# MARSLab-UMN/vi_depth_completion

Measured on AMD Instinct MI355X. Metric: frames/sec, higher is better.
Workload: dtype f32

## Files before the change

include/vidc.h:

```cpp
#ifndef VIDC_H
#define VIDC_H

#include <stddef.h>
#include <stdint.h>

#ifdef __cplusplus
extern "C" {
#endif

#if defined(__GNUC__) || defined(__clang__)
#pragma GCC visibility push(default)
#endif

typedef void* vidc_stream_t;

enum vidc_status {
    VIDC_OK = 0,
    VIDC_ERR_NULL = -1,
    VIDC_ERR_SHAPE = -2,
    VIDC_ERR_HIP = -3,
    VIDC_ERR_STATE = -4
};

int vidc_version(void);
const char* vidc_last_error(void);
int vidc_device_info(int* n_cu, int* lds_bytes_per_cu, char* arch_name, int arch_name_len);
#define VIDC_CLOCK_STAMP_WGS 8
int vidc_clock_stamp(long long* out, vidc_stream_t stream);


#define VIDC_WARP_PARAMS 32

int vidc_warp2dof_params(const float* gravity, const float* aligned, int B, float fx, float fy, float cx, float cy,
                         const float* K_inv, int W, int H, float* params, vidc_stream_t stream);

int vidc_warp2dof_fwd(const float* x, const float* params, float* y, int B, int C, int H, int W, float cx, float cy,
                      int align_corners, vidc_stream_t stream);

int vidc_warp2dof_inv_rot_norm(const float* x, const float* params, float* z, int B, int H, int W, float cx, float cy,
                               int align_corners, int normalize, vidc_stream_t stream);

int vidc_warp2dof_fwd_backward(const float* dy, const float* params, float* dx, int B, int C, int H, int W, float cx, float cy,
                               int align_corners, vidc_stream_t stream);
int vidc_warp2dof_inv_rot_norm_backward(const float* x, const float* dz, const float* params, float* dx, int B, int H, int W,
                                        float cx, float cy, int align_corners, int normalize, vidc_stream_t stream);


int vidc_pack_conv_weight(const float* w_oihw, float* w_packed, int Cout, int Cin, int KH, int KW, vidc_stream_t stream);

enum vidc_conv_flags {
    VIDC_RELU1 = 1,
    VIDC_AFFINE2 = 2,
    VIDC_RELU2 = 4,
    VIDC_RESIDUAL = 8,
    VIDC_RELU3 = 16,
    VIDC_ACCUM = 32,
    VIDC_SPLIT_OUT = 64,
    VIDC_NO_F32_OUT = 128,
    VIDC_X_PLANAR_GROUPS = 512,
    VIDC_MXFP8_OUT = 1024,
    VIDC_BF16_OUT = 2048,
    VIDC_STATS_OUT = 256
};

typedef struct vidc_conv_desc {
    const float* x;
    const float* w;
    float* y;
    const float* scale1;
    const float* shift1;
    const float* scale2;
    const float* shift2;
    const float* residual;
    float* workspace;
    int32_t B, H, W, Cin, ldx;
    int32_t Ho, Wo, Cout, ldy, ldr;
    int32_t KH, KW, stride, pad;
    int32_t flags;
    int32_t groups;
    int64_t x_gs, w_gs, y_gs, r_gs, p_gs;
    int32_t tile;
    int32_t splitk;
    int32_t precision;
    int32_t dilation;
    void* y_split;
} vidc_conv_desc;

enum vidc_conv_tile { VIDC_TILE_AUTO = 0, VIDC_TILE_128x128 = 1, VIDC_TILE_128x64 = 2, VIDC_TILE_64x128 = 3,
                      VIDC_TILE_64x64 = 4, VIDC_TILE_64x64_K2 = 5, VIDC_TILE_32x64_K2 = 6, VIDC_TILE_32x32_K4 = 7,
                      VIDC_TILE_32x128 = 8, VIDC_TILE_32x32_K8 = 9,
                      VIDC_TILE_32x64_K2_D5 = 10, VIDC_TILE_32x32_K4_D4 = 11, VIDC_TILE_32x128_D6 = 12, VIDC_TILE_64x64_K2_D4 = 13,
                      VIDC_TILE_32x64_K2_L = 14, VIDC_TILE_32x64_K2_D5_L = 15, VIDC_TILE_32x32_K4_D4_L = 16, VIDC_TILE_64x64_L = 17,
                      VIDC_TILE_64x64_K2_D4_L = 18, VIDC_TILE_64x128_L = 19, VIDC_TILE_128x64_L = 20,
                      VIDC_TILE_64x32_K2 = 21, VIDC_TILE_64x32_K2_D5 = 22, VIDC_TILE_64x32_K2_D5_L = 23,
                      VIDC_TILE_128x128_D3 = 24, VIDC_TILE_128x128_D3_L = 25,
                      VIDC_TILE_256x128 = 26, VIDC_TILE_128x256 = 27,
                      VIDC_TILE_32x64_K2_D2 = 28, VIDC_TILE_64x64_D2 = 29, VIDC_TILE_32x32_K4_D2 = 30, VIDC_TILE_64x128_D2 = 31,
                      VIDC_TILE_64x32_K2_D2 = 32,
                      VIDC_TILE_128x128_D4_P = 33, VIDC_TILE_128x128_D3_P = 34, VIDC_TILE_64x64_D4_P = 35, VIDC_TILE_128x64_D4_P = 36,
                      VIDC_TILE_64x64_K2_D4_P = 37, VIDC_TILE_64x32_K2_D5_P = 38, VIDC_TILE_32x64_K2_D5_P = 39,
                      VIDC_TILE_G96x32_STREAM = 40,
                      VIDC_TILE_G96x64_STREAM3 = 41,
                      VIDC_TILE_WINO4_FUSED = 42,
                      VIDC_TILE_COUNT = 43 };
enum vidc_conv_tile_kind { VIDC_TILE_KIND_AUTO = 0,
                           VIDC_TILE_KIND_MFMA = 1,
                           VIDC_TILE_KIND_STREAM = 2,
                           VIDC_TILE_KIND_WINOGRAD = 3 };
typedef struct vidc_tile_info {
    const char* name;
    int32_t bm, bn, wmw, wnw, wkw, ns, spec;
    int32_t kind;
    int32_t precisions, planner;
} vidc_tile_info;
int vidc_conv_tile_info(int tile, vidc_tile_info* out);

enum vidc_conv_precision { VIDC_PREC_FP32 = 0, VIDC_PREC_BF16X3 = 1, VIDC_PREC_BF16 = 2, VIDC_PREC_MXFP8 = 3 };
int vidc_quant_mxfp8(const float* x, void* y, long long rows, int C, int ldx, int groups, vidc_stream_t stream);
int vidc_pack_conv_weight_mxfp8(const float* w_oihw, void* w_packed, int Cout, int Cin, int KH, int KW, vidc_stream_t stream);
int vidc_cast_bf16(const float* x, void* y, long long rows, int C, int ldx, vidc_stream_t stream);
int vidc_split_bf16x3(const float* x, void* y, long long rows, int C, int ldx, vidc_stream_t stream);
int vidc_pack_conv_weight_bf16x3(const float* w_oihw, void* w_packed, int Cout, int Cin, int KH, int KW, vidc_stream_t stream);
int vidc_pack_conv_weight_bf16(const float* w_oihw, void* w_packed, int Cout, int Cin, int KH, int KW, vidc_stream_t stream);

int vidc_conv2d_bn_act(const vidc_conv_desc* d, vidc_stream_t stream);
#define VIDC_SPLITK_COUNTERS 16384
size_t vidc_conv2d_workspace_bytes(const vidc_conv_desc* d);
int vidc_conv2d_plan(vidc_conv_desc* d);

int vidc_winograd_tiles(int H, int W, int m, int* th, int* tw);
int vidc_winograd_weight_transform(const float* w_oihw, float* u, int Cout, int Cin, int m, vidc_stream_t stream);
int vidc_winograd_weight_pack_fused(const float* u, float* u_packed, int Cout, int Cin, vidc_stream_t stream);
int vidc_winograd_input_transform(const float* x, void* v, int B, int H, int W, int C, int ldx, int Cin, int m, int split, int ldv,
                                  vidc_stream_t stream);
int vidc_winograd_output_transform(const float* mm, float* y, void* y_split, const float* scale1, const float* shift1,
                                   const float* scale2, const float* shift2, int B, int Ho, int Wo, int C, int Cout, int ldy, int m,
                                   int flags, int ldm, vidc_stream_t stream);

int vidc_stem_conv3x3s2(const float* x, const float* w_oihw, float* y, int B, int Cin, int H, int W, int Cout, int ldy,
                        int relu, void* y_split, int split_ch0, vidc_stream_t stream);

int vidc_stem_conv3x3s2_warped(const float* x, const float* warp_params, const float* w_oihw, float* y, int B, int H, int W, int Cout, int ldy,
                               int relu, void* y_split, int split_ch0, float cx, float cy, int align_corners, vidc_stream_t stream);

int vidc_maxpool3x3s2(const float* x, float* y, int B, int H, int W, int C, int ldx, int ldy, void* y_split, vidc_stream_t stream);

enum vidc_up_flags { VIDC_UP_RELU = 1, VIDC_UP_ACCUM = 2, VIDC_UP_NO_F32_OUT = 4,
                     VIDC_UP_SUM_GROUPS_SHIFT = 8  };
int vidc_upsample_bilinear_ac(const float* x, float* y, int B, int h, int w, int C, int ldx, int H, int W, int ldy,
                              int flags, void* y_split, vidc_stream_t stream);

int vidc_avgpool2d(const float* x, float* y, int B, int H, int W, int C, int ldx, int kh, int kw, int sh, int sw, int ph, int pw, int ldy,
                   vidc_stream_t stream);

int vidc_avgpool2d_backward(const float* dy, float* dx, int B, int H, int W, int C, int ldx, int kh, int kw, int sh, int sw, int ph, int pw, int ldy,
                            vidc_stream_t stream);

int vidc_normalize_nchw(const float* x, float* y, int B, int C, int HW, vidc_stream_t stream);

int vidc_head_conv1x1_upsample(const float* x, const float* w, const float* bias, float* lowres, float* y, int B, int h,
                               int w_in, int Cin, int ldx, int Cout, int pad, int H, int W, int relu, vidc_stream_t stream);


#define VIDC_MAX_HYP 300
#define VIDC_PLANE_RECORD 16

size_t vidc_plane_scratch_bytes(int n_slots, int B, int HW);

int vidc_plane_ransac_normal(const float* normals, const uint8_t* ids, const int32_t* slots, int n_slots,
                             const int32_t* hyp_pix, int HW, uint8_t* inlier_mask, int32_t* counts, void* scratch,
                             vidc_stream_t stream);

int vidc_plane_offset(const float* homo, const float* depth, const int32_t* slots, int n_slots, int B,
                      const uint8_t* inlier_mask, const int32_t* counts, int HW, void* scratch, float* records,
                      vidc_stream_t stream);

int vidc_plane_offset_dense(const float* homo, const float* depth, const int32_t* slots, int n_slots, int B,
                            const uint8_t* inlier_mask, const int32_t* counts, int HW, void* scratch, float* records,
                            const int32_t* dense_hyp, const int32_t* dense_n, float* dense_dots, vidc_stream_t stream);

int vidc_plane_project_depth(const float* homo, const int32_t* slots, int n_slots, const uint8_t* inlier_mask, int HW,
                             void* scratch, float* records, float* plane_depth, vidc_stream_t stream);

int vidc_plane_info_count(int B, int HW);
int vidc_plane_finalize(const float* depth, float* plane_depth, int B, int HW, const float* records, int n_slots,
                        int32_t* info, vidc_stream_t stream);

int vidc_plane_block(const float* normals, const uint8_t* ids, const int32_t* slots, int n_slots, const int32_t* hyp_pix, int B, int HW,
                     const float* homo, const float* depth, uint8_t* inlier_mask, int32_t* counts, void* scratch, float* records,
                     const int32_t* dense_hyp, const int32_t* dense_n, float* dense_dots, float* plane_depth, int32_t* info,
                     vidc_stream_t stream);

int vidc_enrich_scatter(const float* plane_depth, const int32_t* sub, const int32_t* sub_offsets, const int32_t* chunk_base,
                        int B, int HW, float* enriched, vidc_stream_t stream);

int vidc_enrich_scatter_from(const float* plane_depth, const float* sparse_depth, const int32_t* sub, const int32_t* sub_offsets,
                             const int32_t* chunk_base, int B, int HW, float* enriched, vidc_stream_t stream);


int vidc_resize_coeffs(int in_size, int out_size, int32_t* bounds, int32_t* coeffs, int coeffs_capacity, int* ksize_out);

int vidc_resize_bilinear_u8_to_chw(const uint8_t* src_hwc, float* dst_chw, int B, int H, int W, int C, int Ho, int Wo,
                                   const int32_t* bounds_x, const int32_t* coeffs_x, int ksize_x, const int32_t* bounds_y,
                                   const int32_t* coeffs_y, int ksize_y, vidc_stream_t stream);

int vidc_rasterize_sparse_depth(const double* tracks, const int32_t* offsets, int B, double fx, double fy, double cx, double cy,
                                float* depth, int H, int W, vidc_stream_t stream);
int vidc_nearest_table(int in_size, int out_size, int32_t* table);
int vidc_resize_nearest_u16_depth(const uint16_t* src, float* dst, int B, int H, int W, int Ho, int Wo, const int32_t* xtab,
                                  const int32_t* ytab, float divisor, vidc_stream_t stream);


size_t vidc_depth_metrics_scratch_bytes(long long n);
int vidc_depth_metrics(const float* pred, const float* gt, long long n, double* stats, int accumulate, void* scratch, vidc_stream_t stream);

int vidc_depth_to_mm_u32(const float* depth, uint32_t* mm, long long n, vidc_stream_t stream);

int vidc_normal_metrics(const float* pred, const float* gt, const float* mask, int B, int HW, float* err, double* stats,
                        int accumulate, void* scratch, vidc_stream_t stream);

int vidc_hist_u16(const float* vals, long long n, int hi_filter, uint32_t* hist, vidc_stream_t stream);


size_t vidc_nms_scratch_bytes(int n);
int vidc_nms(const float* boxes_xyxy, const int32_t* order, int n, float threshold, int inclusive, int32_t* keep, int32_t* n_keep,
             void* scratch, vidc_stream_t stream);

size_t vidc_nms_segmented_scratch_bytes(int n_segments, int max_n);
int vidc_nms_segmented(const float* boxes_xyxy, const int32_t* seg_offsets, const int32_t* seg_counts, int n_segments, int max_n,
                       float threshold, int inclusive, int max_keep, int32_t* keep, int32_t* n_keep, void* scratch, vidc_stream_t stream);

int vidc_roi_align_forward(const float* x_nhwc, const float* rois, float* y, int K, int C, int H, int W, int ldx, int pooled_h,
                           int pooled_w, float spatial_scale, int sampling_ratio, vidc_stream_t stream);


int vidc_det_stem_im2col(const float* image01_nchw, float* cols, int B, int H, int W, int Hp, int Wp, float mean_b, float mean_g,
                         float mean_r, vidc_stream_t stream);
int vidc_upsample_nearest2x(const float* x, float* y, int B, int h, int w, int C, int ldx, int ldy, vidc_stream_t stream);

int vidc_mask_scale(const float* x, const float* image_nchw, float* y, int B, int h, int w, int C, int ldx, int ldy, int H, int W,
                    vidc_stream_t stream);
int vidc_rpn_topk_decode(const float* rpn_map, int B, int h, int w, int ld, int A, int stride, const float* cell_anchors_host,
                         int pre_nms_top_n, int img_h, int img_w, float* boxes, float* scores, long long out_stride, vidc_stream_t stream);
int vidc_rpn_topk_decode_levels(const float* const* maps_host, const int32_t* hw_host, const int32_t* strides_host,
                                const float* cell_anchors_host, const int32_t* level_offsets_host, int n_levels, int B, int ld, int A,
                                int pre_nms_top_n, int img_h, int img_w, float* boxes, float* scores, long long out_stride,
                                vidc_stream_t stream);
int vidc_rpn_select(const float* boxes, const float* scores, const int32_t* keep, const int32_t* n_keep, int B, int n_levels,
                    const int32_t* level_offsets_host, int per_level, int total, float* proposals, float* proposal_scores,
                    int32_t* n_proposals, vidc_stream_t stream);
int vidc_roi_align_fpn(const float* const* feats_host, const int32_t* hw_host, int n_levels, int C, const float* boxes, int B, int R,
                       int pooled, int sampling_ratio, float* y, vidc_stream_t stream);
int vidc_det_candidates(const float* head_out, int ld, const float* proposals, const int32_t* n_proposals, int B, int R, int img_h, int img_w,
                        float score_thresh, float* cand_boxes, float* cand_scores, int32_t* cand_src, int32_t* n_cand, vidc_stream_t stream);
int vidc_det_select(const float* cand_boxes, const float* cand_scores, const int32_t* cand_src, const int32_t* n_cand, const int32_t* keep,
                    const int32_t* n_keep, int B, int R, float* det_boxes, float* det_scores, int32_t* n_det, vidc_stream_t stream);
int vidc_mask_paste(const float* mask_logits, int ld, int cls, int M, const float* det_boxes, const int32_t* n_det, int B, int R, int H, int W,
                    float thresh, uint8_t* pasted, vidc_stream_t stream);
size_t vidc_instance_map_scratch_bytes(int B, int R, int H, int W);
int vidc_instance_map(const uint8_t* pasted, const float* det_scores, const int32_t* n_det, int B, int R, int H, int W, float confidence,
                      float min_fraction, uint8_t* inst, void* scratch, vidc_stream_t stream);


size_t vidc_train_scratch_bytes(long long M, int C);

int vidc_bn_train_forward(const float* x, float* y, long long M, int C, int ldx, int ldy, const float* gamma, const float* beta,
                          float* running_mean, float* running_var, float eps, float momentum, int relu, float* save_mean, float* save_rstd,
                          void* y_bf16, void* scratch, vidc_stream_t stream);
int vidc_bn_train_forward_add(const float* x, float* y, long long M, int C, int ldx, int ldy, const float* gamma, const float* beta,
                              float* running_mean, float* running_var, float eps, float momentum, int relu, float* save_mean, float* save_rstd,
                              void* y_bf16, const float* residual, int ldr, void* scratch, vidc_stream_t stream);
int vidc_bn_train_forward_stats(const float* x, float* y, long long M, int C, int ldx, int ldy, const float* gamma, const float* beta,
                                float* running_mean, float* running_var, float eps, float momentum, int relu, float* save_mean, float* save_rstd,
                                void* y_bf16, const float* residual, int ldr, const void* conv_stats, void* scratch, vidc_stream_t stream);
int vidc_bn_train_backward(const float* dy, const float* x, const float* y_relu, float* dx, long long M, int C, int lddy, int ldx, int ldy,
                           int lddx, const float* gamma, const float* save_mean, const float* save_rstd, float* dgamma, float* dbeta,
                           void* dx_bf16, void* scratch, vidc_stream_t stream);
int vidc_bn_train_backward_t(const float* dy, const float* x, const float* y_relu, float* dx, long long M, int C, int lddy, int ldx, int ldy,
                             int lddx, const float* gamma, const float* save_mean, const float* save_rstd, float* dgamma, float* dbeta,
                             void* dx_bf16, void* dx_bf16_t, int Mp, void* scratch, vidc_stream_t stream);
int vidc_colsum(const float* dy, long long M, int C, int ld, float* out, void* scratch, vidc_stream_t stream);
int vidc_add_rows(const float* a, const float* b, float* y, long long M, int C, int lda, int ldb, int ldy, int relu, vidc_stream_t stream);
int vidc_add_rows_bf16(const float* a, const float* b, float* y, long long M, int C, int lda, int ldb, int ldy, int relu, void* y_bf16,
                       vidc_stream_t stream);
int vidc_relu_backward(const float* dy, const float* y, float* dx, long long M, int C, int lddy, int ldy, int lddx, int accumulate,
                       vidc_stream_t stream);
int vidc_maxpool3x3s2_backward(const float* x, const float* dy, float* dx, int B, int H, int W, int C, int ldx, int lddy, int lddx,
                               vidc_stream_t stream);
int vidc_upsample_bilinear_ac_backward(const float* dy, float* dx, int B, int h, int w, int C, int lddy, int lddx, int H, int W,
                                       vidc_stream_t stream);
size_t vidc_head_backward_multi_scratch_bytes(int B, int h, int w, int C, int Cout, int pad);
int vidc_head_backward_multi(const float* g_low, const float* x, const float* wgt, float* dx, float* dw, float* dbias, int B, int h, int w,
                             int C, int ldx, int lddx, int Cout, int pad, void* scratch, vidc_stream_t stream);
size_t vidc_head_backward_scratch_bytes(int B, int h, int w, int C);
int vidc_head_backward(const float* g_low, const float* x, const float* wgt, float* dx, float* dw, float* dbias, int B, int h, int w, int C,
                       int ldx, int lddx, void* scratch, vidc_stream_t stream);
int vidc_masked_l1_loss(const float* pred, const float* gt, long long n, int hw, double* loss, float* dpred, float* terms, void* scratch,
                        vidc_stream_t stream);
int vidc_adam_step(float* p, const float* g, float* m, float* v, long long n, float lr, float beta1, float beta2, float eps, int step,
                   vidc_stream_t stream);
int vidc_train_bn_fold(int enable);
int vidc_grad_narrow_bf16(const float* x, void* y_bf16, long long n, vidc_stream_t stream);
int vidc_grad_widen_bf16(const void* x_bf16, float* y, long long n, vidc_stream_t stream);
int vidc_pack_conv_weight_dgrad(const float* w_oihw, float* w_packed, int Cout, int Cin, int KH, int KW, vidc_stream_t stream);
int vidc_host_mt19937_permutation_prefix(uint32_t* key624, int32_t* pos, long long n, int k, int32_t* idx_out, int32_t* scratch);
typedef struct vidc_pack_item {
    const float* w;
    float* packed;
    int32_t Cout, Cin, KH, KW;
    int32_t kind, reserved;
    int64_t block_begin;
} vidc_pack_item;
long long vidc_pack_item_blocks(int Cout, int Cin, int KH, int KW, int kind);
int vidc_pack_conv_weights_batched(const vidc_pack_item* items_device, int n_items, long long total_blocks, vidc_stream_t stream);
int vidc_zero_stuff(const float* dy, float* z, int B, int Ho, int Wo, int C, int lddy, int stride, int H, int W, vidc_stream_t stream);
size_t vidc_conv_wgrad_scratch_bytes(int B, int Ho, int Wo, int Cout, int Cin, int KH, int KW);
int vidc_conv_wgrad(const float* dy, const float* x, float* dw_oihw, int B, int H, int W, int Cin, int ldx, int Ho, int Wo, int Cout, int lddy,
                    int KH, int KW, int stride, int pad, void* scratch, vidc_stream_t stream);
size_t vidc_conv_wgrad_dilated_scratch_bytes(int B, int Ho, int Wo, int Cout, int Cin, int KH, int KW);
int vidc_conv_wgrad_dilated(const float* dy, const float* x, float* dw_oihw, int B, int H, int W, int Cin, int ldx, int Ho, int Wo, int Cout, int lddy,
                            int KH, int KW, int stride, int pad, int dilation, void* scratch, vidc_stream_t stream);
int vidc_im2col_transposed(const float* x, float* xt, int B, int H, int W, int C, int ldx, int Ho, int Wo, int KH, int KW, int stride, int pad,
                           int Mp, int split, vidc_stream_t stream);
int vidc_im2col_transposed_dilated(const float* x, float* xt, int B, int H, int W, int C, int ldx, int Ho, int Wo, int KH, int KW, int stride, int pad,
                                   int dilation, int Mp, int split, vidc_stream_t stream);
int vidc_transpose_bf16(const void* x_bf16, void* xt_bf16, long long M, int C, int Mp, vidc_stream_t stream);
int vidc_im2col_transposed_bf16(const void* x_bf16, void* xt_bf16, int B, int H, int W, int C, int Ho, int Wo, int KH, int KW, int stride, int pad,
                                int Mp, vidc_stream_t stream);
int vidc_wgrad_permute(const float* tmp, float* dw_oihw, int Cout, int Cin, int taps, vidc_stream_t stream);
int vidc_affine_act_backward(const float* dy, const float* y, const float* c_raw, const float* scale, const float* shift, float* dc,
                             float* dscale, float* dshift, long long M, int C, int lddy, int ldy, int ldc, int lddc, int relu, void* scratch,
                             vidc_stream_t stream);
int vidc_stem_conv3x3s2_backward_data(const float* dy, const float* y_relu, const float* w_oihw, float* dx_nchw, int B, int Cin, int H, int W,
                                      int Cout, int lddy, int ldy, vidc_stream_t stream);
size_t vidc_stem_wgrad_scratch_bytes(int B, int Cin, int H, int W, int Cout);
int vidc_stem_wgrad(const float* dy, const float* x_nchw, float* dw_oihw, int B, int Cin, int H, int W, int Cout, int lddy, void* scratch,
                    vidc_stream_t stream);


size_t vidc_normal_l1_loss_scratch_bytes(int B, int H, int W);
int vidc_normal_l1_loss(const float* pred, const float* normal_gt, const float* mask, int B, int H, int W, int normalize_prediction,
                        double* loss, double* count, double* angle, float* dpred, void* scratch, vidc_stream_t stream);

enum vidc_op_kind { VIDC_OP_CONV = 1, VIDC_OP_STEM = 2, VIDC_OP_MAXPOOL = 3, VIDC_OP_UPSAMPLE = 4, VIDC_OP_HEAD = 5,
                    VIDC_OP_WARP_PARAMS = 6, VIDC_OP_WARP_FWD = 7, VIDC_OP_WARP_INV = 8, VIDC_OP_COPY = 9, VIDC_OP_SPLIT = 10,
                    VIDC_OP_AVGPOOL = 11, VIDC_OP_NORMALIZE = 12, VIDC_OP_DET_IM2COL = 13, VIDC_OP_NEAREST2X = 14,
                     VIDC_OP_MASK = 16 ,
                    VIDC_OP_WINO_IN = 17  ,
                    VIDC_OP_WINO_OUT = 18 ,
                    VIDC_OP_QUANT = 19    ,
                    VIDC_OP_CAST = 20      };

typedef struct vidc_generic_args {
    const void* p[8];
    int32_t i[16];
    float f[8];
} vidc_generic_args;

typedef struct vidc_op {
    int32_t kind;
    int32_t stream_id;
    int32_t wait_mask;
    int32_t reserved;
    union {
        vidc_conv_desc conv;
        vidc_generic_args g;
    } u;
} vidc_op;

#define VIDC_MAX_STREAMS 4
#define VIDC_MAX_SEGMENTS 4

typedef struct vidc_program vidc_program;
int vidc_program_create(const vidc_op* ops, int n_ops, vidc_program** out);
int vidc_program_run(vidc_program* p, vidc_stream_t stream);
int vidc_program_capture(vidc_program* p, vidc_stream_t stream);
int vidc_program_launch(vidc_program* p, vidc_stream_t stream);
int vidc_program_run_range(vidc_program* p, vidc_stream_t stream, int begin, int end);
int vidc_program_capture_range(vidc_program* p, vidc_stream_t stream, int begin, int end, int segment);
int vidc_program_launch_segment(vidc_program* p, vidc_stream_t stream, int segment);
int vidc_program_time(vidc_program* p, vidc_stream_t stream, int iters, int use_graph, float* ms_out, float* per_op_ms);
int vidc_program_destroy(vidc_program* p);

#if defined(__GNUC__) || defined(__clang__)
#pragma GCC visibility pop
#endif

#ifdef __cplusplus
}
#endif
#endif
```

vi_depth_completion_amd/_lib.py:

```python
import ctypes as C
import os
import subprocess

_HERE = os.path.dirname(os.path.abspath(__file__))
LIB_PATH = os.path.join(_HERE, os.environ.get("VIDC_LIB_NAME", "libvidc.so"))
CSRC = os.path.join(_HERE, "csrc")

WARP_PARAMS = 32
MAX_HYP = 300
PLANE_RECORD = 16
MAX_STREAMS = 4
MAX_SEGMENTS = 4
CLOCK_STAMP_WGS = 8

RELU1, AFFINE2, RELU2, RESIDUAL, RELU3, ACCUM, SPLIT_OUT, NO_F32_OUT, STATS_OUT, X_PLANAR_GROUPS, MXFP8_OUT, BF16_OUT = 1, 2, 4, 8, 16, 32, 64, 128, 256, 512, 1024, 2048
UP_RELU, UP_ACCUM, UP_NO_F32_OUT = 1, 2, 4
OP_CONV, OP_STEM, OP_MAXPOOL, OP_UPSAMPLE, OP_HEAD, OP_WARP_PARAMS, OP_WARP_FWD, OP_WARP_INV, OP_COPY, OP_SPLIT, OP_AVGPOOL, OP_NORMALIZE, OP_DET_IM2COL, OP_NEAREST2X, _OP_RETIRED_15, OP_MASK, OP_WINO_IN, OP_WINO_OUT, OP_QUANT, OP_CAST = range(1, 21)
TILE_AUTO = 0
PREC_FP32, PREC_BF16X3, PREC_BF16, PREC_MXFP8 = 0, 1, 2, 3
TILE_KIND_AUTO, TILE_KIND_MFMA, TILE_KIND_STREAM, TILE_KIND_WINOGRAD = range(4)
SPLITK_COUNTERS = 16384

_f32p = C.POINTER(C.c_float)


class PackItem(C.Structure):
    _fields_ = [("w", C.c_void_p), ("packed", C.c_void_p), ("Cout", C.c_int32), ("Cin", C.c_int32), ("KH", C.c_int32), ("KW", C.c_int32),
                ("kind", C.c_int32), ("reserved", C.c_int32), ("block_begin", C.c_int64)]


class TileInfo(C.Structure):
    _fields_ = [("_name", C.c_char_p)] + [(f, C.c_int32) for f in ("bm", "bn", "wmw", "wnw", "wkw", "ns", "spec", "kind", "precisions", "planner")]
    name = property(lambda self: self._name.decode())


class ConvDesc(C.Structure):
    _fields_ = [
        ("x", C.c_void_p), ("w", C.c_void_p), ("y", C.c_void_p),
        ("scale1", C.c_void_p), ("shift1", C.c_void_p), ("scale2", C.c_void_p), ("shift2", C.c_void_p),
        ("residual", C.c_void_p), ("workspace", C.c_void_p),
        ("B", C.c_int32), ("H", C.c_int32), ("W", C.c_int32), ("Cin", C.c_int32), ("ldx", C.c_int32),
        ("Ho", C.c_int32), ("Wo", C.c_int32), ("Cout", C.c_int32), ("ldy", C.c_int32), ("ldr", C.c_int32),
        ("KH", C.c_int32), ("KW", C.c_int32), ("stride", C.c_int32), ("pad", C.c_int32),
        ("flags", C.c_int32), ("groups", C.c_int32),
        ("x_gs", C.c_int64), ("w_gs", C.c_int64), ("y_gs", C.c_int64), ("r_gs", C.c_int64), ("p_gs", C.c_int64),
        ("tile", C.c_int32), ("splitk", C.c_int32), ("precision", C.c_int32), ("dilation", C.c_int32),
        ("y_split", C.c_void_p),
    ]


def conv_desc(B, H, W, Cin, Cout, KH=1, KW=1, stride=1, pad=0, dilation=1, groups=1, Ho=None, Wo=None, ldx=None, ldy=None,
              precision=PREC_FP32, x=None, w=None, y=None, scale1=None, shift1=None, shared_affine=False, scale2=None, shift2=None,
              relu1=False, relu2=False, residual=None, ldr=None, relu3=False, accumulate=False, split_out=None, mx_out=None,
              stats_out=None, no_f32_out=False, wino_fused=False, bf16_out=None):
    assert sum(p is not None for p in (split_out, mx_out, stats_out, bf16_out)) <= 1
    dil = max(dilation, 1)
    Ho = (H + 2 * pad - dil * (KH - 1) - 1) // stride + 1 if Ho is None else Ho
    Wo = (W + 2 * pad - dil * (KW - 1) - 1) // stride + 1 if Wo is None else Wo
    ldx = (Cin if precision == PREC_MXFP8 else groups * Cin) if ldx is None else ldx
    ldy = groups * Cout if ldy is None else ldy
    flags = ((RELU1 if relu1 else 0) | (AFFINE2 | (RELU2 if relu2 else 0) if scale2 is not None else 0) |
             (RESIDUAL | (RELU3 if relu3 else 0) if residual is not None else 0) | (ACCUM if accumulate else 0) |
             (SPLIT_OUT if split_out is not None else 0) | (MXFP8_OUT if mx_out is not None else 0) | (STATS_OUT if stats_out is not None else 0) |
             (BF16_OUT if bf16_out is not None else 0) |
             (NO_F32_OUT if no_f32_out and (split_out is not None or mx_out is not None or bf16_out is not None) else 0))
    x_gs, w_gs = Cin, Cout * KH * KW * Cin
    if precision == PREC_BF16:
        Cin, ldx = Cin // 2, ldx // 2
        x_gs, w_gs = Cin, Cout * KH * KW * Cin
    elif precision == PREC_MXFP8:
        assert ldx == Cin, "an MXFP8 activation is one dense plane of Cin channels per group"
        x_gs, w_gs = B * H * W * Cin // 128 * 33, Cout * KH * KW * Cin // 128 * 33
        Cin, ldx = Cin // 4, Cin // 4
    if wino_fused:
        w_gs = 36 * Cout * Cin
    return ConvDesc(x=x, w=w, y=y, scale1=scale1, shift1=shift1, scale2=scale2, shift2=shift2, residual=residual,
                    B=B, H=H, W=W, Cin=Cin, ldx=ldx, Ho=Ho, Wo=Wo, Cout=Cout, ldy=ldy, ldr=(0 if residual is None else ldr or ldy),
                    KH=KH, KW=KW, stride=stride, pad=pad, flags=flags, groups=groups,
                    x_gs=x_gs, w_gs=w_gs, y_gs=Cout, r_gs=(0 if residual is None else Cout),
                    p_gs=(0 if shared_affine and groups > 1 else Cout),
                    tile=(__getattr__("TILE_WINO4_FUSED") if wino_fused else TILE_AUTO), splitk=1, precision=precision, dilation=dil,
                    y_split=next((p for p in (split_out, mx_out, stats_out, bf16_out) if p is not None), None))


def gemm_desc(rows, K, N, groups=1, ldx=None, ldy=None, precision=PREC_FP32, planar=False, x=None, w=None, y=None, scale1=None,
              shift1=None, shared_affine=True):
    d = conv_desc(1, 1, rows, K, N, groups=groups, ldx=ldx, ldy=ldy, precision=precision, x=x, w=w, y=y, scale1=scale1, shift1=shift1,
                  shared_affine=shared_affine)
    if planar:
        d.flags |= X_PLANAR_GROUPS
        d.x_gs, d.y_gs = rows * d.ldx, rows * d.ldy
    return d


def plan(d, tiling=None):
    if tiling is not None:
        d.tile, d.splitk = tiling
    else:
        check(lib().vidc_conv2d_plan(C.byref(d)), "conv plan")
    return d


class GenericArgs(C.Structure):
    _fields_ = [("p", C.c_void_p * 8), ("i", C.c_int32 * 16), ("f", C.c_float * 8)]


class _OpUnion(C.Union):
    _fields_ = [("conv", ConvDesc), ("g", GenericArgs)]


class Op(C.Structure):
    _fields_ = [("kind", C.c_int32), ("stream_id", C.c_int32), ("wait_mask", C.c_int32), ("reserved", C.c_int32),
                ("u", _OpUnion)]


_vp, _i, _f = C.c_void_p, C.c_int, C.c_float
SIGNATURES = {
    "vidc_version": (C.c_int, []),
    "vidc_last_error": (C.c_char_p, []),
    "vidc_device_info": (C.c_int, [C.POINTER(C.c_int), C.POINTER(C.c_int), C.c_char_p, _i]),
    "vidc_warp2dof_params": (C.c_int, [_vp, _vp, _i, _f, _f, _f, _f, _vp, _i, _i, _vp, _vp]),
    "vidc_warp2dof_fwd": (C.c_int, [_vp, _vp, _vp, _i, _i, _i, _i, _f, _f, _i, _vp]),
    "vidc_warp2dof_inv_rot_norm": (C.c_int, [_vp, _vp, _vp, _i, _i, _i, _f, _f, _i, _i, _vp]),
    "vidc_warp2dof_fwd_backward": (C.c_int, [_vp, _vp, _vp, _i, _i, _i, _i, _f, _f, _i, _vp]),
    "vidc_warp2dof_inv_rot_norm_backward": (C.c_int, [_vp, _vp, _vp, _vp, _i, _i, _i, _f, _f, _i, _i, _vp]),
    "vidc_affine_act_backward": (C.c_int, [_vp, _vp, _vp, _vp, _vp, _vp, _vp, _vp, C.c_longlong, _i, _i, _i, _i, _i, _i, _vp, _vp]),
    "vidc_stem_conv3x3s2_backward_data": (C.c_int, [_vp, _vp, _vp, _vp, _i, _i, _i, _i, _i, _i, _i, _vp]),
    "vidc_pack_conv_weight": (C.c_int, [_vp, _vp, _i, _i, _i, _i, _vp]),
    "vidc_split_bf16x3": (C.c_int, [_vp, _vp, C.c_longlong, _i, _i, _vp]),
    "vidc_pack_conv_weight_bf16x3": (C.c_int, [_vp, _vp, _i, _i, _i, _i, _vp]),
    "vidc_pack_conv_weight_bf16": (C.c_int, [_vp, _vp, _i, _i, _i, _i, _vp]),
    "vidc_quant_mxfp8": (C.c_int, [_vp, _vp, C.c_longlong, _i, _i, _i, _vp]),
    "vidc_pack_conv_weight_mxfp8": (C.c_int, [_vp, _vp, _i, _i, _i, _i, _vp]),
    "vidc_conv2d_bn_act": (C.c_int, [C.POINTER(ConvDesc), _vp]),
    "vidc_conv2d_workspace_bytes": (C.c_size_t, [C.POINTER(ConvDesc)]),
    "vidc_conv2d_plan": (C.c_int, [C.POINTER(ConvDesc)]),
    "vidc_conv_tile_info": (C.c_int, [_i, C.POINTER(TileInfo)]),
    "vidc_train_scratch_bytes": (C.c_size_t, [C.c_longlong, _i]),
    "vidc_bn_train_forward": (C.c_int, [_vp, _vp, C.c_longlong, _i, _i, _i, _vp, _vp, _vp, _vp, _f, _f, _i, _vp, _vp, _vp, _vp, _vp]),
    "vidc_bn_train_forward_add": (C.c_int, [_vp, _vp, C.c_longlong, _i, _i, _i, _vp, _vp, _vp, _vp, _f, _f, _i, _vp, _vp, _vp, _vp, _i, _vp, _vp]),
    "vidc_bn_train_forward_stats": (C.c_int, [_vp, _vp, C.c_longlong, _i, _i, _i, _vp, _vp, _vp, _vp, _f, _f, _i, _vp, _vp, _vp, _vp, _i, _vp, _vp, _vp]),
    "vidc_bn_train_backward": (C.c_int, [_vp, _vp, _vp, _vp, C.c_longlong, _i, _i, _i, _i, _i, _vp, _vp, _vp, _vp, _vp, _vp, _vp, _vp]),
    "vidc_bn_train_backward_t": (C.c_int, [_vp, _vp, _vp, _vp, C.c_longlong, _i, _i, _i, _i, _i, _vp, _vp, _vp, _vp, _vp, _vp, _vp, _i, _vp, _vp]),
    "vidc_colsum": (C.c_int, [_vp, C.c_longlong, _i, _i, _vp, _vp, _vp]),
    "vidc_add_rows": (C.c_int, [_vp, _vp, _vp, C.c_longlong, _i, _i, _i, _i, _i, _vp]),
    "vidc_add_rows_bf16": (C.c_int, [_vp, _vp, _vp, C.c_longlong, _i, _i, _i, _i, _i, _vp, _vp]),
    "vidc_relu_backward": (C.c_int, [_vp, _vp, _vp, C.c_longlong, _i, _i, _i, _i, _i, _vp]),
    "vidc_maxpool3x3s2_backward": (C.c_int, [_vp, _vp, _vp, _i, _i, _i, _i, _i, _i, _i, _vp]),
    "vidc_upsample_bilinear_ac_backward": (C.c_int, [_vp, _vp, _i, _i, _i, _i, _i, _i, _i, _i, _vp]),
    "vidc_head_backward_scratch_bytes": (C.c_size_t, [_i, _i, _i, _i]),
    "vidc_head_backward": (C.c_int, [_vp, _vp, _vp, _vp, _vp, _vp, _i, _i, _i, _i, _i, _i, _vp, _vp]),
    "vidc_masked_l1_loss": (C.c_int, [_vp, _vp, C.c_longlong, _i, _vp, _vp, _vp, _vp, _vp]),
    "vidc_normal_l1_loss_scratch_bytes": (C.c_size_t, [_i, _i, _i]),
    "vidc_normal_l1_loss": (C.c_int, [_vp, _vp, _vp, _i, _i, _i, _i, _vp, _vp, _vp, _vp, _vp, _vp]),
    "vidc_head_backward_multi_scratch_bytes": (C.c_size_t, [_i, _i, _i, _i, _i, _i]),
    "vidc_head_backward_multi": (C.c_int, [_vp, _vp, _vp, _vp, _vp, _vp, _i, _i, _i, _i, _i, _i, _i, _i, _vp, _vp]),
    "vidc_clock_stamp": (C.c_int, [_vp, _vp]),
    "vidc_adam_step": (C.c_int, [_vp, _vp, _vp, _vp, C.c_longlong, _f, _f, _f, _f, _i, _vp]),
    "vidc_train_bn_fold": (C.c_int, [_i]),
    "vidc_grad_narrow_bf16": (C.c_int, [_vp, _vp, C.c_longlong, _vp]),
    "vidc_grad_widen_bf16": (C.c_int, [_vp, _vp, C.c_longlong, _vp]),
    "vidc_pack_conv_weight_dgrad": (C.c_int, [_vp, _vp, _i, _i, _i, _i, _vp]),
    "vidc_cast_bf16": (C.c_int, [_vp, _vp, C.c_longlong, _i, _i, _vp]),
    "vidc_host_mt19937_permutation_prefix": (C.c_int, [_vp, _vp, C.c_longlong, _i, _vp, _vp]),
    "vidc_pack_item_blocks": (C.c_longlong, [_i, _i, _i, _i, _i]),
    "vidc_pack_conv_weights_batched": (C.c_int, [_vp, _i, C.c_longlong, _vp]),
    "vidc_zero_stuff": (C.c_int, [_vp, _vp, _i, _i, _i, _i, _i, _i, _i, _i, _vp]),
    "vidc_conv_wgrad_scratch_bytes": (C.c_size_t, [_i, _i, _i, _i, _i, _i, _i]),
    "vidc_conv_wgrad": (C.c_int, [_vp, _vp, _vp, _i, _i, _i, _i, _i, _i, _i, _i, _i, _i, _i, _i, _i, _vp, _vp]),
    "vidc_im2col_transposed": (C.c_int, [_vp, _vp, _i, _i, _i, _i, _i, _i, _i, _i, _i, _i, _i, _i, _i, _vp]),
    "vidc_conv_wgrad_dilated_scratch_bytes": (C.c_size_t, [_i, _i, _i, _i, _i, _i, _i]),
    "vidc_conv_wgrad_dilated": (C.c_int, [_vp, _vp, _vp, _i, _i, _i, _i, _i, _i, _i, _i, _i, _i, _i, _i, _i, _i, _vp, _vp]),
    "vidc_im2col_transposed_dilated": (C.c_int, [_vp, _vp, _i, _i, _i, _i, _i, _i, _i, _i, _i, _i, _i, _i, _i, _i, _vp]),
    "vidc_wgrad_permute": (C.c_int, [_vp, _vp, _i, _i, _i, _vp]),
    "vidc_transpose_bf16": (C.c_int, [_vp, _vp, C.c_longlong, _i, _i, _vp]),
    "vidc_im2col_transposed_bf16": (C.c_int, [_vp, _vp, _i, _i, _i, _i, _i, _i, _i, _i, _i, _i, _i, _vp]),
    "vidc_stem_wgrad_scratch_bytes": (C.c_size_t, [_i, _i, _i, _i, _i]),
    "vidc_stem_wgrad": (C.c_int, [_vp, _vp, _vp, _i, _i, _i, _i, _i, _i, _vp, _vp]),
    "vidc_winograd_tiles": (C.c_int, [_i, _i, _i, C.POINTER(C.c_int), C.POINTER(C.c_int)]),
    "vidc_winograd_weight_transform": (C.c_int, [_vp, _vp, _i, _i, _i, _vp]),
    "vidc_winograd_weight_pack_fused": (C.c_int, [_vp, _vp, _i, _i, _vp]),
    "vidc_winograd_input_transform": (C.c_int, [_vp, _vp, _i, _i, _i, _i, _i, _i, _i, _i, _i, _vp]),
    "vidc_winograd_output_transform": (C.c_int, [_vp, _vp, _vp, _vp, _vp, _vp, _vp, _i, _i, _i, _i, _i, _i, _i, _i, _i, _vp]),
    "vidc_stem_conv3x3s2": (C.c_int, [_vp, _vp, _vp, _i, _i, _i, _i, _i, _i, _i, _vp, _i, _vp]),
    "vidc_stem_conv3x3s2_warped": (C.c_int, [_vp, _vp, _vp, _vp, _i, _i, _i, _i, _i, _i, _vp, _i, _f, _f, _i, _vp]),
    "vidc_maxpool3x3s2": (C.c_int, [_vp, _vp, _i, _i, _i, _i, _i, _i, _vp, _vp]),
    "vidc_upsample_bilinear_ac": (C.c_int, [_vp, _vp, _i, _i, _i, _i, _i, _i, _i, _i, _i, _vp, _vp]),
    "vidc_avgpool2d": (C.c_int, [_vp, _vp, _i, _i, _i, _i, _i, _i, _i, _i, _i, _i, _i, _i, _vp]),
    "vidc_avgpool2d_backward": (C.c_int, [_vp, _vp, _i, _i, _i, _i, _i, _i, _i, _i, _i, _i, _i, _i, _vp]),
    "vidc_normalize_nchw": (C.c_int, [_vp, _vp, _i, _i, _i, _vp]),
    "vidc_head_conv1x1_upsample": (C.c_int, [_vp, _vp, _vp, _vp, _vp, _i, _i, _i, _i, _i, _i, _i, _i, _i, _i, _vp]),
    "vidc_plane_scratch_bytes": (C.c_size_t, [_i, _i, _i]),
    "vidc_plane_ransac_normal": (C.c_int, [_vp, _vp, _vp, _i, _vp, _i, _vp, _vp, _vp, _vp]),
    "vidc_plane_offset": (C.c_int, [_vp, _vp, _vp, _i, _i, _vp, _vp, _i, _vp, _vp, _vp]),
    "vidc_plane_offset_dense": (C.c_int, [_vp, _vp, _vp, _i, _i, _vp, _vp, _i, _vp, _vp, _vp, _vp, _vp, _vp]),
    "vidc_plane_project_depth": (C.c_int, [_vp, _vp, _i, _vp, _i, _vp, _vp, _vp, _vp]),
    "vidc_plane_info_count": (C.c_int, [_i, _i]),
    "vidc_plane_finalize": (C.c_int, [_vp, _vp, _i, _i, _vp, _i, _vp, _vp]),
    "vidc_plane_block": (C.c_int, [_vp, _vp, _vp, _i, _vp, _i, _i, _vp, _vp, _vp, _vp, _vp, _vp, _vp, _vp, _vp, _vp, _vp, _vp]),
    "vidc_enrich_scatter": (C.c_int, [_vp, _vp, _vp, _vp, _i, _i, _vp, _vp]),
    "vidc_enrich_scatter_from": (C.c_int, [_vp, _vp, _vp, _vp, _vp, _i, _i, _vp, _vp]),
    "vidc_resize_coeffs": (C.c_int, [_i, _i, _vp, _vp, _i, C.POINTER(C.c_int)]),
    "vidc_resize_bilinear_u8_to_chw": (C.c_int, [_vp, _vp, _i, _i, _i, _i, _i, _i, _vp, _vp, _i, _vp, _vp, _i, _vp]),
    "vidc_rasterize_sparse_depth": (C.c_int, [_vp, _vp, _i, C.c_double, C.c_double, C.c_double, C.c_double, _vp, _i, _i, _vp]),
    "vidc_nearest_table": (C.c_int, [_i, _i, _vp]),
    "vidc_resize_nearest_u16_depth": (C.c_int, [_vp, _vp, _i, _i, _i, _i, _i, _vp, _vp, C.c_float, _vp]),
    "vidc_depth_metrics_scratch_bytes": (C.c_size_t, [C.c_longlong]),
    "vidc_depth_metrics": (C.c_int, [_vp, _vp, C.c_longlong, _vp, _i, _vp, _vp]),
    "vidc_depth_to_mm_u32": (C.c_int, [_vp, _vp, C.c_longlong, _vp]),
    "vidc_normal_metrics": (C.c_int, [_vp, _vp, _vp, _i, _i, _vp, _vp, _i, _vp, _vp]),
    "vidc_hist_u16": (C.c_int, [_vp, C.c_longlong, _i, _vp, _vp]),
    "vidc_nms_scratch_bytes": (C.c_size_t, [_i]),
    "vidc_nms": (C.c_int, [_vp, _vp, _i, _f, _i, _vp, _vp, _vp, _vp]),
    "vidc_nms_segmented_scratch_bytes": (C.c_size_t, [_i, _i]),
    "vidc_nms_segmented": (C.c_int, [_vp, _vp, _vp, _i, _i, _f, _i, _i, _vp, _vp, _vp, _vp]),
    "vidc_roi_align_forward": (C.c_int, [_vp, _vp, _vp, _i, _i, _i, _i, _i, _i, _i, _f, _i, _vp]),
    "vidc_det_stem_im2col": (C.c_int, [_vp, _vp, _i, _i, _i, _i, _i, _f, _f, _f, _vp]),
    "vidc_upsample_nearest2x": (C.c_int, [_vp, _vp, _i, _i, _i, _i, _i, _i, _vp]),
    "vidc_mask_scale": (C.c_int, [_vp, _vp, _vp, _i, _i, _i, _i, _i, _i, _i, _i, _vp]),
    "vidc_rpn_topk_decode": (C.c_int, [_vp, _i, _i, _i, _i, _i, _i, _vp, _i, _i, _i, _vp, _vp, C.c_longlong, _vp]),
    "vidc_rpn_topk_decode_levels": (C.c_int, [_vp, _vp, _vp, _vp, _vp, _i, _i, _i, _i, _i, _i, _i, _vp, _vp, C.c_longlong, _vp]),
    "vidc_rpn_select": (C.c_int, [_vp, _vp, _vp, _vp, _i, _i, _vp, _i, _i, _vp, _vp, _vp, _vp]),
    "vidc_roi_align_fpn": (C.c_int, [_vp, _vp, _i, _i, _vp, _i, _i, _i, _i, _vp, _vp]),
    "vidc_det_candidates": (C.c_int, [_vp, _i, _vp, _vp, _i, _i, _i, _i, _f, _vp, _vp, _vp, _vp, _vp]),
    "vidc_det_select": (C.c_int, [_vp, _vp, _vp, _vp, _vp, _vp, _i, _i, _vp, _vp, _vp, _vp]),
    "vidc_mask_paste": (C.c_int, [_vp, _i, _i, _i, _vp, _vp, _i, _i, _i, _i, _f, _vp, _vp]),
    "vidc_instance_map_scratch_bytes": (C.c_size_t, [_i, _i, _i, _i]),
    "vidc_instance_map": (C.c_int, [_vp, _vp, _vp, _i, _i, _i, _i, _f, _f, _vp, _vp, _vp]),
    "vidc_program_create": (C.c_int, [C.POINTER(Op), _i, C.POINTER(_vp)]),
    "vidc_program_run": (C.c_int, [_vp, _vp]),
    "vidc_program_capture": (C.c_int, [_vp, _vp]),
    "vidc_program_launch": (C.c_int, [_vp, _vp]),
    "vidc_program_run_range": (C.c_int, [_vp, _vp, _i, _i]),
    "vidc_program_capture_range": (C.c_int, [_vp, _vp, _i, _i, _i]),
    "vidc_program_launch_segment": (C.c_int, [_vp, _vp, _i]),
    "vidc_program_time": (C.c_int, [_vp, _vp, _i, _i, _f32p, _f32p]),
    "vidc_program_destroy": (C.c_int, [_vp]),
}

_lib = None


def build(force=False, verbose=False):
    srcs = [os.path.join(CSRC, f) for f in os.listdir(CSRC) if f.endswith((".hip", ".h", ".def", ".map")) or f == "Makefile"]
    srcs.append(os.path.join(os.path.dirname(_HERE), "include", "vidc.h"))
    if not force and os.path.exists(LIB_PATH) and os.path.getmtime(LIB_PATH) >= max(os.path.getmtime(s) for s in srcs):
        return LIB_PATH
    cmd = ["make", "-C", CSRC, "-j%d" % min(8, os.cpu_count() or 1)]
    r = subprocess.run(cmd, stdout=subprocess.PIPE, stderr=subprocess.STDOUT, text=True)
    if verbose or r.returncode != 0:
        print(r.stdout)
    if r.returncode != 0:
        raise RuntimeError("building libvidc.so failed (hipcc, gfx950)")
    return LIB_PATH


def lib():
    global _lib
    if _lib is None:
        if not os.path.exists(LIB_PATH):
            raise RuntimeError("libvidc.so is not built (%s); run `python -c 'import __graft_entry__ as g; g.build()'`. "
                               "There is no CPU/eager fallback for the HIP path." % LIB_PATH)
        L = C.CDLL(LIB_PATH)
        for name, (res, args) in SIGNATURES.items():
            fn = getattr(L, name)
            fn.restype, fn.argtypes = res, args
        if L.vidc_version() != 1:
            raise RuntimeError("libvidc.so ABI version mismatch")
        _lib = L
    return _lib


_TILE_TABLES = ("TILE_INFO", "TILE_COUNT", "TILE_NAMES", "MXFP8_TILES", "BF16_TILES", "TILE_WINO4_FUSED")


def __getattr__(name):
    if name not in _TILE_TABLES:
        raise AttributeError("module %r has no attribute %r" % (__name__, name))
    info, ti = {}, TileInfo()
    while lib().vidc_conv_tile_info(len(info), C.byref(ti)) == 0:
        info[len(info)], ti = ti, TileInfo()
    globals().update(TILE_INFO=info, TILE_COUNT=len(info), TILE_NAMES={t: ti.name for t, ti in info.items()},
                     MXFP8_TILES=tuple(t for t, ti in info.items() if ti.precisions >> PREC_MXFP8 & 1),
                     BF16_TILES=tuple(t for t, ti in info.items() if ti.precisions >> PREC_BF16 & 1),
                     TILE_WINO4_FUSED=next(t for t, ti in info.items() if ti.kind == TILE_KIND_WINOGRAD))
    return globals()[name]


def check(rc, what=""):
    if rc != 0:
        raise RuntimeError("libvidc %s failed (status %d): %s" % (what, rc, lib().vidc_last_error().decode()))


def ptr(t):
    return None if t is None else t.data_ptr()


_raw_stream = None


def current_stream():
    global _raw_stream
    import torch
    if _raw_stream is None:
        get_raw, get_dev = getattr(torch._C, "_cuda_getCurrentRawStream", None), getattr(torch._C, "_cuda_getDevice", None)
        if get_raw is not None and get_dev is not None:
            _raw_stream = lambda: get_raw(get_dev())
        else:
            _raw_stream = lambda: torch.cuda.current_stream().cuda_stream
    return _raw_stream()
```

vi_depth_completion_amd/csrc/common.h:

```cpp
#pragma once
#include <hip/hip_runtime.h>
#include <cstdio>
#include <cstdarg>
#include "../../include/vidc.h"

namespace vidc {

void set_error(const char* fmt, ...);

inline hipStream_t as_stream(vidc_stream_t s) { return reinterpret_cast<hipStream_t>(s); }

#define VIDC_REQUIRE(cond, code, ...)                  \
    do {                                               \
        if (!(cond)) {                                 \
            ::vidc::set_error(__VA_ARGS__);            \
            return (code);                             \
        }                                              \
    } while (0)

#define VIDC_CHECK_LAUNCH(name)                                                          \
    do {                                                                                 \
        hipError_t e__ = hipGetLastError();                                              \
        if (e__ != hipSuccess) {                                                         \
            ::vidc::set_error("%s: launch failed: %s", name, hipGetErrorString(e__));    \
            return VIDC_ERR_HIP;                                                         \
        }                                                                                \
    } while (0)

#define VIDC_HIP(call)                                                                        \
    do {                                                                                      \
        hipError_t e__ = (call);                                                              \
        if (e__ != hipSuccess) {                                                              \
            ::vidc::set_error("%s failed: %s", #call, hipGetErrorString(e__));                \
            return VIDC_ERR_HIP;                                                              \
        }                                                                                     \
    } while (0)

__host__ __device__ inline int cdiv(int a, int b) { return (a + b - 1) / b; }

constexpr int TT = 256;
inline unsigned blocks(long long n) { return (unsigned)((n + TT - 1) / TT); }
template <int K>
__device__ inline void block_tree(double (*red)[TT]) {
    __syncthreads();
    for (int off = TT / 2; off > 0; off >>= 1) {
        if ((int)threadIdx.x < off) {
#pragma unroll
            for (int k = 0; k < K; ++k) red[k][threadIdx.x] += red[k][threadIdx.x + off];
        }
        __syncthreads();
    }
}

int launch_wgemm_stream(const vidc_conv_desc& d, hipStream_t st);
int launch_wino4_fused(const vidc_conv_desc& d, hipStream_t st);

__device__ inline unsigned short bf16_rne(float x) {
    unsigned u = __float_as_uint(x);
    u += 0x7FFFu + ((u >> 16) & 1u);
    return (unsigned short)(u >> 16);
}
__device__ inline void split_bf16(float x, unsigned short& hi, unsigned short& lo) {
    hi = bf16_rne(x);
    lo = bf16_rne(x - __uint_as_float((unsigned)hi << 16));
}
__device__ inline void store_split(unsigned short* img, size_t row, int ld, int c, float v) {
    unsigned short hi, lo;
    split_bf16(v, hi, lo);
    unsigned short* u = img + (row * ld + (c & ~31)) * 2 + (c & 31);
    u[0] = hi;
    u[32] = lo;
}
__device__ inline void store_split4(unsigned short* img, size_t row, int ld, int c, float4 v) {
    unsigned short h0, h1, h2, h3, l0, l1, l2, l3;
    split_bf16(v.x, h0, l0); split_bf16(v.y, h1, l1); split_bf16(v.z, h2, l2); split_bf16(v.w, h3, l3);
    unsigned short* u = img + (row * ld + (c & ~31)) * 2 + (c & 31);
    *reinterpret_cast<uint2*>(u) = make_uint2(h0 | ((unsigned)h1 << 16), h2 | ((unsigned)h3 << 16));
    *reinterpret_cast<uint2*>(u + 32) = make_uint2(l0 | ((unsigned)l1 << 16), l2 | ((unsigned)l3 << 16));
}

struct Taps {
    int o00, o01, o10, o11;
    float w00, w01, w10, w11;
};

__device__ inline Taps make_taps(float u, float v, float cx, float cy, int W, int H, int align_corners) {
    float gx = (1.0f / ((float)W / 2)) * (u - cx);
    float gy = (1.0f / ((float)H / 2)) * (v - cy);
    float ix, iy;
    if (align_corners) {
        ix = ((gx + 1.f) / 2.f) * (float)(W - 1);
        iy = ((gy + 1.f) / 2.f) * (float)(H - 1);
    } else {
        ix = ((gx + 1.f) * (float)W - 1.f) / 2.f;
        iy = ((gy + 1.f) * (float)H - 1.f) / 2.f;
    }
    if (!(ix > -2.0f && ix < (float)W + 1.0f)) ix = -2.0f;
    if (!(iy > -2.0f && iy < (float)H + 1.0f)) iy = -2.0f;
    float fx0 = floorf(ix), fy0 = floorf(iy);
    int x0 = (int)fx0, y0 = (int)fy0, x1 = x0 + 1, y1 = y0 + 1;
    float wx1 = ix - fx0, wx0 = (fx0 + 1.f) - ix;
    float wy1 = iy - fy0, wy0 = (fy0 + 1.f) - iy;
    bool vx0 = x0 >= 0 && x0 < W, vx1 = x1 >= 0 && x1 < W, vy0 = y0 >= 0 && y0 < H, vy1 = y1 >= 0 && y1 < H;
    int cx0 = min(max(x0, 0), W - 1), cx1 = min(max(x1, 0), W - 1), cy0 = min(max(y0, 0), H - 1), cy1 = min(max(y1, 0), H - 1);
    Taps t;
    t.o00 = cy0 * W + cx0; t.o01 = cy0 * W + cx1; t.o10 = cy1 * W + cx0; t.o11 = cy1 * W + cx1;
    t.w00 = (vx0 && vy0) ? wx0 * wy0 : 0.f;
    t.w01 = (vx1 && vy0) ? wx1 * wy0 : 0.f;
    t.w10 = (vx0 && vy1) ? wx0 * wy1 : 0.f;
    t.w11 = (vx1 && vy1) ? wx1 * wy1 : 0.f;
    return t;
}

__device__ inline float sample(const float* __restrict__ plane, const Taps& t) {
    return fmaf(plane[t.o11], t.w11, fmaf(plane[t.o10], t.w10, fmaf(plane[t.o01], t.w01, plane[t.o00] * t.w00)));
}
__device__ inline float sample_nt(const float* __restrict__ plane, const Taps& t) {
    const float a00 = __builtin_nontemporal_load(plane + t.o00), a01 = __builtin_nontemporal_load(plane + t.o01);
    const float a10 = __builtin_nontemporal_load(plane + t.o10), a11 = __builtin_nontemporal_load(plane + t.o11);
    return fmaf(a11, t.w11, fmaf(a10, t.w10, fmaf(a01, t.w01, a00 * t.w00)));
}

__device__ inline Taps warp_fwd_taps(const float* __restrict__ p, int X, int Y, float cx, float cy, int W, int H, int align_corners) {
    const float px_min = p[27], py_min = p[28], kw = p[29], kh = p[30];
    float Xs, Ys, P0, P1, P2;
    {
#pragma clang fp contract(off)
        Xs = (1.0f / kw) * (float)X + px_min;
        Ys = (1.0f / kh) * (float)Y + py_min;
        P0 = (p[18] * Xs + p[19] * Ys) + p[20];
        P1 = (p[21] * Xs + p[22] * Ys) + p[23];
        P2 = (p[24] * Xs + p[25] * Ys) + p[26];
    }
    return make_taps(P0 / P2, P1 / P2, cx, cy, W, H, align_corners);
}

}
```

vi_depth_completion_amd/csrc/pointwise.hip:

```cpp
#include "common.h"
#include <cstdlib>

namespace {

template <int CIN, bool WARP, bool CONTROL = false>
__global__ void __launch_bounds__(256)
stem_conv_kernel(const float* __restrict__ x, const float* __restrict__ w, float* __restrict__ y, int H, int W, int Ho, int Wo,
                 int Cout, int ldy, int relu, unsigned short* __restrict__ ysp, int ch0, const float* __restrict__ warp_params, float wcx, float wcy,
                 int align_corners) {
    constexpr int PIX = 64;
    constexpr int PW = 2 * PIX + 1;
    __shared__ float patch[CIN][3][PW + 3];
    const int b = blockIdx.z, oy = blockIdx.y, ox0 = blockIdx.x * PIX;
    const int tid = threadIdx.x;
    const size_t plane = (size_t)H * W;
    const float* xb = x + (size_t)b * CIN * plane;
    const int ix_base = ox0 * 2 - 1, iy_base = oy * 2 - 1;
    if constexpr (WARP) {
        __shared__ float wp[VIDC_WARP_PARAMS];
        if (tid < VIDC_WARP_PARAMS) wp[tid] = __builtin_nontemporal_load(warp_params + (size_t)b * VIDC_WARP_PARAMS + tid);
        __syncthreads();
        for (int e = tid; e < 3 * PW; e += 256) {
            const int r = e / PW, i = e - r * PW;
            const int iy = iy_base + r, ix = ix_base + i;
            const bool in = (unsigned)iy < (unsigned)H && (unsigned)ix < (unsigned)W;
            vidc::Taps t;
            if (in) t = vidc::warp_fwd_taps(wp, ix, iy, wcx, wcy, W, H, align_corners);
            if constexpr (CONTROL) {
                typedef float f32x2_ __attribute__((ext_vector_type(2)));
                f32x2_ wa = {t.w01, t.w10}, ones = {1.0f, 1.0f}, wd;
                asm volatile("v_pk_mul_f32 %0, %1, %2 op_sel:[0,1] op_sel_hi:[1,0]" : "=&v"(wd) : "v"(wa), "v"(ones));
                t.w01 = wd.x;
                t.w10 = wd.y;
            }
#pragma unroll
            for (int c = 0; c < CIN; ++c) {
                float v = 0.f;
                if (in) {
                    const float* pl = xb + c * plane;
                    const float a00 = __hip_atomic_load(pl + t.o00, __ATOMIC_RELAXED, __HIP_MEMORY_SCOPE_SYSTEM), a01 = __hip_atomic_load(pl + t.o01, __ATOMIC_RELAXED, __HIP_MEMORY_SCOPE_SYSTEM);
                    const float a10 = __hip_atomic_load(pl + t.o10, __ATOMIC_RELAXED, __HIP_MEMORY_SCOPE_SYSTEM), a11 = __hip_atomic_load(pl + t.o11, __ATOMIC_RELAXED, __HIP_MEMORY_SCOPE_SYSTEM);
                    v = fmaf(a11, t.w11, fmaf(a10, t.w10, fmaf(a01, t.w01, a00 * t.w00)));
                }
                patch[c][r][i] = v;
            }
        }
    } else {
        for (int e = tid; e < CIN * 3 * PW; e += 256) {
            int c = e / (3 * PW), r = (e / PW) % 3, i = e % PW;
            int iy = iy_base + r, ix = ix_base + i;
            float v = 0.f;
            if ((unsigned)iy < (unsigned)H && (unsigned)ix < (unsigned)W) v = __builtin_nontemporal_load(xb + c * plane + (size_t)iy * W + ix);
            patch[c][r][i] = v;
        }
    }
    __syncthreads();
    const int co = tid & 63, pgrp = tid >> 6;
    for (int cbase = 0; cbase < Cout; cbase += 64) {
        const int c_out = cbase + co;
        float wr[CIN * 9];
        if (c_out < Cout) {
#pragma unroll
            for (int k = 0; k < CIN * 9; ++k) wr[k] = w[(size_t)c_out * CIN * 9 + k];
        }
        for (int p = pgrp; p < PIX; p += 4) {
            const int ox = ox0 + p;
            if (ox >= Wo || c_out >= Cout) continue;
            float acc = 0.f;
#pragma unroll
            for (int c = 0; c < CIN; ++c)
#pragma unroll
                for (int r = 0; r < 3; ++r)
#pragma unroll
                    for (int s = 0; s < 3; ++s) acc += patch[c][r][2 * p + s] * wr[(c * 3 + r) * 3 + s];
            if (relu) acc = fmaxf(acc, 0.f);
            const size_t row = (size_t)(b * Ho + oy) * Wo + ox;
            if (y) y[row * ldy + c_out] = acc;
            if (ysp) vidc::store_split(ysp, row, ldy, ch0 + c_out, acc);
        }
    }
}

__device__ __forceinline__ void xcd_band_block(unsigned& bx, unsigned& by) {
    const unsigned gx = gridDim.x, L = blockIdx.y * gx + blockIdx.x, per = (gx >> 3) * gridDim.y;
    const unsigned idx = (L & 7u) * per + (L >> 3);
    by = idx / gx;
    bx = idx - by * gx;
}
constexpr unsigned kRowGroup = 4;
__device__ __forceinline__ void xcd_rowgroup_block(unsigned& bx, unsigned& by) {
    const unsigned gx = gridDim.x, L = blockIdx.y * gx + blockIdx.x;
    const unsigned k = L & 7u, j = L >> 3, per_group = kRowGroup * gx;
    const unsigned t = j / per_group, r = j - t * per_group;
    const unsigned rr = r / gx;
    by = (t * 8u + k) * kRowGroup + rr;
    bx = r - rr * gx;
}

__global__ void __launch_bounds__(256)
maxpool_kernel(const float* __restrict__ x, float* __restrict__ y, int B, int H, int W, int C, int ldx, int Ho, int Wo, int ldy,
               unsigned short* __restrict__ ysp) {
    const unsigned q = (unsigned)C / 4u;
    unsigned bx, by;
    xcd_band_block(bx, by);
    const unsigned i = bx * blockDim.x + threadIdx.x;
    if (i >= (unsigned)Wo * q) return;
    const int ox = (int)(i / q);
    const int c = (int)(i - (unsigned)ox * q) * 4;
    const int b = (int)(by / (unsigned)Ho), oy = (int)(by - (unsigned)b * (unsigned)Ho);
    float4 m = make_float4(-INFINITY, -INFINITY, -INFINITY, -INFINITY);
#pragma unroll
    for (int r = 0; r < 3; ++r) {
        int iy = oy * 2 - 1 + r;
        if ((unsigned)iy >= (unsigned)H) continue;
#pragma unroll
        for (int s = 0; s < 3; ++s) {
            int ix = ox * 2 - 1 + s;
            if ((unsigned)ix >= (unsigned)W) continue;
            float4 v = *reinterpret_cast<const float4*>(&x[((size_t)(b * H + iy) * W + ix) * ldx + c]);
            m.x = fmaxf(m.x, v.x); m.y = fmaxf(m.y, v.y); m.z = fmaxf(m.z, v.z); m.w = fmaxf(m.w, v.w);
        }
    }
    const size_t row = (size_t)(b * Ho + oy) * Wo + ox;
    if (y) *reinterpret_cast<float4*>(&y[row * ldy + c]) = m;
    if (ysp) vidc::store_split4(ysp, row, ldy, c, m);
}

__device__ inline void src_index(int dst, int in, int out, int& i0, int& i1, float& l1) {
    float scale = out > 1 ? (float)(in - 1) / (float)(out - 1) : 0.f;
    float s = scale * (float)dst;
    i0 = (int)s;
    if (i0 > in - 1) i0 = in - 1;
    i1 = i0 + ((i0 < in - 1) ? 1 : 0);
    l1 = s - (float)i0;
}

__global__ void __launch_bounds__(256)
upsample_kernel(const float* __restrict__ x, float* __restrict__ y, int B, int h, int w, int C, int ldx, int H, int W, int ldy,
                int flags, unsigned short* __restrict__ ysp) {
    const unsigned q = (unsigned)C / 4u;
    unsigned bx, by;
    xcd_rowgroup_block(bx, by);
    const unsigned i = bx * blockDim.x + threadIdx.x;
    if (i >= (unsigned)W * q) return;
    const int ox = (int)(i / q);
    const int c = (int)(i - (unsigned)ox * q) * 4;
    if (by >= (unsigned)(B * H)) return;
    const int b = (int)(by / (unsigned)H), oy = (int)(by - (unsigned)b * (unsigned)H);
    int y0, y1, x0, x1; float ly, lx;
    src_index(oy, h, H, y0, y1, ly);
    src_index(ox, w, W, x0, x1, lx);
    const float hy = 1.f - ly, hx = 1.f - lx;
    const size_t row = (size_t)(b * H + oy) * W + ox;
    float4* dst = reinterpret_cast<float4*>(&y[row * ldy + c]);
    const int G = (flags >> 8) & 0xFF;
    float4 o = make_float4(0.f, 0.f, 0.f, 0.f);
    if (flags & VIDC_UP_ACCUM) o = *dst;
    for (int g = 0; g < (G > 1 ? G : 1); ++g) {
        const float* xb = x + (size_t)b * h * w * ldx + g * C + c;
        const float4 v00 = *reinterpret_cast<const float4*>(xb + ((size_t)y0 * w + x0) * ldx);
        const float4 v01 = *reinterpret_cast<const float4*>(xb + ((size_t)y0 * w + x1) * ldx);
        const float4 v10 = *reinterpret_cast<const float4*>(xb + ((size_t)y1 * w + x0) * ldx);
        const float4 v11 = *reinterpret_cast<const float4*>(xb + ((size_t)y1 * w + x1) * ldx);
        float4 u;
        u.x = hy * (hx * v00.x + lx * v01.x) + ly * (hx * v10.x + lx * v11.x);
        u.y = hy * (hx * v00.y + lx * v01.y) + ly * (hx * v10.y + lx * v11.y);
        u.z = hy * (hx * v00.z + lx * v01.z) + ly * (hx * v10.z + lx * v11.z);
        u.w = hy * (hx * v00.w + lx * v01.w) + ly * (hx * v10.w + lx * v11.w);
        if (flags & VIDC_UP_RELU) { u.x = fmaxf(u.x, 0.f); u.y = fmaxf(u.y, 0.f); u.z = fmaxf(u.z, 0.f); u.w = fmaxf(u.w, 0.f); }
        o.x = u.x + o.x; o.y = u.y + o.y; o.z = u.z + o.z; o.w = u.w + o.w;
    }
    if (!(flags & VIDC_UP_NO_F32_OUT)) *dst = o;
    if (ysp) vidc::store_split4(ysp, row, ldy, c, o);
}

__global__ void __launch_bounds__(256)
head_conv_kernel(const float* __restrict__ x, const float* __restrict__ w, const float* __restrict__ bias, float* __restrict__ low,
                 int B, int h, int wd, int Cin, int ldx, int Cout, int pad) {
    const int hp = h + 2 * pad, wp = wd + 2 * pad;
    const int wave = (blockIdx.x * blockDim.x + threadIdx.x) >> 6, lane = threadIdx.x & 63;
    const int total = B * hp * wp;
    if (wave >= total) return;
    const int px = wave % wp, py = (wave / wp) % hp, b = wave / (wp * hp);
    const int iy = py - pad, ix = px - pad;
    float acc[4] = {0.f, 0.f, 0.f, 0.f};
    if ((unsigned)iy < (unsigned)h && (unsigned)ix < (unsigned)wd) {
        const float* xp = x + ((size_t)(b * h + iy) * wd + ix) * ldx;
        for (int c = lane; c < Cin; c += 64) {
            float v = xp[c];
            for (int o = 0; o < Cout; ++o) acc[o] += v * w[o * Cin + c];
        }
    }
    for (int o = 0; o < Cout; ++o) {
        float v = acc[o];
#pragma unroll
        for (int off = 32; off > 0; off >>= 1) v += __shfl_xor(v, off, 64);
        if (lane == 0) low[((size_t)(b * Cout + o) * hp + py) * wp + px] = v + bias[o];
    }
}

__global__ void __launch_bounds__(256)
head_upsample_kernel(const float* __restrict__ low, float* __restrict__ y, int BC, int h, int w, int H, int W, int relu) {
    const long long idx = (long long)blockIdx.x * blockDim.x + threadIdx.x;
    if (idx >= (long long)BC * H * W) return;
    const int ox = (int)(idx % W);
    const int oy = (int)((idx / W) % H);
    const int bc = (int)(idx / ((long long)W * H));
    int y0, y1, x0, x1; float ly, lx;
    src_index(oy, h, H, y0, y1, ly);
    src_index(ox, w, W, x0, x1, lx);
    const float* p = low + (size_t)bc * h * w;
    const float hy = 1.f - ly, hx = 1.f - lx;
    float v = hy * (hx * p[y0 * w + x0] + lx * p[y0 * w + x1]) + ly * (hx * p[y1 * w + x0] + lx * p[y1 * w + x1]);
    if (relu) v = fmaxf(v, 0.f);
    y[idx] = v;
}

__global__ void __launch_bounds__(256)
avgpool_kernel(const float* __restrict__ x, float* __restrict__ y, int B, int H, int W, int C, int ldx, int kh, int kw, int sh, int sw, int ph,
               int pw, int Ho, int Wo, int ldy) {
    const int q = C / 4;
    const long long idx = (long long)blockIdx.x * blockDim.x + threadIdx.x;
    if (idx >= (long long)B * Ho * Wo * q) return;
    const int c = (int)(idx % q) * 4;
    long long t = idx / q;
    const int ox = (int)(t % Wo); t /= Wo;
    const int oy = (int)(t % Ho);
// ... 176 lines not shown
```

vi_depth_completion_amd/csrc/program.hip:

```cpp
#include "common.h"
#include <vector>

struct vidc_program {
    std::vector<vidc_op> ops;
    hipStream_t side[VIDC_MAX_STREAMS] = {nullptr, nullptr, nullptr, nullptr};
    hipEvent_t ev[VIDC_MAX_STREAMS] = {nullptr, nullptr, nullptr, nullptr};
    hipEvent_t fork_ev = nullptr;
    int n_streams = 1;
    hipGraph_t graph[VIDC_MAX_SEGMENTS] = {};
    hipGraphExec_t exec[VIDC_MAX_SEGMENTS] = {};
    std::vector<hipEvent_t> op_ev;
};

namespace {

int launch_op(const vidc_op& op, hipStream_t st) {
    vidc_stream_t s = reinterpret_cast<vidc_stream_t>(st);
    const vidc_generic_args& g = op.u.g;
    switch (op.kind) {
        case VIDC_OP_CONV:
            return vidc_conv2d_bn_act(&op.u.conv, s);
        case VIDC_OP_STEM:
            if (g.p[4])
                return vidc_stem_conv3x3s2_warped((const float*)g.p[0], (const float*)g.p[4], (const float*)g.p[1], (float*)g.p[2], g.i[0], g.i[2], g.i[3], g.i[4],
                                                  g.i[5], g.i[6], const_cast<void*>(g.p[3]), g.i[7], g.f[0], g.f[1], g.i[8], s);
            return vidc_stem_conv3x3s2((const float*)g.p[0], (const float*)g.p[1], (float*)g.p[2], g.i[0], g.i[1], g.i[2], g.i[3],
                                       g.i[4], g.i[5], g.i[6], const_cast<void*>(g.p[3]), g.i[7], s);
        case VIDC_OP_MAXPOOL:
            return vidc_maxpool3x3s2((const float*)g.p[0], (float*)g.p[1], g.i[0], g.i[1], g.i[2], g.i[3], g.i[4], g.i[5],
                                     const_cast<void*>(g.p[2]), s);
        case VIDC_OP_UPSAMPLE:
            return vidc_upsample_bilinear_ac((const float*)g.p[0], (float*)g.p[1], g.i[0], g.i[1], g.i[2], g.i[3], g.i[4], g.i[5],
                                             g.i[6], g.i[7], g.i[8], const_cast<void*>(g.p[2]), s);
        case VIDC_OP_HEAD:
            return vidc_head_conv1x1_upsample((const float*)g.p[0], (const float*)g.p[1], (const float*)g.p[2], (float*)g.p[3],
                                              (float*)g.p[4], g.i[0], g.i[1], g.i[2], g.i[3], g.i[4], g.i[5], g.i[6], g.i[7],
                                              g.i[8], g.i[9], s);
        case VIDC_OP_WARP_PARAMS:
            return vidc_warp2dof_params((const float*)g.p[0], (const float*)g.p[1], g.i[0], g.f[0], g.f[1], g.f[2], g.f[3],
                                        (const float*)g.p[2], g.i[1], g.i[2], (float*)g.p[3], s);
        case VIDC_OP_WARP_FWD:
            return vidc_warp2dof_fwd((const float*)g.p[0], (const float*)g.p[1], (float*)g.p[2], g.i[0], g.i[1], g.i[2], g.i[3],
                                     g.f[0], g.f[1], g.i[4], s);
        case VIDC_OP_WARP_INV:
            return vidc_warp2dof_inv_rot_norm((const float*)g.p[0], (const float*)g.p[1], (float*)g.p[2], g.i[0], g.i[1], g.i[2],
                                              g.f[0], g.f[1], g.i[3], g.i[4], s);
        case VIDC_OP_SPLIT: {
            long long rows = (long long)(uint32_t)g.i[0] | ((long long)(uint32_t)g.i[1] << 32);
            return vidc_split_bf16x3((const float*)g.p[0], const_cast<void*>(g.p[1]), rows, g.i[2], g.i[3], s);
        }
        case VIDC_OP_AVGPOOL:
            return vidc_avgpool2d((const float*)g.p[0], (float*)g.p[1], g.i[0], g.i[1], g.i[2], g.i[3], g.i[4], g.i[5], g.i[6], g.i[7], g.i[8],
                                  g.i[9], g.i[10], g.i[11], s);
        case VIDC_OP_NORMALIZE:
            return vidc_normalize_nchw((const float*)g.p[0], (float*)g.p[1], g.i[0], g.i[1], g.i[2], s);
        case VIDC_OP_DET_IM2COL:
            return vidc_det_stem_im2col((const float*)g.p[0], (float*)g.p[1], g.i[0], g.i[1], g.i[2], g.i[3], g.i[4], g.f[0], g.f[1], g.f[2], s);
        case VIDC_OP_NEAREST2X:
            return vidc_upsample_nearest2x((const float*)g.p[0], (float*)g.p[1], g.i[0], g.i[1], g.i[2], g.i[3], g.i[4], g.i[5], s);
        case VIDC_OP_MASK:
            return vidc_mask_scale((const float*)g.p[0], (const float*)g.p[1], (float*)g.p[2], g.i[0], g.i[1], g.i[2], g.i[3], g.i[4], g.i[5], g.i[6], g.i[7], s);
        case VIDC_OP_WINO_IN:
            return vidc_winograd_input_transform((const float*)g.p[0], const_cast<void*>(g.p[1]), g.i[0], g.i[1], g.i[2], g.i[3], g.i[4], g.i[5], g.i[6],
                                                 g.i[7], g.i[8], s);
        case VIDC_OP_WINO_OUT:
            return vidc_winograd_output_transform((const float*)g.p[0], (float*)g.p[1], const_cast<void*>(g.p[2]), (const float*)g.p[3],
                                                  (const float*)g.p[4], (const float*)g.p[5], (const float*)g.p[6], g.i[0], g.i[1], g.i[2], g.i[3],
                                                  g.i[4], g.i[5], g.i[6], g.i[7], g.i[8], s);
        case VIDC_OP_QUANT: {
            long long rows = (long long)(uint32_t)g.i[0] | ((long long)(uint32_t)g.i[1] << 32);
            return vidc_quant_mxfp8((const float*)g.p[0], const_cast<void*>(g.p[1]), rows, g.i[2], g.i[3], g.i[4], s);
        }
        case VIDC_OP_CAST: {
            long long rows = (long long)(uint32_t)g.i[0] | ((long long)(uint32_t)g.i[1] << 32);
            return vidc_cast_bf16((const float*)g.p[0], const_cast<void*>(g.p[1]), rows, g.i[2], g.i[3], s);
        }
        case VIDC_OP_COPY: {
            size_t bytes = (size_t)(uint32_t)g.i[0] | ((size_t)(uint32_t)g.i[1] << 32);
            VIDC_HIP(hipMemcpyAsync(const_cast<void*>(g.p[1]), g.p[0], bytes, hipMemcpyDeviceToDevice, st));
            return VIDC_OK;
        }
        default:
            vidc::set_error("program: unknown op kind %d", op.kind);
            return VIDC_ERR_SHAPE;
    }
}

int issue(vidc_program* p, hipStream_t main, bool timing, size_t begin = 0, size_t end = (size_t)-1) {
    if (end > p->ops.size()) end = p->ops.size();
    hipStream_t st[VIDC_MAX_STREAMS];
    st[0] = main;
    for (int k = 1; k < VIDC_MAX_STREAMS; ++k) st[k] = p->side[k];
    bool forked[VIDC_MAX_STREAMS] = {true, false, false, false};
    bool dirty[VIDC_MAX_STREAMS] = {false, false, false, false};
    for (size_t i = begin; i < end; ++i) {
        const vidc_op& op = p->ops[i];
        const int sid = op.stream_id;
        if (!forked[sid]) {
            VIDC_HIP(hipEventRecord(p->fork_ev, main));
            VIDC_HIP(hipStreamWaitEvent(st[sid], p->fork_ev, 0));
            forked[sid] = true;
        }
        for (int k = 0; k < p->n_streams; ++k)
            if (k != sid && (op.wait_mask >> k & 1)) {
                VIDC_HIP(hipEventRecord(p->ev[k], st[k]));
                VIDC_HIP(hipStreamWaitEvent(st[sid], p->ev[k], 0));
                if (sid == 0) dirty[k] = false;
            }
        if (timing) VIDC_HIP(hipEventRecord(p->op_ev[i], st[sid]));
        int rc = launch_op(op, st[sid]);
        if (rc != VIDC_OK) return rc;
        dirty[sid] = true;
    }
    if (timing) VIDC_HIP(hipEventRecord(p->op_ev[end], main));
    for (int k = 1; k < p->n_streams; ++k)
        if (forked[k] && dirty[k]) {
            VIDC_HIP(hipEventRecord(p->ev[k], st[k]));
            VIDC_HIP(hipStreamWaitEvent(main, p->ev[k], 0));
        }
    return VIDC_OK;
}

}

extern "C" int vidc_program_create(const vidc_op* ops, int n_ops, vidc_program** out) {
    VIDC_REQUIRE(ops && out, VIDC_ERR_NULL, "vidc_program_create: null pointer");
    VIDC_REQUIRE(n_ops > 0, VIDC_ERR_SHAPE, "vidc_program_create: empty program");
    vidc_program* p = new vidc_program();
    p->ops.assign(ops, ops + n_ops);
    for (const vidc_op& op : p->ops) {
        if (op.stream_id < 0 || op.stream_id >= VIDC_MAX_STREAMS) {
            delete p;
            vidc::set_error("vidc_program_create: stream_id %d out of range", op.stream_id);
            return VIDC_ERR_SHAPE;
        }
        if (op.stream_id + 1 > p->n_streams) p->n_streams = op.stream_id + 1;
    }
    hipError_t e = hipSuccess;
    for (int k = 1; k < p->n_streams && e == hipSuccess; ++k) e = hipStreamCreateWithFlags(&p->side[k], hipStreamNonBlocking);
    for (int k = 0; k < p->n_streams && e == hipSuccess; ++k) e = hipEventCreateWithFlags(&p->ev[k], hipEventDisableTiming);
    if (e == hipSuccess) e = hipEventCreateWithFlags(&p->fork_ev, hipEventDisableTiming);
    if (e != hipSuccess) {
        vidc::set_error("vidc_program_create: stream/event creation failed: %s", hipGetErrorString(e));
        vidc_program_destroy(p);
        return VIDC_ERR_HIP;
    }
    *out = p;
    return VIDC_OK;
}

extern "C" int vidc_program_run(vidc_program* p, vidc_stream_t stream) {
    VIDC_REQUIRE(p, VIDC_ERR_STATE, "vidc_program_run: null program");
    return issue(p, vidc::as_stream(stream), false);
}

namespace {
int capture_range(vidc_program* p, hipStream_t st, size_t begin, size_t end, int seg) {
    if (p->exec[seg]) { hipGraphExecDestroy(p->exec[seg]); p->exec[seg] = nullptr; }
    if (p->graph[seg]) { hipGraphDestroy(p->graph[seg]); p->graph[seg] = nullptr; }
    VIDC_HIP(hipStreamBeginCapture(st, hipStreamCaptureModeThreadLocal));
    int rc = issue(p, st, false, begin, end);
    hipGraph_t g = nullptr;
    hipError_t e = hipStreamEndCapture(st, &g);
    if (rc != VIDC_OK) { if (g) hipGraphDestroy(g); return rc; }
    if (e != hipSuccess) { vidc::set_error("hipStreamEndCapture failed: %s", hipGetErrorString(e)); return VIDC_ERR_HIP; }
    p->graph[seg] = g;
    VIDC_HIP(hipGraphInstantiate(&p->exec[seg], p->graph[seg], nullptr, nullptr, 0));
    return VIDC_OK;
}
}

extern "C" int vidc_program_capture(vidc_program* p, vidc_stream_t stream) {
    VIDC_REQUIRE(p, VIDC_ERR_STATE, "vidc_program_capture: null program");
    hipStream_t st = vidc::as_stream(stream);
    VIDC_REQUIRE(st != nullptr, VIDC_ERR_STATE, "vidc_program_capture: needs a non-default stream");
    return capture_range(p, st, 0, p->ops.size(), 0);
}

extern "C" int vidc_program_launch(vidc_program* p, vidc_stream_t stream) {
    VIDC_REQUIRE(p && p->exec[0], VIDC_ERR_STATE, "vidc_program_launch: program not captured");
    for (int k = 0; k < VIDC_MAX_SEGMENTS && p->exec[k]; ++k)
        VIDC_HIP(hipGraphLaunch(p->exec[k], vidc::as_stream(stream)));
    return VIDC_OK;
}

extern "C" int vidc_program_run_range(vidc_program* p, vidc_stream_t stream, int begin, int end) {
    VIDC_REQUIRE(p, VIDC_ERR_STATE, "vidc_program_run_range: null program");
    VIDC_REQUIRE(begin >= 0 && begin < end && (size_t)end <= p->ops.size(), VIDC_ERR_SHAPE, "vidc_program_run_range: bad range [%d, %d)", begin, end);
    return issue(p, vidc::as_stream(stream), false, (size_t)begin, (size_t)end);
}

extern "C" int vidc_program_capture_range(vidc_program* p, vidc_stream_t stream, int begin, int end, int segment) {
    VIDC_REQUIRE(p, VIDC_ERR_STATE, "vidc_program_capture_range: null program");
    VIDC_REQUIRE(begin >= 0 && begin < end && (size_t)end <= p->ops.size(), VIDC_ERR_SHAPE, "vidc_program_capture_range: bad range [%d, %d)", begin, end);
    VIDC_REQUIRE(segment >= 0 && segment < VIDC_MAX_SEGMENTS, VIDC_ERR_SHAPE, "vidc_program_capture_range: segment %d out of range", segment);
    hipStream_t st = vidc::as_stream(stream);
    VIDC_REQUIRE(st != nullptr, VIDC_ERR_STATE, "vidc_program_capture_range: needs a non-default stream");
    return capture_range(p, st, (size_t)begin, (size_t)end, segment);
}

extern "C" int vidc_program_launch_segment(vidc_program* p, vidc_stream_t stream, int segment) {
    VIDC_REQUIRE(p && segment >= 0 && segment < VIDC_MAX_SEGMENTS && p->exec[segment], VIDC_ERR_STATE,
                 "vidc_program_launch_segment: segment not captured");
    VIDC_HIP(hipGraphLaunch(p->exec[segment], vidc::as_stream(stream)));
    return VIDC_OK;
}

extern "C" int vidc_program_time(vidc_program* p, vidc_stream_t stream, int iters, int use_graph, float* ms_out, float* per_op_ms) {
    VIDC_REQUIRE(p && ms_out, VIDC_ERR_NULL, "vidc_program_time: null pointer");
    VIDC_REQUIRE(iters > 0, VIDC_ERR_SHAPE, "vidc_program_time: iters must be > 0");
    hipStream_t st = vidc::as_stream(stream);
    hipEvent_t t0, t1;
    VIDC_HIP(hipEventCreate(&t0));
    VIDC_HIP(hipEventCreate(&t1));
    int rc = VIDC_OK;
    if (per_op_ms && !use_graph) {
        const size_t n = p->ops.size();
        if (p->op_ev.size() != n + 1) {
            p->op_ev.resize(n + 1);
            for (auto& e : p->op_ev) VIDC_HIP(hipEventCreate(&e));
        }
// ... 45 lines not shown
```

vi_depth_completion_amd/csrc/winograd.hip:

```cpp
#include "common.h"

#pragma clang fp contract(off)

namespace {

template <int N> struct vecn {
    float v[N];
};
template <int N> __device__ __forceinline__ vecn<N> operator+(const vecn<N>& a, const vecn<N>& b) {
    vecn<N> r;
#pragma unroll
    for (int i = 0; i < N; ++i) r.v[i] = a.v[i] + b.v[i];
    return r;
}
template <int N> __device__ __forceinline__ vecn<N> operator-(const vecn<N>& a, const vecn<N>& b) {
    vecn<N> r;
#pragma unroll
    for (int i = 0; i < N; ++i) r.v[i] = a.v[i] - b.v[i];
    return r;
}
template <int N> __device__ __forceinline__ vecn<N> operator*(float s, const vecn<N>& a) {
    vecn<N> r;
#pragma unroll
    for (int i = 0; i < N; ++i) r.v[i] = s * a.v[i];
    return r;
}
template <int N> __device__ __forceinline__ vecn<N> vzero() {
    vecn<N> r;
#pragma unroll
    for (int i = 0; i < N; ++i) r.v[i] = 0.f;
    return r;
}
template <int N> __device__ __forceinline__ vecn<N> vload(const float* p) {
    vecn<N> r;
    if constexpr (N == 4) {
        const float4 t = *reinterpret_cast<const float4*>(p);
        r.v[0] = t.x; r.v[1] = t.y; r.v[2] = t.z; r.v[3] = t.w;
    } else {
#pragma unroll
        for (int i = 0; i < N; ++i) r.v[i] = p[i];
    }
    return r;
}
template <int N> __device__ __forceinline__ void vstore(float* p, const vecn<N>& a) {
    if constexpr (N == 4) *reinterpret_cast<float4*>(p) = make_float4(a.v[0], a.v[1], a.v[2], a.v[3]);
    else {
#pragma unroll
        for (int i = 0; i < N; ++i) p[i] = a.v[i];
    }
}
template <int N> __device__ __forceinline__ void vstore_split(unsigned short* img, size_t row, int ld, int c, const vecn<N>& a) {
    if constexpr (N == 4) vidc::store_split4(img, row, ld, c, make_float4(a.v[0], a.v[1], a.v[2], a.v[3]));
    else {
#pragma unroll
        for (int i = 0; i < N; ++i) vidc::store_split(img, row, ld, c + i, a.v[i]);
    }
}

template <int M_> struct Wino;
template <> struct Wino<2> {
    static constexpr int A = 4;
    template <typename V> __device__ static __forceinline__ void bt(const V (&d)[4], V (&t)[4]) {
        t[0] = d[0] - d[2];
        t[1] = d[1] + d[2];
        t[2] = d[2] - d[1];
        t[3] = d[1] - d[3];
    }
    template <typename V> __device__ static __forceinline__ void at(const V (&m)[4], V (&o)[2]) {
        o[0] = (m[0] + m[1]) + m[2];
        o[1] = (m[1] - m[2]) - m[3];
    }
};
template <> struct Wino<4> {
    static constexpr int A = 6;
    template <typename V> __device__ static __forceinline__ void bt(const V (&d)[6], V (&t)[6]) {
        const V p = d[4] - 4.f * d[2], q = d[3] - 4.f * d[1];
        const V r = d[4] - d[2], s = 2.f * (d[3] - d[1]);
        t[0] = (4.f * d[0] - 5.f * d[2]) + d[4];
        t[1] = p + q;
        t[2] = p - q;
        t[3] = r + s;
        t[4] = r - s;
        t[5] = (4.f * d[1] - 5.f * d[3]) + d[5];
    }
    template <typename V> __device__ static __forceinline__ void at(const V (&m)[6], V (&o)[4]) {
        const V s12 = m[1] + m[2], d12 = m[1] - m[2], s34 = m[3] + m[4], d34 = m[3] - m[4];
        o[0] = (m[0] + s12) + s34;
        o[1] = d12 + 2.f * d34;
        o[2] = s12 + 4.f * s34;
        o[3] = (d12 + 8.f * d34) + m[5];
    }
};

__device__ __forceinline__ void band_block(unsigned& bx, unsigned& by) {
    const unsigned gx = gridDim.x, L = blockIdx.y * gx + blockIdx.x, per = (gx >> 3) * gridDim.y;
    const unsigned idx = (L & 7u) * per + (L >> 3);
    by = idx / gx;
    bx = idx - by * gx;
}

template <int M_, int N>
__global__ void __launch_bounds__(256)
wino_in_kernel(const float* __restrict__ x, float* __restrict__ v, unsigned short* __restrict__ vsp, int H, int W, int C, int ldx, int Cin,
               int th, int tw, int ldv) {
    constexpr int A = Wino<M_>::A;
    typedef vecn<N> V;
    const unsigned q = (unsigned)C / (unsigned)N;
    unsigned bx, by;
    band_block(bx, by);
    const unsigned i = bx * blockDim.x + threadIdx.x;
    if (i >= (unsigned)tw * q) return;
    const int tx = (int)(i / q);
    const int c = (int)(i - (unsigned)tx * q) * N;
    const int b = (int)(by / (unsigned)th), ty = (int)(by - (unsigned)b * (unsigned)th);
    const int iy0 = ty * M_ - 1, ix0 = tx * M_ - 1;
    V d[A][A];
#pragma unroll
    for (int r = 0; r < A; ++r) {
        const int iy = iy0 + r;
        const bool rok = (unsigned)iy < (unsigned)H;
#pragma unroll
        for (int s = 0; s < A; ++s) {
            const int ix = ix0 + s;
            d[r][s] = (rok && (unsigned)ix < (unsigned)W) ? vload<N>(&x[((size_t)(b * H + iy) * W + ix) * ldx + c]) : vzero<N>();
        }
    }
    V t[A][A];
#pragma unroll
    for (int s = 0; s < A; ++s) {
        V col[A], out[A];
#pragma unroll
        for (int r = 0; r < A; ++r) col[r] = d[r][s];
        Wino<M_>::bt(col, out);
#pragma unroll
        for (int r = 0; r < A; ++r) t[r][s] = out[r];
    }
    const int gg = c / Cin, cc = c - gg * Cin;
    const size_t tile = ((size_t)by) * tw + tx;
    const int ch0 = gg * (A * A) * Cin + cc;
#pragma unroll
    for (int r = 0; r < A; ++r) {
        V out[A];
        Wino<M_>::bt(t[r], out);
#pragma unroll
        for (int s = 0; s < A; ++s) {
            const int ch = ch0 + (r * A + s) * Cin;
            if (vsp) vstore_split<N>(vsp, tile, ldv, ch, out[s]);
            else vstore<N>(&v[tile * ldv + ch], out[s]);
        }
    }
}

template <int M_, int N>
__global__ void __launch_bounds__(256)
wino_out_kernel(const float* __restrict__ mm, float* __restrict__ y, unsigned short* __restrict__ ysp, const float* __restrict__ scale1,
                const float* __restrict__ shift1, const float* __restrict__ scale2, const float* __restrict__ shift2, int Ho, int Wo, int C,
                int Cout, int ldy, int th, int tw, int flags, int ldm) {
    constexpr int A = Wino<M_>::A;
    typedef vecn<N> V;
    const unsigned q = (unsigned)C / (unsigned)N;
    unsigned bx, by;
    band_block(bx, by);
    const unsigned i = bx * blockDim.x + threadIdx.x;
    if (i >= (unsigned)tw * q) return;
    const int tx = (int)(i / q);
    const int c = (int)(i - (unsigned)tx * q) * N;
    const int b = (int)(by / (unsigned)th), ty = (int)(by - (unsigned)b * (unsigned)th);
    const int gg = c / Cout, cc = c - gg * Cout;
    const size_t tile = ((size_t)by) * tw + tx;
    const float* src = mm + tile * ldm + gg * (A * A) * Cout + cc;
    V m[A][A];
#pragma unroll
    for (int r = 0; r < A; ++r)
#pragma unroll
        for (int s = 0; s < A; ++s) m[r][s] = vload<N>(&src[(r * A + s) * Cout]);
    V t[M_][A];
#pragma unroll
    for (int s = 0; s < A; ++s) {
        V col[A], out[M_];
#pragma unroll
        for (int r = 0; r < A; ++r) col[r] = m[r][s];
        Wino<M_>::at(col, out);
#pragma unroll
        for (int r = 0; r < M_; ++r) t[r][s] = out[r];
    }
    const V s1 = vload<N>(&scale1[c]), b1 = vload<N>(&shift1[c]);
    const float lo1 = (flags & VIDC_RELU1) ? 0.f : -INFINITY, lo2 = (flags & VIDC_RELU2) ? 0.f : -INFINITY;
    const bool aff2 = flags & VIDC_AFFINE2;
    V s2 = vzero<N>(), b2 = vzero<N>();
    if (aff2) { s2 = vload<N>(&scale2[c]); b2 = vload<N>(&shift2[c]); }
    const bool st_f32 = !(flags & VIDC_NO_F32_OUT);
#pragma unroll
    for (int r = 0; r < M_; ++r) {
        V out[M_];
        Wino<M_>::at(t[r], out);
        const int oy = ty * M_ + r;
        if (oy >= Ho) continue;
#pragma unroll
        for (int s = 0; s < M_; ++s) {
            const int ox = tx * M_ + s;
            if (ox >= Wo) continue;
            V o = out[s];
#pragma unroll
            for (int k = 0; k < N; ++k) o.v[k] = fmaxf(o.v[k] * s1.v[k] + b1.v[k], lo1);
            if (aff2) {
#pragma unroll
                for (int k = 0; k < N; ++k) o.v[k] = fmaxf(o.v[k] * s2.v[k] + b2.v[k], lo2);
            }
            const size_t row = (size_t)(b * Ho + oy) * Wo + ox;
            if (st_f32) vstore<N>(&y[row * ldy + c], o);
            if (ysp) vstore_split<N>(ysp, row, ldy, c, o);
        }
    }
}

template <int M_>
__global__ void __launch_bounds__(256)
wino_weight_kernel(const float* __restrict__ w, float* __restrict__ u, int Cout, int Cin) {
    constexpr int A = M_ + 2;
    const long long idx = (long long)blockIdx.x * blockDim.x + threadIdx.x;
    if (idx >= (long long)Cout * Cin) return;
    double G[A][3];
    if constexpr (M_ == 2) {
        const double g_[4][3] = {{1, 0, 0}, {.5, .5, .5}, {.5, -.5, .5}, {0, 0, 1}};
        for (int i = 0; i < A; ++i) for (int j = 0; j < 3; ++j) G[i][j] = g_[i][j];
    } else {
        const double g_[6][3] = {{1. / 4, 0, 0}, {-1. / 6, -1. / 6, -1. / 6}, {-1. / 6, 1. / 6, -1. / 6}, {1. / 24, 1. / 12, 1. / 6}, {1. / 24, -1. / 12, 1. / 6}, {0, 0, 1}};
        for (int i = 0; i < A; ++i) for (int j = 0; j < 3; ++j) G[i][j] = g_[i][j];
    }
    double g[3][3];
    for (int k = 0; k < 9; ++k) g[k / 3][k % 3] = (double)w[idx * 9 + k];
    double t[A][3];
    for (int i = 0; i < A; ++i)
        for (int j = 0; j < 3; ++j) t[i][j] = G[i][0] * g[0][j] + G[i][1] * g[1][j] + G[i][2] * g[2][j];
    for (int i = 0; i < A; ++i)
        for (int j = 0; j < A; ++j) {
            const double v = t[i][0] * G[j][0] + t[i][1] * G[j][1] + t[i][2] * G[j][2];
            u[(size_t)(i * A + j) * Cout * Cin + idx] = (float)v;
        }
}

}

extern "C" int vidc_winograd_tiles(int H, int W, int m, int* th, int* tw) {
    VIDC_REQUIRE(th && tw, VIDC_ERR_NULL, "vidc_winograd_tiles: null pointer");
    VIDC_REQUIRE((m == 2 || m == 4) && H > 0 && W > 0, VIDC_ERR_SHAPE, "vidc_winograd_tiles: m must be 2 or 4");
    *th = (H + m - 1) / m;
    *tw = (W + m - 1) / m;
    return VIDC_OK;
}

extern "C" int vidc_winograd_weight_transform(const float* w_oihw, float* u, int Cout, int Cin, int m, vidc_stream_t stream) {
    VIDC_REQUIRE(w_oihw && u, VIDC_ERR_NULL, "vidc_winograd_weight_transform: null pointer");
    VIDC_REQUIRE((m == 2 || m == 4) && Cout > 0 && Cin > 0, VIDC_ERR_SHAPE, "vidc_winograd_weight_transform: m must be 2 or 4");
    const unsigned blocks = (unsigned)(((long long)Cout * Cin + 255) / 256);
    if (m == 2) hipLaunchKernelGGL(wino_weight_kernel<2>, dim3(blocks), dim3(256), 0, vidc::as_stream(stream), w_oihw, u, Cout, Cin);
    else hipLaunchKernelGGL(wino_weight_kernel<4>, dim3(blocks), dim3(256), 0, vidc::as_stream(stream), w_oihw, u, Cout, Cin);
    VIDC_CHECK_LAUNCH("wino_weight_kernel");
    return VIDC_OK;
}

extern "C" int vidc_winograd_input_transform(const float* x, void* v, int B, int H, int W, int C, int ldx, int Cin, int m, int split,
                                             int ldv, vidc_stream_t stream) {
    VIDC_REQUIRE(x && v, VIDC_ERR_NULL, "vidc_winograd_input_transform: null pointer");
    VIDC_REQUIRE(m == 2 || m == 4, VIDC_ERR_SHAPE, "vidc_winograd_input_transform: m must be 2 or 4");
    VIDC_REQUIRE(B > 0 && H > 0 && W > 0 && C > 0 && Cin > 0 && C % Cin == 0 && Cin % 4 == 0 && ldx % 4 == 0 && ldx >= C, VIDC_ERR_SHAPE,
                 "vidc_winograd_input_transform: bad shape (C = G * Cin, Cin and ldx multiples of 4)");
    VIDC_REQUIRE(!split || Cin % 32 == 0, VIDC_ERR_SHAPE, "vidc_winograd_input_transform: split output needs Cin % 32 == 0");
    const int th = (H + m - 1) / m, tw = (W + m - 1) / m;
    if (ldv == 0) ldv = (m + 2) * (m + 2) * C;
    VIDC_REQUIRE(ldv >= (m + 2) * (m + 2) * C && ldv % 4 == 0 && (!split || ldv % 32 == 0), VIDC_ERR_SHAPE, "vidc_winograd_input_transform: bad row stride ldv = %d", ldv);
    VIDC_REQUIRE((long long)B * th <= 65535, VIDC_ERR_SHAPE, "vidc_winograd_input_transform: B * tile rows = %lld exceed the grid", (long long)B * th);
    const bool wide = (long long)B * th * tw * (C / 4) >= 131072;
    const int per = wide ? 4 : 1;
    const dim3 grid((unsigned)(vidc::cdiv(tw * (C / per), 256) + 7) / 8 * 8, (unsigned)(B * th));
    float* vf = split ? nullptr : reinterpret_cast<float*>(v);
    unsigned short* vs = split ? reinterpret_cast<unsigned short*>(v) : nullptr;
    hipStream_t st = vidc::as_stream(stream);
    if (m == 2 && wide) hipLaunchKernelGGL((wino_in_kernel<2, 4>), grid, dim3(256), 0, st, x, vf, vs, H, W, C, ldx, Cin, th, tw, ldv);
    else if (m == 2) hipLaunchKernelGGL((wino_in_kernel<2, 1>), grid, dim3(256), 0, st, x, vf, vs, H, W, C, ldx, Cin, th, tw, ldv);
    else if (wide) hipLaunchKernelGGL((wino_in_kernel<4, 4>), grid, dim3(256), 0, st, x, vf, vs, H, W, C, ldx, Cin, th, tw, ldv);
    else hipLaunchKernelGGL((wino_in_kernel<4, 1>), grid, dim3(256), 0, st, x, vf, vs, H, W, C, ldx, Cin, th, tw, ldv);
    VIDC_CHECK_LAUNCH("wino_in_kernel");
    return VIDC_OK;
}

extern "C" int vidc_winograd_output_transform(const float* mm, float* y, void* y_split, const float* scale1, const float* shift1,
                                              const float* scale2, const float* shift2, int B, int Ho, int Wo, int C, int Cout, int ldy,
                                              int m, int flags, int ldm, vidc_stream_t stream) {
    VIDC_REQUIRE(mm && scale1 && shift1 && (y || y_split), VIDC_ERR_NULL, "vidc_winograd_output_transform: null pointer");
    VIDC_REQUIRE(m == 2 || m == 4, VIDC_ERR_SHAPE, "vidc_winograd_output_transform: m must be 2 or 4");
    VIDC_REQUIRE(B > 0 && Ho > 0 && Wo > 0 && C > 0 && Cout > 0 && C % Cout == 0 && Cout % 4 == 0 && ldy % 4 == 0 && ldy >= C, VIDC_ERR_SHAPE,
                 "vidc_winograd_output_transform: bad shape (C = G * Cout, Cout and ldy multiples of 4)");
    VIDC_REQUIRE(!(flags & ~(VIDC_RELU1 | VIDC_AFFINE2 | VIDC_RELU2 | VIDC_SPLIT_OUT | VIDC_NO_F32_OUT)), VIDC_ERR_SHAPE,
                 "vidc_winograd_output_transform: unsupported flags 0x%x", flags);
    VIDC_REQUIRE(!(flags & VIDC_AFFINE2) || (scale2 && shift2), VIDC_ERR_NULL, "vidc_winograd_output_transform: AFFINE2 without scale2 / shift2");
    VIDC_REQUIRE(!!(flags & VIDC_SPLIT_OUT) == (y_split != nullptr), VIDC_ERR_SHAPE, "vidc_winograd_output_transform: SPLIT_OUT and y_split must come together");
    VIDC_REQUIRE(!(flags & VIDC_NO_F32_OUT) || y_split, VIDC_ERR_SHAPE, "vidc_winograd_output_transform: NO_F32_OUT without y_split writes nothing");
    VIDC_REQUIRE((flags & VIDC_NO_F32_OUT) || y, VIDC_ERR_NULL, "vidc_winograd_output_transform: y is NULL");
    VIDC_REQUIRE(!y_split || ldy % 32 == 0, VIDC_ERR_SHAPE, "vidc_winograd_output_transform: split output needs ldy % 32 == 0");
    const int th = (Ho + m - 1) / m, tw = (Wo + m - 1) / m;
    if (ldm == 0) ldm = (m + 2) * (m + 2) * C;
    VIDC_REQUIRE(ldm >= (m + 2) * (m + 2) * C && ldm % 4 == 0, VIDC_ERR_SHAPE, "vidc_winograd_output_transform: bad row stride ldm = %d", ldm);
    VIDC_REQUIRE((long long)B * th <= 65535, VIDC_ERR_SHAPE, "vidc_winograd_output_transform: B * tile rows = %lld exceed the grid", (long long)B * th);
    const bool wide = (long long)B * th * tw * (C / 4) >= 131072;
    const int per = wide ? 4 : 1;
    const dim3 grid((unsigned)(vidc::cdiv(tw * (C / per), 256) + 7) / 8 * 8, (unsigned)(B * th));
    unsigned short* ys = reinterpret_cast<unsigned short*>(y_split);
    hipStream_t st = vidc::as_stream(stream);
    if (m == 2 && wide) hipLaunchKernelGGL((wino_out_kernel<2, 4>), grid, dim3(256), 0, st, mm, y, ys, scale1, shift1, scale2, shift2, Ho, Wo, C, Cout, ldy, th, tw, flags, ldm);
    else if (m == 2) hipLaunchKernelGGL((wino_out_kernel<2, 1>), grid, dim3(256), 0, st, mm, y, ys, scale1, shift1, scale2, shift2, Ho, Wo, C, Cout, ldy, th, tw, flags, ldm);
    else if (wide) hipLaunchKernelGGL((wino_out_kernel<4, 4>), grid, dim3(256), 0, st, mm, y, ys, scale1, shift1, scale2, shift2, Ho, Wo, C, Cout, ldy, th, tw, flags, ldm);
    else hipLaunchKernelGGL((wino_out_kernel<4, 1>), grid, dim3(256), 0, st, mm, y, ys, scale1, shift1, scale2, shift2, Ho, Wo, C, Cout, ldy, th, tw, flags, ldm);
    VIDC_CHECK_LAUNCH("wino_out_kernel");
    return VIDC_OK;
}
```

vi_depth_completion_amd/engine.py:

```python
import collections
import ctypes as C
import json
import os

import torch

from . import _lib as L


class K(tuple):

    def __new__(cls, items):
        return super().__new__(cls, (items,) if isinstance(items, str) else tuple(items))

    def __add__(self, s):
        return K(p + s for p in self)


def _keys(k):
    return k if isinstance(k, K) else K(k)


class T:
    __slots__ = ("buf", "B", "H", "W", "C", "G", "ld", "ch_off", "nchw", "esz")

    def __init__(self, buf, B, H, W, Cc, G=1, ld=None, ch_off=0, nchw=False, esz=4):
        self.buf, self.B, self.H, self.W, self.C, self.G = buf, B, H, W, Cc, G
        self.ld = ld if ld is not None else G * Cc
        self.ch_off, self.nchw = ch_off, nchw
        self.esz = esz

    @property
    def numel(self):
        return self.B * self.H * self.W * self.ld


class WeightStore:

    def __init__(self, module):
        self.module = module
        self._cache = {}
        self._sd = None
        self._virtual = {}
        self.bn_eps = 1e-5

    def add_virtual(self, name, fn):
        if name not in self._virtual:
            self._virtual[name] = fn
            self._sd = None

    def invalidate(self):
        self._cache.clear()
        self._sd = None

    def sd(self):
        if self._sd is None:
            self._sd = {k: v.detach() for k, v in self.module.state_dict().items()}
            for name, fn in self._virtual.items():
                self._sd[name] = fn(self._sd)
        return self._sd

    def raw(self, key):
        return self.sd()[key]

    def packed(self, keys, dry_run=False, precision=0):
        ck = ("w", precision) + tuple(keys)
        if ck not in self._cache:
            ws = [self.sd()[k + ".weight"].contiguous() for k in keys]
            co, ci, kh, kw = ws[0].shape
            fmt = FORMATS[precision]
            out = torch.empty((len(ws), co, fmt.welems(kh * kw * ci)), dtype=torch.float32, device=ws[0].device)
            for g, w in enumerate(ws):
                assert tuple(w.shape) == (co, ci, kh, kw)
                if not dry_run:
                    L.check(getattr(L.lib(), fmt.pack)(L.ptr(w), L.ptr(out[g]), co, ci, kh, kw, L.current_stream()), "pack")
            if dry_run:
                return out
            self._cache[ck] = out
        return self._cache[ck]

    def packed_winograd(self, keys, m, dry_run=False, precision=0):
        ck = ("wino", m, precision) + tuple(keys)
        if ck not in self._cache:
            ws = [self.sd()[k + ".weight"].contiguous() for k in keys]
            co, ci, kh, kw = ws[0].shape
            assert (kh, kw) == (3, 3)
            a2 = (m + 2) * (m + 2)
            out = torch.empty((len(ws) * a2, co, ci), dtype=torch.float32, device=ws[0].device)
            if dry_run:
                return out
            for g, w in enumerate(ws):
                assert tuple(w.shape) == (co, ci, 3, 3)
                L.check(L.lib().vidc_winograd_weight_transform(L.ptr(w), L.ptr(out[g * a2]), co, ci, m, L.current_stream()), "winograd weights")
            if precision == L.PREC_BF16X3:
                img = torch.empty_like(out)
                L.check(L.lib().vidc_pack_conv_weight_bf16x3(L.ptr(out), L.ptr(img), len(ws) * a2 * co, ci, 1, 1, L.current_stream()), "pack")
                out = img
            self._cache[ck] = out
        return self._cache[ck]

    def packed_winograd_fused(self, keys, dry_run=False):
        ck = ("winof",) + tuple(keys)
        if ck not in self._cache:
            u = self.packed_winograd(keys, 4, dry_run, 0)
            out = torch.empty_like(u)
            if dry_run:
                return out
            co, ci = u.shape[1], u.shape[2]
            for g in range(len(keys)):
                L.check(L.lib().vidc_winograd_weight_pack_fused(L.ptr(u[g * 36]), L.ptr(out[g * 36]), co, ci, L.current_stream()), "winograd weights (fused order)")
            self._cache[ck] = out
        return self._cache[ck]

    def identity_affine(self, co, device):
        ck = ("id", co, str(device))
        if ck not in self._cache:
            self._cache[ck] = (torch.ones(co, dtype=torch.float32, device=device), torch.zeros(co, dtype=torch.float32, device=device))
        return self._cache[ck]

    def affine(self, conv_keys, bn_keys):
        ck = ("a",) + tuple(conv_keys) + tuple(bn_keys or ())
        if ck not in self._cache:
            sd = self.sd()
            scales, shifts = [], []
            for g, ckey in enumerate(conv_keys):
                co = sd[ckey + ".weight"].shape[0] if ckey is not None else sd[bn_keys[g] + ".weight"].shape[0]
                dev = sd[(ckey or bn_keys[g]) + ".weight"].device
                bias = sd.get(ckey + ".bias") if ckey is not None else None
                bias = bias.double() if bias is not None else torch.zeros(co, dtype=torch.float64, device=dev)
                if bn_keys is not None:
                    bn = bn_keys[g]
                    s = sd[bn + ".weight"].double() / torch.sqrt(sd[bn + ".running_var"].double() + self.bn_eps)
                    t = sd[bn + ".bias"].double() - sd[bn + ".running_mean"].double() * s + bias * s
                else:
                    s, t = torch.ones(co, dtype=torch.float64, device=dev), bias
                scales.append(s.float())
                shifts.append(t.float())
            self._cache[ck] = (torch.stack(scales).contiguous(), torch.stack(shifts).contiguous())
        return self._cache[ck]


class JointWeightStore(WeightStore):

    def __init__(self, modules):
        super().__init__(None)
        self.modules = dict(modules)

    def sd(self):
        if self._sd is None:
            self._sd = {"%s/%s" % (name, k): v.detach() for name, m in self.modules.items() for k, v in m.state_dict().items()}
            for name, fn in self._virtual.items():
                self._sd[name] = fn(self._sd)
        return self._sd


_TUNING = None


def tuning_table():
    global _TUNING
    if _TUNING is None:
        path = os.path.join(os.path.dirname(os.path.abspath(__file__)), "conv_tuning.json")
        _TUNING = json.load(open(path)) if os.path.exists(path) else {}
        if os.environ.get("VIDC_TUNING_OVERRIDE"):
            _TUNING = dict(_TUNING)
            _TUNING.update(json.loads(os.environ["VIDC_TUNING_OVERRIDE"]))
    return _TUNING


def precision_mode():
    return os.environ.get("VIDC_PRECISION", "mixed")


def default_precision(flops):
    return L.PREC_BF16X3 if flops >= 1.5e9 else L.PREC_FP32


MXFP8_MIN_FLOPS = 1e8
MXFP8_EXCLUDED = ("layer1.", "_upsamping.", "feature_concat.")


def mxfp8_layer(key, co, ci, flops):
    return ci % 128 == 0 and co % 32 == 0 and flops >= MXFP8_MIN_FLOPS and not any(e in key for e in MXFP8_EXCLUDED)


BF16_EXCLUDED = ()


def bf16_layer(key, co, ci, flops):
    return ci % 64 == 0 and co % 32 == 0 and not any(e in key for e in BF16_EXCLUDED)


def winograd_mode():
    return os.environ.get("VIDC_WINOGRAD", "auto")


def winograd_choice(B, H, W, co, ci, kh, kw, stride, padding, dilation, G, mode=None, precision=None, reduced=False):
    if reduced or (kh, kw, stride, padding, dilation) != (3, 3, 1, 1, 1) or ci % 32 or co % 32:
        return 0
    mode = mode if mode is not None else winograd_mode()
    precision = precision if precision is not None else precision_mode()
    if precision in ("mxfp8", "bf16"):
        precision = "mixed"
    if mode in ("0", "2", "4"):
        m = int(mode)
    else:
        ent = None
        for gg in (G, 4, 3, 1, 2):
            ent = tuning_table().get("W:" + conv_signature(L.conv_desc(B, H, W, ci, co, 3, 3, 1, 1, groups=gg)))
            if ent is not None:
                break
        if ent is not None:
            m = int(ent[1 if precision == "mixed" else 0]) if isinstance(ent, (list, tuple)) else int(ent)
            if m == 5 and gg != G:
                m = 4
        elif ci < 128 or precision == "mixed":
            m = 0
        else:
            m = 4 if min(H, W) >= 24 else 2
    if m:
        mt = 4 if m == 5 else m
        a2 = (mt + 2) * (mt + 2)
        tiles = B * (-(-H // mt)) * (-(-W // mt))
        if tiles * a2 * G * max(ci, co) * 4 >= 2 ** 31 or B * (-(-H // mt)) > 65535:
            return 0
    return m


def conv_signature(d):
    return "M%d_N%d_K%d_k%ds%d_G%d" % (d.B * d.Ho * d.Wo, d.Cout, d.KH * d.KW * d.Cin, d.KH, d.stride, d.groups)


Format = collections.namedtuple("Format", "name pack welems kind op unit esz elems sliceable folded out_flag out_key out_gs out_esz",
                                defaults=(None,) * 11)
FORMATS = {
    L.PREC_FP32: Format("fp32", "vidc_pack_conv_weight", lambda k: k),
    L.PREC_BF16X3: Format("bf16x3", "vidc_pack_conv_weight_bf16x3", lambda k: k,
                          kind="split", op=L.OP_SPLIT, unit=32, esz=4, elems=lambda rows, c, g: rows * c * g, sliceable=True, folded=True,
                          out_flag=L.SPLIT_OUT, out_key="split_out", out_gs=lambda d: d.y_gs, out_esz=4),
    L.PREC_MXFP8: Format("mxfp8", "vidc_pack_conv_weight_mxfp8", lambda k: k // 128 * 33,
                         kind="quant", op=L.OP_QUANT, unit=128, esz=4, elems=lambda rows, c, g: -(-g * rows * c * 33 // 128), sliceable=False,
                         folded=False, out_flag=L.MXFP8_OUT, out_key="mx_out", out_gs=lambda d: d.B * d.Ho * d.Wo * d.Cout * 33 // 128, out_esz=4),
    L.PREC_BF16: Format("bf16", "vidc_pack_conv_weight_bf16", lambda k: k // 2,
                        kind="cast", op=L.OP_CAST, unit=64, esz=2, elems=lambda rows, c, g: rows * c * g // 2, sliceable=True, folded=True,
                        out_flag=L.BF16_OUT, out_key="bf16_out", out_gs=lambda d: d.y_gs, out_esz=2),
}
IMAGE_FORMATS = {f.kind: f for f in FORMATS.values() if f.kind}
OP_KINDS = dict({"conv": L.OP_CONV, "stem": L.OP_STEM, "maxpool": L.OP_MAXPOOL, "upsample": L.OP_UPSAMPLE, "head": L.OP_HEAD,
                 "warp_params": L.OP_WARP_PARAMS, "warp_fwd": L.OP_WARP_FWD, "warp_inv": L.OP_WARP_INV, "avgpool": L.OP_AVGPOOL,
                 "normalize": L.OP_NORMALIZE, "det_im2col": L.OP_DET_IM2COL, "mask": L.OP_MASK, "wino_in": L.OP_WINO_IN,
                 "wino_out": L.OP_WINO_OUT, "nearest2x": L.OP_NEAREST2X, "copy": L.OP_COPY}, **{f.kind: f.op for f in IMAGE_FORMATS.values()})
MODE_LAYERS = {"mxfp8": (mxfp8_layer, L.PREC_MXFP8), "bf16": (bf16_layer, L.PREC_BF16)}


def _args(g, p=(), i=(), f=()):
    for arr, vals in ((g.p, p), (g.i, i), (g.f, f)):
        for j, v in enumerate(vals):
            arr[j] = v


class Program:

    def __init__(self, weights, device, batch, reuse_buffers=True, mode=None, winograd=None):
        self.ws, self.device, self.B = weights, device, batch
        self.ops = []
        self.buf_elems = []
        self.pinned = set()
        self.inputs, self.outputs = {}, {}
        self.reuse = reuse_buffers and os.environ.get("VIDC_NO_BUFFER_REUSE", "0") != "1"
        self.stream_id = 0
        self.wait_mask = 0
        self.handle = None
        self.flops = 0
        self.direct_flops = 0
        self.ref_flops = 0
        self._keep = []
        self._images = {}
        self.cuts = []
        self._cut_markers = []
        self.n_fused_splits = self.n_fused_quants = self.n_fused_casts = self.n_fused_warps = 0
        self.mode = mode if mode is not None else precision_mode()
        if self.mode not in ("fp32", "mixed", "mxfp8", "bf16"):
            raise ValueError("unknown precision mode %r (VIDC_PRECISION: fp32, mixed, mxfp8 or bf16)" % (self.mode,))
        self.winograd = winograd

    def _new_buf(self, elems, pinned=False):
        self.buf_elems.append(int(elems))
        if pinned:
            self.pinned.add(len(self.buf_elems) - 1)
        return len(self.buf_elems) - 1

    def input_nchw(self, name, Cc, H, W):
        t = T(self._new_buf(self.B * Cc * H * W, True), self.B, H, W, Cc, nchw=True)
        self.inputs[name] = t
        return t

    def input_raw(self, name, elems):
        t = T(self._new_buf(elems, True), 1, 1, 1, elems)
        self.inputs[name] = t
        return t

    def mark_output(self, name, t):
        self.pinned.add(t.buf)
        self.outputs[name] = t

    def nhwc(self, H, W, Cc, G=1):
        return T(self._new_buf(self.B * H * W * G * Cc), self.B, H, W, Cc, G)

    def cut(self):
        assert self.ops, "cut() before the first op"
        self._cut_markers.append(self.ops[-1])

    def on_stream(self, sid, wait_mask=0):
        self.stream_id, self.wait_mask = sid, wait_mask

    def _written(self, t):
        self._images = {k: v for k, v in self._images.items() if k[0] != t.buf}

    def _emit(self, kind, reads, writes, **kw):
        kw.update(stream_id=self.stream_id, wait_mask=self.wait_mask)
        self.wait_mask = 0
        self.ops.append((kind, [t.buf for t in reads if t is not None], [t.buf for t in writes], kw))

    def conv(self, x, key, bn=None, relu=False, stride=1, padding=0, bn2=None, relu2=False, residual=None,
             relu_after_residual=False, out=None, accumulate=False, ref_flops_scale=1.0, dilation=1):
        keys = _keys(key)
        G = len(keys)
        assert x.G == G and not x.nchw
        w0 = self.ws.raw(keys[0] + ".weight")
        co, ci, kh, kw = w0.shape
        assert ci == x.C, "conv %s expects Cin=%d, got %d" % (keys[0], ci, x.C)
        Ho = (x.H + 2 * padding - dilation * (kh - 1) - 1) // stride + 1
        Wo = (x.W + 2 * padding - dilation * (kw - 1) - 1) // stride + 1
        y = out if out is not None else self.nhwc(Ho, Wo, co, G)
        assert (y.H, y.W, y.C, y.G) == (Ho, Wo, co, G)
        self._written(y)
        flags = (L.RELU1 if relu else 0) | (L.AFFINE2 if bn2 is not None else 0) | (L.RELU2 if relu2 else 0)
        if residual is not None:
            assert (residual.H, residual.W, residual.C, residual.G) == (Ho, Wo, co, G)
            flags |= L.RESIDUAL | (L.RELU3 if relu_after_residual else 0)
        if accumulate:
            flags |= L.ACCUM
        flops = 2 * self.B * Ho * Wo * co * ci * kh * kw * G
        selects, reduced_prec = MODE_LAYERS.get(self.mode, (None, None))
        reduced = selects is not None and selects(keys[0], co, ci, flops)
        wm = 0
        if residual is None and not accumulate:
            wm = winograd_choice(self.B, x.H, x.W, co, ci, kh, kw, stride, padding, dilation, G, mode=self.winograd, precision=self.mode, reduced=reduced)
        if wm:
            self.ref_flops += int(round(flops * ref_flops_scale))
            self.direct_flops += flops
            knob = os.environ.get("VIDC_WINO_FUSED")
            fusable = self.mode == "fp32" and ci % 16 == 0 and not (flags & ~(L.RELU1 | L.AFFINE2 | L.RELU2))
            forced = (wm in (4, 5) and knob is not None and int(knob) > 0 and self.B * (-(-Ho // 4)) * (-(-Wo // 4)) <= int(knob)
                      and ci <= int(os.environ.get("VIDC_WINO_FUSED_MAXC", "256")))
            if fusable and (forced or (wm == 5 and knob is None)):
                return self._conv_winograd_fused(x, y, keys, bn, bn2, flags, (co, ci, Ho, Wo))
            return self._conv_winograd(x, y, keys, bn, bn2, flags, 4 if wm == 5 else wm, (co, ci, Ho, Wo))
        self.flops += flops
        self.direct_flops += flops
        self.ref_flops += int(round(flops * ref_flops_scale))
        sig = conv_signature(L.conv_desc(self.B, x.H, x.W, ci, co, kh, kw, stride, padding, dilation, G))
        prec = reduced_prec if reduced else self._table_precision(sig, flops)
        xin = self.image(x, prec) if FORMATS[prec].kind else x
        self._emit("conv", [xin, residual, y if accumulate else None], [y], x=xin, y=y, keys=keys, precision=prec,
                   bn=_keys(bn) if bn is not None else None, bn2=_keys(bn2) if bn2 is not None else None,
                   residual=residual, flags=flags, stride=stride, pad=padding, geom=(co, ci, kh, kw, Ho, Wo), dilation=dilation, sig=sig)
        return y

    def _conv_winograd(self, x, y, keys, bn, bn2, flags, m, geom):
        co, ci, Ho, Wo = geom
        G = len(keys)
        a2 = (m + 2) * (m + 2)
        tiles = self.B * (-(-Ho // m)) * (-(-Wo // m))
        gflops = 2 * tiles * a2 * G * co * ci
        self.flops += gflops
        sig = conv_signature(L.gemm_desc(tiles, ci, co, groups=a2 * G))
        prec = self._table_precision(sig, gflops)
        V = T(self._new_buf(tiles * a2 * G * ci), 1, 1, tiles, ci, a2 * G)
        Mm = T(self._new_buf(tiles * a2 * G * co), 1, 1, tiles, co, a2 * G)
        self._emit("wino_in", [x], [V], x=x, v=V, m=m, cin=ci, split=int(prec == L.PREC_BF16X3))
        self._emit("conv", [V], [Mm], x=V, y=Mm, keys=keys, precision=prec, bn=None, bn2=None, residual=None, flags=0, stride=1, pad=0,
                   geom=(co, ci, 1, 1, 1, tiles), dilation=1, wino=m, sig=sig)
        self._emit("wino_out", [Mm], [y], mm=Mm, y=y, keys=keys, bn=_keys(bn) if bn is not None else None,
                   bn2=_keys(bn2) if bn2 is not None else None, flags=flags, m=m, cout=co)
        return y

    def _conv_winograd_fused(self, x, y, keys, bn, bn2, flags, geom):
        co, ci, Ho, Wo = geom
        tiles = self.B * (-(-Ho // 4)) * (-(-Wo // 4))
        self.flops += 2 * tiles * 36 * len(keys) * co * ci
        self._emit("conv", [x], [y], x=x, y=y, keys=keys, precision=L.PREC_FP32, bn=_keys(bn) if bn is not None else None,
                   bn2=_keys(bn2) if bn2 is not None else None, residual=None, flags=flags, stride=1, pad=1, geom=(co, ci, 3, 3, Ho, Wo), dilation=1,
                   wino_fused=tiles, sig=conv_signature(L.gemm_desc(tiles, ci, co, groups=36 * len(keys))))
        return y

    def _table_precision(self, sig, flops):
        if self.mode == "fp32":
            return L.PREC_FP32
        ent = tuning_table().get(sig)
        return ent[2] if (ent is not None and len(ent) > 2) else default_precision(flops)

    def image(self, x, precision):
        fmt = FORMATS[precision]
        ch, planes = (x.C * x.G, 1) if fmt.folded else (x.C, x.G)
        ck = (x.buf, precision, x.ch_off, ch, planes)
        if ck not in self._images:
            assert not x.nchw and x.esz == 4 and ch % fmt.unit == 0
            if fmt.sliceable:
                for (b0, p0, off0, ch0, _), img in self._images.items():
                    if (b0, p0) == (x.buf, precision) and off0 <= x.ch_off and x.ch_off + ch <= off0 + ch0 and (x.ch_off - off0) % fmt.unit == 0:
                        return T(img.buf, x.B, x.H, x.W, x.C, x.G, ld=img.ld, ch_off=x.ch_off - off0, esz=fmt.esz)
            y = T(self._new_buf(fmt.elems(x.B * x.H * x.W, x.C, x.G)), x.B, x.H, x.W, x.C, x.G, ld=ch, esz=fmt.esz)
            self._emit(fmt.kind, [x], [y], x=x, y=y)
            self._images[ck] = y
        return T(self._images[ck].buf, x.B, x.H, x.W, x.C, x.G, ld=ch, esz=fmt.esz)

    def split(self, x):
        return self.image(x, L.PREC_BF16X3)

    def quant(self, x):
        return self.image(x, L.PREC_MXFP8)

    def cast(self, x):
        return self.image(x, L.PREC_BF16)

    def level_image(self, t):
        if self.mode == "bf16":
            if (t.C * t.G) % FORMATS[L.PREC_BF16].unit == 0:
                self.image(t, L.PREC_BF16)
        elif self.mode != "fp32":
            self.image(t, L.PREC_BF16X3)

# ... 82 lines not shown
        hp, wp = x.H + 2 * pad, x.W + 2 * pad
        low = T(self._new_buf(self.B * co * hp * wp), self.B, hp, wp, co, nchw=True)
        y = T(self._new_buf(self.B * co * out_size[0] * out_size[1]), self.B, out_size[0], out_size[1], co, nchw=True)
        self._emit("head", [x], [low, y], x=x, low=low, y=y, key=key, pad=pad, relu=relu)
        return y, low

    def warp_params(self, g, a, intr, kinv):
        p = T(self._new_buf(self.B * L.WARP_PARAMS), 1, 1, 1, self.B * L.WARP_PARAMS)
        self._emit("warp_params", [g, a, kinv], [p], g=g, a=a, kinv=kinv, p=p, intr=intr)
        return p

    def warp_fwd(self, x, params, intr, align_corners):
        y = T(self._new_buf(x.B * x.C * x.H * x.W), x.B, x.H, x.W, x.C, nchw=True)
        self._emit("warp_fwd", [x, params], [y], x=x, p=params, y=y, intr=intr, ac=int(align_corners))
        return y

    def warp_inv(self, x, params, intr, align_corners, normalize=True, out=None):
        y = out if out is not None else T(self._new_buf(x.B * 3 * x.H * x.W), x.B, x.H, x.W, 3, nchw=True)
        assert y.nchw and (y.B, y.C, y.H, y.W) == (x.B, 3, x.H, x.W)
        self._emit("warp_inv", [x, params], [y], x=x, p=params, y=y, intr=intr, ac=int(align_corners), norm=int(normalize))
        return y

    def copy(self, src, dst):
        self._emit("copy", [src], [dst], src=src, dst=dst)

    def _last_writer(self, i, buf):
        return next((t for t in range(i - 1, -1, -1) if buf in self.ops[t][2]), None)

    def _cut_between(self, marks, j, i):
        return any(id(self.ops[t]) in marks for t in range(j, i))

    def _attach(self, t, fmt, img):
        kind, _r, writes, kw = self.ops[t]
        kw[fmt.out_key] = img
        if kind in ("conv", "wino_out"):
            kw["flags"] |= fmt.out_flag
        writes.append(img.buf)

    def _fold_split(self, i, kw, marks):
        fmt, xs = IMAGE_FORMATS["split"], kw["x"]
        j = self._last_writer(i, xs.buf)
        if j is None or self.ops[j][0] not in ("conv", "maxpool", "upsample", "stem", "wino_out"):
            return False
        if self.ops[j][0] == "stem":
            y = self.ops[j][3]["y"]
            writers = [t for t in range(j + 1) if self.ops[t][0] == "stem" and self.ops[t][3]["y"].buf == y.buf]
            if xs.ch_off != 0 or xs.C * xs.G != y.C * y.G or y.ld != y.C * y.G or y.ld % fmt.unit or y.C % fmt.unit or \
                    any(self.ops[t][3].get(fmt.out_key) is not None for t in writers) or len(writers) != y.G:
                return False
            for t in writers:
                self._attach(t, fmt, kw["y"])
            return True
        last = {}
        foreign = False
        for t in range(i):
            if xs.buf in self.ops[t][2]:
                if self.ops[t][0] not in ("conv", "maxpool", "upsample", "wino_out"):
                    foreign = True
                    continue
                yt = self.ops[t][3]["y"]
                if yt.buf == xs.buf:
                    last[(yt.ch_off, yt.C * yt.G)] = t
        writers = sorted(last.values())
        lo, hi = xs.ch_off, xs.ch_off + xs.C * xs.G
        ok = bool(writers) and not foreign and xs.ld % fmt.unit == 0 and lo % fmt.unit == 0
        cover = []
        for t in writers:
            yt, pk = self.ops[t][3]["y"], self.ops[t][3]
            ok = ok and yt.ld == xs.ld and yt.ch_off % fmt.unit == 0 and (yt.C * yt.G) % fmt.unit == 0 and lo <= yt.ch_off and \
                yt.ch_off + yt.C * yt.G <= hi and pk.get(fmt.out_key) is None and \
                FORMATS[pk.get("precision", L.PREC_FP32)].out_key in (None, fmt.out_key)
            cover.append((yt.ch_off, yt.ch_off + yt.C * yt.G))
        cover.sort()
        ok = ok and cover[0][0] == lo and cover[-1][1] == hi and all(cover[k][1] == cover[k + 1][0] for k in range(len(cover) - 1))
        if not ok:
            return False
        simg = kw["y"]
        for t in writers:
            yt = self.ops[t][3]["y"]
            self._attach(t, fmt, T(simg.buf, yt.B, yt.H, yt.W, yt.C, yt.G, ld=simg.C * simg.G, ch_off=yt.ch_off - lo))
        return True

    def _fold_quant(self, i, kw, marks):
        fmt, xs = IMAGE_FORMATS["quant"], kw["x"]
        writers = [t for t in range(i) if xs.buf in self.ops[t][2]]
        if len(writers) != 1 or self.ops[writers[0]][0] != "conv":
            return False
        pk = self.ops[writers[0]][3]
        y = pk["y"]
        if FORMATS[pk["precision"]] is not fmt or pk.get(fmt.out_key) is not None or y.buf != xs.buf or \
                (y.ch_off, y.C, y.G, y.ld) != (xs.ch_off, xs.C, xs.G, xs.ld) or y.ch_off != 0 or y.ld != y.C * y.G:
            return False
        self._attach(writers[0], fmt, kw["y"])
        return True

    def _fold_cast(self, i, kw, marks):
        fmt, xs = IMAGE_FORMATS["cast"], kw["x"]
        j = self._last_writer(i, xs.buf)
        if j is None or self.ops[j][0] != "conv":
            return False
        pk = self.ops[j][3]
        y = pk["y"]
        if FORMATS[pk["precision"]] is not fmt or pk.get(fmt.out_key) is not None or pk.get("wino") or y.buf != xs.buf or \
                (y.ch_off, y.C * y.G, y.ld) != (xs.ch_off, xs.C * xs.G, xs.ld) or y.ch_off != 0 or y.ld != y.C * y.G or \
                (y.B, y.H, y.W) != (xs.B, xs.H, xs.W) or self._cut_between(marks, j, i):
            return False
        self._attach(j, fmt, kw["y"])
        return True

    def _fuse_images(self):
        marks = {id(mk) for mk in self._cut_markers}
        n = len(self.ops)
        order = list(IMAGE_FORMATS)
        drop = {}
        for i, (kind, _r, _w, kw) in enumerate(self.ops):
            if kind in IMAGE_FORMATS and getattr(self, "_fold_" + kind)(i, kw, marks):
                drop[i] = order.index(kind)
        for j, (kind, _r, _w, kw) in enumerate(self.ops):
            place = next((k for k, fmt in enumerate(IMAGE_FORMATS.values()) if kw.get(fmt.out_key) is not None), None)
            if place is None or kw["y"].buf in self.pinned:
                continue
            yb = kw["y"].buf
            if not any(yb in self.ops[t][1] and drop.get(t, len(order)) > place for t in range(j + 1, n)):
                if kind in ("conv", "wino_out"):
                    kw["flags"] |= L.NO_F32_OUT
                elif kind == "upsample":
                    kw["flags"] |= L.UP_NO_F32_OUT
                else:
                    kw["no_f32"] = True
        self.n_fused_splits, self.n_fused_quants, self.n_fused_casts = (sum(1 for v in drop.values() if v == k) for k in range(len(order)))
        self.ops = [op for i, op in enumerate(self.ops) if i not in drop]

    def _fuse_warp_into_stem(self):
        marks = {id(mk) for mk in self._cut_markers}
        drop = set()
        for i, (kind, reads, _w, kw) in enumerate(self.ops):
            if kind != "stem" or kw["x"].C != 3:
                continue
            xb = kw["x"].buf
            j = self._last_writer(i, xb)
            if j is None or self.ops[j][0] != "warp_fwd" or xb in self.pinned:
                continue
            if any(t != i and t not in drop and xb in self.ops[t][1] for t in range(len(self.ops))):
                continue
            if self._cut_between(marks, j, i):
                continue
            wkw = self.ops[j][3]
            kw["warp"] = {"x": wkw["x"], "p": wkw["p"], "intr": wkw["intr"], "ac": wkw["ac"]}
            self.ops[i] = (kind, [b for b in reads if b != xb] + [wkw["x"].buf, wkw["p"].buf], _w, kw)
            drop.add(j)
        self.ops = [op for t, op in enumerate(self.ops) if t not in drop]
        self.n_fused_warps = len(drop)

    def _conv_desc(self, kw, dry_run):
        x, y, keys, f = kw["x"], kw["y"], kw["keys"], kw["flags"]
        co, ci, kh, kwid, Ho, Wo = kw["geom"]
        prec, wm, wf, sig = kw["precision"], kw.get("wino", 0), kw.get("wino_fused", 0), kw["sig"]

        def addr(t):
            return self._addr(t) or None
        if wm:
            wp = self.ws.packed_winograd(list(keys), wm, dry_run, prec)
            s1, b1 = self.ws.identity_affine(co, wp.device)
            s2 = b2 = None
            d = L.gemm_desc(x.W, ci, co, groups=len(keys) * (wm + 2) * (wm + 2), ldx=x.ld, ldy=y.ld, precision=prec, x=addr(x),
                            w=wp.data_ptr(), y=addr(y), scale1=s1.data_ptr(), shift1=b1.data_ptr())
        else:
            wp = self.ws.packed_winograd_fused(list(keys), dry_run) if wf else self.ws.packed(list(keys), dry_run, prec)
            s1, b1 = self.ws.affine(list(keys), list(kw["bn"]) if kw["bn"] is not None else None)
            s2, b2 = self.ws.affine([None] * len(keys), list(kw["bn2"])) if kw["bn2"] is not None else (None, None)
            r = kw["residual"]
            d = L.conv_desc(x.B, x.H, x.W, ci, co, kh, kwid, kw["stride"], kw["pad"], kw["dilation"], len(keys), Ho, Wo, x.ld, y.ld, prec,
                            x=addr(x), w=wp.data_ptr(), y=addr(y), scale1=s1.data_ptr(), shift1=b1.data_ptr(),
                            scale2=s2.data_ptr() if s2 is not None else None, shift2=b2.data_ptr() if b2 is not None else None,
                            relu1=f & L.RELU1, relu2=f & L.RELU2, residual=addr(r), ldr=r.ld if r is not None else None,
                            relu3=f & L.RELU3, accumulate=f & L.ACCUM, no_f32_out=f & L.NO_F32_OUT, wino_fused=bool(wf),
                            **{fmt.out_key: addr(kw.get(fmt.out_key)) for fmt in IMAGE_FORMATS.values()})
        self._keep += [t for t in (wp, s1, b1, s2, b2) if t is not None]
        if prec == L.PREC_MXFP8:
            L.plan(d)
        elif prec == L.PREC_BF16:
            ent = tuning_table().get(sig)
            L.plan(d, (ent[0], ent[1]) if ent is not None and ent[0] in L.BF16_TILES else None)
        elif not wf:
            ent = tuning_table().get(sig)
            L.plan(d, None if ent is None else (ent[0], ent[1]) if len(ent) < 5 or prec == ent[2] else (ent[3], ent[4]))
        form = "@wino4f" if wf else ("@wino%d" % wm if wm else "")
        return d, "conv:%s%s:%s:sk%d:%s %s flags=0x%x" % (keys[0], form, L.TILE_NAMES[d.tile], d.splitk, FORMATS[prec].name, sig, d.flags)

    def _plan_buffers(self):
        n = len(self.buf_elems)
        multi_stream = any(kw["stream_id"] != 0 for _, _, _, kw in self.ops)
        storage = [None] * n
        if not self.reuse or multi_stream:
            for b in range(n):
                storage[b] = torch.zeros(max(self.buf_elems[b], 4), dtype=torch.float32, device=self.device)
            return storage
        last = [-1] * n
        first = [None] * n
        for i, (_, reads, writes, _) in enumerate(self.ops):
            for b in reads + writes:
                last[b] = i
                if first[b] is None:
                    first[b] = i
        free = []
        expire = {}
        for b in range(n):
            if b in self.pinned or first[b] is None:
                storage[b] = torch.zeros(max(self.buf_elems[b], 4), dtype=torch.float32, device=self.device)
            else:
                expire.setdefault(last[b], []).append(b)
        for i, (_, reads, writes, _) in enumerate(self.ops):
            for b in writes + reads:
                if storage[b] is None:
                    need = self.buf_elems[b]
                    best = None
                    for j, (el, _t) in enumerate(free):
                        if el >= need and (best is None or el < free[best][0]):
                            best = j
                    if best is not None:
                        storage[b] = free.pop(best)[1]
                    else:
                        storage[b] = torch.zeros(max(need, 4), dtype=torch.float32, device=self.device)
            for b in expire.get(i, []):
                free.append((storage[b].numel(), storage[b]))
        return storage

    def _addr(self, t, extra=0):
        return 0 if t is None else self.storage[t.buf].data_ptr() + t.esz * (t.ch_off + extra)

    def _lower_image(self, g, kw, fmt):
        x = kw["x"]
        rows, dims = x.B * x.H * x.W, ((x.C * x.G,) if fmt.folded else (x.C, x.G))
        _args(g, (self._addr(x), self._addr(kw["y"])), (rows & 0xFFFFFFFF, rows >> 32, dims[0], x.ld) + dims[1:])
        return "%s:%s" % (fmt.kind, "x".join("%d" % v for v in (rows,) + dims))

    def _lower_stem(self, g, kw):
        x, y, wf = kw["x"], kw["y"], kw.get("warp")
        w = self.ws.raw(kw["key"] + ".weight").contiguous()
        self._keep.append(w)
        _args(g, (self._addr(x), w.data_ptr(), 0 if kw.get("no_f32") else self._addr(y, kw["g"] * y.C), self._addr(kw.get("split_out"))),
              (x.B, x.C, x.H, x.W, y.C, y.ld, int(kw["relu"]), kw["g"] * y.C))
        if wf is not None:
            g.p[0], g.p[4] = self._addr(wf["x"]), self._addr(wf["p"])
            g.f[0], g.f[1], g.i[8] = wf["intr"].cx, wf["intr"].cy, wf["ac"]
        return "stem:" + kw["key"] + ("+warp" if wf is not None else "")

    def _lower_maxpool(self, g, kw):
        x, y = kw["x"], kw["y"]
        _args(g, (self._addr(x), 0 if kw.get("no_f32") else self._addr(y), self._addr(kw.get("split_out"))), (x.B, x.H, x.W, x.C * x.G, x.ld, y.ld))
        return "maxpool"

    def _lower_upsample(self, g, kw):
        x, y = kw["x"], kw["y"]
        _args(g, (self._addr(x), self._addr(y), self._addr(kw.get("split_out"))),
              (x.B, x.H, x.W, (x.C if kw.get("sum_groups") else x.C * x.G), x.ld, y.H, y.W, y.ld, kw["flags"]))
        return "upsample:%dx%dx%d->%dx%d" % (x.H, x.W, x.C * x.G, y.H, y.W)

    def _lower_head(self, g, kw):
        x, low, y = kw["x"], kw["low"], kw["y"]
        w = self.ws.raw(kw["key"] + ".weight").reshape(y.C, -1).contiguous()
        b = self.ws.raw(kw["key"] + ".bias").contiguous()
        self._keep += [w, b]
        _args(g, (self._addr(x), w.data_ptr(), b.data_ptr(), self._addr(low), self._addr(y)),
              (x.B, x.H, x.W, x.C * x.G, x.ld, y.C, kw["pad"], y.H, y.W, int(kw["relu"])))
        return "head:" + kw["key"]

    def _lower_warp_params(self, g, kw):
        it = kw["intr"]
        _args(g, [self._addr(kw[k]) for k in ("g", "a", "kinv", "p")], (self.B, it.W, it.H), (it.fx, it.fy, it.cx, it.cy))
        return "warp_params"

    def _lower_warp_fwd(self, g, kw):
        x, it = kw["x"], kw["intr"]
        _args(g, (self._addr(x), self._addr(kw["p"]), self._addr(kw["y"])), (x.B, x.C, x.H, x.W, kw["ac"]), (it.cx, it.cy))
        return "warp_fwd"

    def _lower_warp_inv(self, g, kw):
        x, it = kw["x"], kw["intr"]
        _args(g, (self._addr(x), self._addr(kw["p"]), self._addr(kw["y"])), (x.B, x.H, x.W, kw["ac"], kw["norm"]), (it.cx, it.cy))
        return "warp_inv_rot_norm"

    def _lower_avgpool(self, g, kw):
        x, y = kw["x"], kw["y"]
        _args(g, (self._addr(x), self._addr(y)), (x.B, x.H, x.W, x.C * x.G, x.ld) + tuple(kw["geom"]) + (y.ld,))
        return "avgpool"

    def _lower_normalize(self, g, kw):
        x = kw["x"]
        _args(g, (self._addr(x), self._addr(kw["y"])), (x.B, x.C, x.H * x.W))
        return "normalize"

    def _lower_det_im2col(self, g, kw):
        _args(g, (self._addr(kw["x"]), self._addr(kw["y"])), (kw["x"].B,) + tuple(kw["geom"]), kw["mean"])
        return "det_im2col"

    def _lower_mask(self, g, kw):
        x, y, im = kw["x"], kw["y"], kw["image"]
        _args(g, (self._addr(x), self._addr(im), self._addr(y)), (x.B, x.H, x.W, x.C * x.G, x.ld, y.ld, im.H, im.W))
        return "mask_scale"

    def _lower_wino_in(self, g, kw):
        x, v = kw["x"], kw["v"]
        _args(g, (self._addr(x), self._addr(v)), (x.B, x.H, x.W, x.C * x.G, x.ld, kw["cin"], kw["m"], kw["split"], v.ld))
        return "wino_in:F%d:%dx%dx%d" % (kw["m"], x.H, x.W, x.C * x.G)

    def _lower_wino_out(self, g, kw):
        mm, y, keys = kw["mm"], kw["y"], kw["keys"]
        s1, b1 = self.ws.affine(list(keys), list(kw["bn"]) if kw["bn"] is not None else None)
        s2, b2 = self.ws.affine([None] * len(keys), list(kw["bn2"])) if kw["bn2"] is not None else (None, None)
        self._keep += [t for t in (s1, b1, s2, b2) if t is not None]
        _args(g, (self._addr(mm), 0 if kw["flags"] & L.NO_F32_OUT else self._addr(y), self._addr(kw.get("split_out")), s1.data_ptr(), b1.data_ptr(),
                  L.ptr(s2) or 0, L.ptr(b2) or 0), (y.B, y.H, y.W, y.C * y.G, kw["cout"], y.ld, kw["m"], kw["flags"], mm.ld))
        return "wino_out:F%d:%dx%dx%d" % (kw["m"], y.H, y.W, y.C * y.G)

    def _lower_nearest2x(self, g, kw):
        x, y = kw["x"], kw["y"]
        _args(g, (self._addr(x), self._addr(y)), (x.B, x.H, x.W, x.C * x.G, x.ld, y.ld))
        return "nearest2x"

    def _lower_copy(self, g, kw):
        src, dst = kw["src"], kw["dst"]
        nbytes = min(self.buf_elems[src.buf], self.buf_elems[dst.buf]) * 4
        _args(g, (self._addr(src), self._addr(dst)), (nbytes & 0xFFFFFFFF, nbytes >> 32))
        return "copy"

    def finalize(self, dry_run=False):
        lib = L.lib()
        if os.environ.get("VIDC_FUSE_WARP", "0") == "1":
            self._fuse_warp_into_stem()
        if os.environ.get("VIDC_FUSE_SPLIT", "1") == "1":
            self._fuse_images()
        self.cuts = [next(i for i, op in enumerate(self.ops) if op is mk) + 1 for mk in self._cut_markers]
        assert len(self.cuts) < L.MAX_SEGMENTS and self.cuts == sorted(set(self.cuts))
        self.storage = self._plan_buffers()
        self.bytes_allocated = sum({t.data_ptr(): t.numel() * 4 for t in self.storage if t is not None}.values())
        ops = (L.Op * len(self.ops))()
        ws_need = {}
        ws_ops = []
        self.op_names = []
        for op, (kind, _r, _w, kw) in zip(ops, self.ops):
            if kind not in OP_KINDS:
                raise ValueError(kind)
            op.kind, op.stream_id, op.wait_mask = OP_KINDS[kind], kw["stream_id"], kw["wait_mask"]
            if kind == "conv":
                op.u.conv, name = self._conv_desc(kw, dry_run)
                need = lib.vidc_conv2d_workspace_bytes(C.byref(op.u.conv))
                if need:
                    ws_need[op.stream_id] = max(ws_need.get(op.stream_id, 0), need)
                    ws_ops.append(op)
            elif kind in IMAGE_FORMATS:
                name = self._lower_image(op.u.g, kw, IMAGE_FORMATS[kind])
            else:
                name = getattr(self, "_lower_" + kind)(op.u.g, kw)
            self.op_names.append(name)
        self.workspaces = {sid: torch.zeros(nb // 4 + 4, dtype=torch.float32, device=self.device) for sid, nb in ws_need.items()}
        for op in ws_ops:
            op.u.conv.workspace = self.workspaces[op.stream_id].data_ptr()
        self.c_ops = ops
        self.captured = False
        if dry_run:
            return self
        h = C.c_void_p()
        L.check(lib.vidc_program_create(ops, len(ops), C.byref(h)), "program_create")
        self.handle = h
        self.captured = False
        torch.cuda.current_stream(self.device).synchronize()
        return self

    def tensor(self, t):
        s = self.storage[t.buf]
        if t.nchw:
            return s[: t.B * t.C * t.H * t.W].view(t.B, t.C, t.H, t.W)
        return s[: t.B * t.H * t.W * t.ld].view(t.B, t.H, t.W, t.ld)[..., t.ch_off: t.ch_off + t.C * t.G]

    def run(self, stream=None):
        L.check(L.lib().vidc_program_run(self.handle, stream if stream is not None else L.current_stream()), "program_run")

    def capture(self, stream=None):
        L.check(L.lib().vidc_program_capture(self.handle, stream if stream is not None else L.current_stream()), "program_capture")
        self.captured = True

    def segments(self):
        edges = [0] + list(self.cuts) + [len(self.ops)]
        return [(edges[i], edges[i + 1]) for i in range(len(edges) - 1)]

    def run_segment(self, k, stream=None):
        b, e = self.segments()[k]
        L.check(L.lib().vidc_program_run_range(self.handle, stream if stream is not None else L.current_stream(), b, e), "program_run_range")

    def capture_segments(self, stream=None):
        st = stream if stream is not None else L.current_stream()
        for k, (b, e) in enumerate(self.segments()):
            L.check(L.lib().vidc_program_capture_range(self.handle, st, b, e, k), "program_capture_range")
        self.captured = True

    def launch_segment(self, k, stream=None):
        L.check(L.lib().vidc_program_launch_segment(self.handle, stream if stream is not None else L.current_stream(), k), "program_launch_segment")

    def launch(self, stream=None):
        L.check(L.lib().vidc_program_launch(self.handle, stream if stream is not None else L.current_stream()), "program_launch")

    def group_variant(self, name, segment, g_lo, g_hi, groups, keep_ungrouped):
        assert self.handle is not None and 0 <= g_lo < g_hi <= groups
        b, e = self.segments()[segment]
        picked = []
        for i in range(b, e):
            kind, _r, _w, kw = self.ops[i]
            if kind == "stem":
                if g_lo <= kw["g"] < g_hi:
                    picked.append(i)
                continue
            grouped = (kind in ("conv", "wino_out") and len(kw["keys"]) == groups) or (kind in ("maxpool", "wino_in") and kw["x"].G == groups)
            if grouped or keep_ungrouped or (kind in IMAGE_FORMATS and kw["x"].G == groups):
                picked.append(i)
        ops = (L.Op * len(picked))()
        for j, i in enumerate(picked):
            C.memmove(C.byref(ops[j]), C.byref(self.c_ops[i]), C.sizeof(L.Op))
            kind, _r, _w, kw = self.ops[i]
            if kind == "conv" and len(kw["keys"]) == groups:
                d = ops[j].u.conv
                a2 = (kw["wino"] + 2) ** 2 if kw.get("wino") else 1
                strides = [("x", d.x_gs, 4), ("w", d.w_gs, 4), ("y", d.y_gs, 4), ("scale1", d.p_gs, 4), ("shift1", d.p_gs, 4), ("scale2", d.p_gs, 4),
                           ("shift2", d.p_gs, 4), ("residual", d.r_gs, 4)]
                strides += [("y_split", fmt.out_gs(d), fmt.out_esz) for fmt in IMAGE_FORMATS.values() if d.flags & fmt.out_flag]
                for field, gs, esz in strides:
                    v = getattr(d, field)
                    if v:
                        setattr(d, field, v + esz * g_lo * gs * a2)
                d.groups = (g_hi - g_lo) * a2
            elif kind == "wino_in" and kw["x"].G == groups:
                g = ops[j].u.g
                cin, a2 = kw["cin"], (kw["m"] + 2) ** 2
                g.p[0], g.p[1] = g.p[0] + 4 * g_lo * cin, g.p[1] + 4 * g_lo * a2 * cin
                g.i[3] = cin * (g_hi - g_lo)
            elif kind == "wino_out" and len(kw["keys"]) == groups:
                g = ops[j].u.g
                co, a2 = kw["cout"], (kw["m"] + 2) ** 2
                g.p[0] = g.p[0] + 4 * g_lo * a2 * co
                for k in (1, 2, 3, 4, 5, 6):
                    if g.p[k]:
                        g.p[k] = g.p[k] + 4 * g_lo * co
                g.i[3] = co * (g_hi - g_lo)
            elif kind == "maxpool" and kw["x"].G == groups:
                g = ops[j].u.g
                cg = kw["x"].C
                for k in range(3):
                    if g.p[k]:
                        g.p[k] = g.p[k] + 4 * g_lo * cg
                g.i[3] = cg * (g_hi - g_lo)
        h = C.c_void_p()
        L.check(L.lib().vidc_program_create(ops, len(ops), C.byref(h)), "program_create (variant)")
        self._variants = getattr(self, "_variants", {})
        self._variants[name] = {"handle": h, "ops": ops, "captured": False, "indices": picked}
        return self._variants[name]

    def has_variant(self, name):
        return name in getattr(self, "_variants", {})

    def run_variant(self, name, stream=None):
        L.check(L.lib().vidc_program_run(self._variants[name]["handle"], stream if stream is not None else L.current_stream()), "variant_run")

    def capture_variant(self, name, stream=None):
        v = self._variants[name]
        L.check(L.lib().vidc_program_capture(v["handle"], stream if stream is not None else L.current_stream()), "variant_capture")
        v["captured"] = True

    def launch_variant(self, name, stream=None):
        v = self._variants[name]
        st = stream if stream is not None else L.current_stream()
        if v["captured"]:
            L.check(L.lib().vidc_program_launch(v["handle"], st), "variant_launch")
        else:
            L.check(L.lib().vidc_program_run(v["handle"], st), "variant_run")

    def time(self, iters=20, use_graph=False, per_op=False, stream=None):
        ms = (C.c_float * 1)()
        per = (C.c_float * len(self.ops))() if per_op else None
        L.check(L.lib().vidc_program_time(self.handle, stream if stream is not None else L.current_stream(), iters,
                                          int(use_graph), ms, per), "program_time")
        return (ms[0], list(per)) if per_op else ms[0]

    def __del__(self):
        try:
            if self.handle is not None:
                L.lib().vidc_program_destroy(self.handle)
            for v in getattr(self, "_variants", {}).values():
                L.lib().vidc_program_destroy(v["handle"])
        except Exception:
            pass
```

vi_depth_completion_amd/ops.py:

```python
import ctypes as C

import torch

from . import _lib as L


def _dev(*ts):
    for t in ts:
        if t is not None and not t.is_cuda:
            raise RuntimeError("vidc ops take GPU tensors only (no CPU fallback)")


def pack_conv_weight(w_oihw):
    _dev(w_oihw)
    w = w_oihw.contiguous().float()
    co, ci, kh, kw = w.shape
    out = torch.empty((co, kh * kw * ci), dtype=torch.float32, device=w.device)
    L.check(L.lib().vidc_pack_conv_weight(L.ptr(w), L.ptr(out), co, ci, kh, kw, L.current_stream()), "pack_conv_weight")
    return out


def pack_conv_weight_bf16x3(w_oihw):
    _dev(w_oihw)
    w = w_oihw.contiguous().float()
# ... 69 lines not shown
        assert wp.dtype == torch.bfloat16 and wp.numel() == G * cout * kh * kw * cin
    elif precision == L.PREC_MXFP8:
        wp = w_packed.contiguous()
        cout = wp.numel() // G // (kh * kw * cin // 32 * 33)
        assert wp.numel() == G * cout * kh * kw * cin // 32 * 33
    else:
        wp = w_packed.contiguous().view(G, -1, kh * kw * cin)
        cout = wp.shape[1]
    Ho, Wo = (H + 2 * pad - dilation * (kh - 1) - 1) // stride + 1, (W + 2 * pad - dilation * (kw - 1) - 1) // stride + 1
    y = accumulate_into if accumulate_into is not None else torch.empty((B, Ho, Wo, G * cout), dtype=torch.float32, device=x.device)
    s1, b1 = scale1.contiguous().float(), shift1.contiguous().float()
    s2, b2 = (scale2.contiguous().float(), shift2.contiguous().float()) if scale2 is not None else (None, None)
    residual = residual.contiguous() if residual is not None else None
    if mx_out is not None:
        assert mx_out.dtype == torch.uint8 and mx_out.numel() >= G * B * Ho * Wo * cout // 32 * 33
    if bf16_out is not None:
        assert bf16_out.dtype == torch.bfloat16 and bf16_out.is_contiguous() and bf16_out.numel() >= B * Ho * Wo * G * cout
    d = L.conv_desc(B, H, W, cin, cout, kh, kw, stride, pad, dilation, G, Ho, Wo, precision=precision, x=L.ptr(x), w=L.ptr(wp), y=L.ptr(y),
                    scale1=L.ptr(s1), shift1=L.ptr(b1), shared_affine=s1.numel() < G * cout, scale2=L.ptr(s2), shift2=L.ptr(b2),
                    relu1=relu1, relu2=relu2, residual=L.ptr(residual), ldr=residual.shape[-1] if residual is not None else None, relu3=relu3,
                    accumulate=accumulate_into is not None, split_out=L.ptr(split_out), mx_out=L.ptr(mx_out), no_f32_out=no_f32_out,
                    bf16_out=L.ptr(bf16_out))
    _launch(d, x.device, tile, splitk, workspace, "conv2d_bn_act")
    return y


def _launch(d, device, tile, splitk, workspace, what):
    L.plan(d, (tile, splitk) if tile else None)
    if not tile and splitk > 1:
        d.splitk = splitk
    ws = None
    nbytes = L.lib().vidc_conv2d_workspace_bytes(C.byref(d))
    if nbytes and workspace is not None:
        if workspace.numel() * 4 < nbytes:
            raise RuntimeError("split-K workspace too small: %d < %d bytes" % (workspace.numel() * 4, nbytes))
        d.workspace = L.ptr(workspace)
    elif nbytes:
        ws = torch.zeros(nbytes // 4, dtype=torch.float32, device=device)
        d.workspace = L.ptr(ws)
    L.check(L.lib().vidc_conv2d_bn_act(C.byref(d), L.current_stream()), what)


def stem_conv3x3s2(x_nchw, w_oihw, relu=True, split_out=None):
    _dev(x_nchw, w_oihw)
    x, w = x_nchw.contiguous().float(), w_oihw.contiguous().float()
    B, cin, H, W = x.shape
    co = w.shape[0]
    Ho, Wo = (H + 2 - 3) // 2 + 1, (W + 2 - 3) // 2 + 1
    y = torch.empty((B, Ho, Wo, co), dtype=torch.float32, device=x.device)
    L.check(L.lib().vidc_stem_conv3x3s2(L.ptr(x), L.ptr(w), L.ptr(y), B, cin, H, W, co, co, int(relu), L.ptr(split_out), 0,
                                        L.current_stream()), "stem")
    return y


def stem_conv3x3s2_warped(x_nchw, warp_params, w_oihw, cx, cy, align_corners=False, relu=True):
    _dev(x_nchw, warp_params, w_oihw)
    x, w = x_nchw.contiguous().float(), w_oihw.contiguous().float()
    B, cin, H, W = x.shape
    assert cin == 3
    co = w.shape[0]
    Ho, Wo = (H + 2 - 3) // 2 + 1, (W + 2 - 3) // 2 + 1
    y = torch.empty((B, Ho, Wo, co), dtype=torch.float32, device=x.device)
    L.check(L.lib().vidc_stem_conv3x3s2_warped(L.ptr(x), L.ptr(warp_params), L.ptr(w), L.ptr(y), B, H, W, co, co, int(relu), None, 0, float(cx), float(cy),
                                               int(align_corners), L.current_stream()), "stem (warped input)")
    return y


def maxpool3x3s2(x, split_out=None):
    _dev(x)
    x = x.contiguous()
    B, H, W, Cc = x.shape
    Ho, Wo = (H + 2 - 3) // 2 + 1, (W + 2 - 3) // 2 + 1
    y = torch.empty((B, Ho, Wo, Cc), dtype=torch.float32, device=x.device)
    L.check(L.lib().vidc_maxpool3x3s2(L.ptr(x), L.ptr(y), B, H, W, Cc, Cc, Cc, L.ptr(split_out), L.current_stream()), "maxpool")
    return y


def upsample_bilinear_ac(x, size, relu=False, accumulate_into=None, split_out=None, store_f32=True, sum_groups=1):
    _dev(x)
    x = x.contiguous()
    B, h, w, Cc = x.shape
    if sum_groups > 1:
        assert accumulate_into is not None and Cc % sum_groups == 0
        y = accumulate_into
        co = Cc // sum_groups
        flags = (L.UP_RELU if relu else 0) | L.UP_ACCUM | (sum_groups << 8)
        L.check(L.lib().vidc_upsample_bilinear_ac(L.ptr(x), L.ptr(y), B, h, w, co, Cc, size[0], size[1], co, flags, L.ptr(split_out),
                                                  L.current_stream()), "upsample")
        return y
    y = accumulate_into if accumulate_into is not None else torch.empty((B, size[0], size[1], Cc), dtype=torch.float32, device=x.device)
    flags = (L.UP_RELU if relu else 0) | (L.UP_ACCUM if accumulate_into is not None else 0) | (0 if store_f32 else L.UP_NO_F32_OUT)
    L.check(L.lib().vidc_upsample_bilinear_ac(L.ptr(x), L.ptr(y), B, h, w, Cc, Cc, size[0], size[1], Cc, flags, L.ptr(split_out),
                                              L.current_stream()), "upsample")
    return y


def head_conv1x1_upsample(x, w, bias, pad, size, relu):
    _dev(x, w, bias)
    x = x.contiguous()
    B, h, wd, cin = x.shape
    w2 = w.reshape(w.shape[0], -1).contiguous().float()
    co = w2.shape[0]
    low = torch.empty((B, co, h + 2 * pad, wd + 2 * pad), dtype=torch.float32, device=x.device)
    y = torch.empty((B, co, size[0], size[1]), dtype=torch.float32, device=x.device)
    b = bias.contiguous().float()
    L.check(L.lib().vidc_head_conv1x1_upsample(L.ptr(x), L.ptr(w2), L.ptr(b), L.ptr(low), L.ptr(y), B, h, wd, cin, cin, co, pad,
                                               size[0], size[1], int(relu), L.current_stream()), "head")
    return y, low


def winograd_weight_transform(w_oihw, m):
    _dev(w_oihw)
    w = w_oihw.contiguous().float()
    co, ci, kh, kw = w.shape
    assert (kh, kw) == (3, 3)
    a2 = (m + 2) * (m + 2)
    u = torch.empty((a2, co, ci), dtype=torch.float32, device=w.device)
    L.check(L.lib().vidc_winograd_weight_transform(L.ptr(w), L.ptr(u), co, ci, m, L.current_stream()), "winograd_weight_transform")
    return u


def winograd_input_transform(x, cin, m, split=False):
    _dev(x)
    x = x.contiguous()
    B, H, W, Cc = x.shape
    th, tw = -(-H // m), -(-W // m)
    a2 = (m + 2) * (m + 2)
    v = torch.empty((B * th * tw, a2 * Cc), dtype=torch.float32, device=x.device)
    L.check(L.lib().vidc_winograd_input_transform(L.ptr(x), L.ptr(v), B, H, W, Cc, Cc, cin, m, int(split), 0, L.current_stream()),
            "winograd_input_transform")
    return v


def winograd_output_transform(mm, B, Ho, Wo, cout, m, scale1, shift1, relu1=False, scale2=None, shift2=None, relu2=False, split_out=None,
                              no_f32_out=False):
    _dev(mm, scale1, shift1)
    mm = mm.contiguous()
    a2 = (m + 2) * (m + 2)
    Cc = mm.shape[1] // a2
    y = torch.empty((B, Ho, Wo, Cc), dtype=torch.float32, device=mm.device)
    s1, b1 = scale1.contiguous().float().view(-1), shift1.contiguous().float().view(-1)
    flags = (L.RELU1 if relu1 else 0)
    s2 = b2 = None
    if scale2 is not None:
        s2, b2 = scale2.contiguous().float().view(-1), shift2.contiguous().float().view(-1)
        flags |= L.AFFINE2 | (L.RELU2 if relu2 else 0)
    if split_out is not None:
        flags |= L.SPLIT_OUT | (L.NO_F32_OUT if no_f32_out else 0)
    L.check(L.lib().vidc_winograd_output_transform(L.ptr(mm), L.ptr(y), L.ptr(split_out), L.ptr(s1), L.ptr(b1), L.ptr(s2), L.ptr(b2), B, Ho, Wo,
                                                   Cc, cout, Cc, m, flags, 0, L.current_stream()), "winograd_output_transform")
    return y


def conv3x3_winograd(x, w_oihw_groups, scale1, shift1, m, relu1=False, scale2=None, shift2=None, relu2=False, precision=0, tile=0, splitk=1,
                     split_out=None, no_f32_out=False):
    if precision not in (L.PREC_FP32, L.PREC_BF16X3):
        raise RuntimeError("conv3x3_winograd: precision %d has no Winograd form (fp32 = 0 and bf16x3 = 1 only; plain bf16 and MXFP8 run the direct "
                           "conv: the transforms amplify their rounding)" % precision)
    G = len(w_oihw_groups)
    B, H, W, Cc = x.shape
    cin = Cc // G
    cout = w_oihw_groups[0].shape[0]
    a2 = (m + 2) * (m + 2)
    u = torch.cat([winograd_weight_transform(w, m) for w in w_oihw_groups], 0)
    if precision == L.PREC_BF16X3:
        img = torch.empty_like(u)
        L.check(L.lib().vidc_pack_conv_weight_bf16x3(L.ptr(u), L.ptr(img), G * a2 * cout, cin, 1, 1, L.current_stream()), "pack")
        u = img
    v = winograd_input_transform(x, cin, m, split=precision == L.PREC_BF16X3)
    tiles = v.shape[0]
    mm = torch.empty((tiles, a2 * G * cout), dtype=torch.float32, device=x.device)
    one, zero = torch.ones(cout, dtype=torch.float32, device=x.device), torch.zeros(cout, dtype=torch.float32, device=x.device)
    d = L.gemm_desc(tiles, cin, cout, groups=a2 * G, precision=precision, x=L.ptr(v), w=L.ptr(u), y=L.ptr(mm), scale1=L.ptr(one), shift1=L.ptr(zero))
    _launch(d, x.device, tile, splitk, None, "conv2d_bn_act (winograd GEMMs)")
    return winograd_output_transform(mm, B, H, W, cout, m, scale1, shift1, relu1, scale2, shift2, relu2, split_out, no_f32_out)


def winograd_weight_pack_fused(u):
    _dev(u)
    u = u.contiguous().float()
    a2, co, ci = u.shape
    assert a2 == 36
    out = torch.empty_like(u)
    L.check(L.lib().vidc_winograd_weight_pack_fused(L.ptr(u), L.ptr(out), co, ci, L.current_stream()), "winograd_weight_pack_fused")
    return out


def conv3x3_winograd_fused(x, w_oihw_groups, scale1, shift1, relu1=False, scale2=None, shift2=None, relu2=False, u=None):
    _dev(x, scale1, shift1)
    x = x.contiguous()
    G = len(w_oihw_groups) if u is None else u.shape[0] // 36
    B, H, W, Cc = x.shape
    cin = Cc // G
    if u is None:
        u = torch.cat([winograd_weight_pack_fused(winograd_weight_transform(w, 4)) for w in w_oihw_groups], 0)
    cout = u.shape[1]
    y = torch.empty((B, H, W, G * cout), dtype=torch.float32, device=x.device)
    s1, b1 = scale1.contiguous().float().view(-1), shift1.contiguous().float().view(-1)
    s2, b2 = (scale2.contiguous().float().view(-1), shift2.contiguous().float().view(-1)) if scale2 is not None else (None, None)
    d = L.conv_desc(B, H, W, cin, cout, 3, 3, 1, 1, groups=G, x=L.ptr(x), w=L.ptr(u), y=L.ptr(y), scale1=L.ptr(s1), shift1=L.ptr(b1),
                    shared_affine=s1.numel() < G * cout, scale2=L.ptr(s2), shift2=L.ptr(b2), relu1=relu1, relu2=relu2, wino_fused=True)
    L.check(L.lib().vidc_conv2d_bn_act(C.byref(d), L.current_stream()), "conv2d_bn_act (fused Winograd)")
    return y


def clock_stamps(n, device=None):
    return torch.zeros((n, L.CLOCK_STAMP_WGS, 4), dtype=torch.int64, device=device if device is not None else "cuda")


def clock_stamp(stamps, i):
    if not stamps.is_cuda or stamps.dtype != torch.int64 or tuple(stamps.shape[1:]) != (L.CLOCK_STAMP_WGS, 4) or not stamps.is_contiguous():
        raise RuntimeError("clock_stamp: a buffer made by ops.clock_stamps is required")
    L.check(L.lib().vidc_clock_stamp(stamps.data_ptr() + 8 * 4 * L.CLOCK_STAMP_WGS * int(i), L.current_stream()), "clock_stamp")


def shader_clock_ghz(stamps, a, b):
    h = stamps.cpu()
    sa = {int(r[0]): (int(r[1]), int(r[2])) for r in h[a] if int(r[3]) == 1}
    sb = {int(r[0]): (int(r[1]), int(r[2])) for r in h[b] if int(r[3]) == 1}
    ghz = sorted((sb[x][0] - sa[x][0]) / (sb[x][1] - sa[x][1]) * 0.1 for x in sa if x in sb and sb[x][1] > sa[x][1] and sb[x][0] > sa[x][0])
    return ghz[len(ghz) // 2] if ghz else None


def _scratch(nbytes, device):
    return torch.empty(int(nbytes) + 256, dtype=torch.uint8, device=device)


def warp2dof_fwd_backward(dy, params, cx, cy, align_corners):
    _dev(dy, params)
    dy = dy.contiguous().float()
    B, Cc, H, W = dy.shape
    dx = torch.empty_like(dy)
    L.check(L.lib().vidc_warp2dof_fwd_backward(L.ptr(dy), L.ptr(params), L.ptr(dx), B, Cc, H, W, float(cx), float(cy), int(align_corners),
                                               L.current_stream()), "warp2dof_fwd_backward")
    return dx


def warp2dof_inv_rot_norm_backward(x, dz, params, cx, cy, align_corners, normalize):
    _dev(x, dz, params)
    x, dz = x.contiguous().float(), dz.contiguous().float()
    B, _c, H, W = x.shape
    dx = torch.empty_like(x)
    L.check(L.lib().vidc_warp2dof_inv_rot_norm_backward(L.ptr(x), L.ptr(dz), L.ptr(params), L.ptr(dx), B, H, W, float(cx), float(cy),
                                                        int(align_corners), int(normalize), L.current_stream()), "warp2dof_inv_rot_norm_backward")
    return dx


def affine_act_backward(dy, y, scale, shift, relu, c_raw=None, all_from_raw=False):
    _dev(dy, y, scale, shift, c_raw)
    dy, y = dy.contiguous().float(), y.contiguous()
    Cc = y.shape[-1]
    M = y.numel() // Cc
    s, b = scale.contiguous().float(), shift.contiguous().float()
    c_raw = c_raw.contiguous() if c_raw is not None else None
    dc = torch.empty_like(y)
    dscale, dshift = torch.empty_like(s), torch.empty_like(b)
    sc = _scratch(L.lib().vidc_train_scratch_bytes(M, Cc), y.device)
    L.check(L.lib().vidc_affine_act_backward(L.ptr(dy), L.ptr(y), L.ptr(c_raw), L.ptr(s), L.ptr(b), L.ptr(dc), L.ptr(dscale), L.ptr(dshift), M, Cc,
                                             Cc, Cc, -Cc if (all_from_raw and c_raw is not None) else Cc, Cc, int(relu), L.ptr(sc), L.current_stream()),
            "affine_act_backward")
    return dc, dscale, dshift


def pack_conv_weight_dgrad(w_oihw, precision=0):
    _dev(w_oihw)
    w = w_oihw.contiguous().float()
    co, ci, kh, kw = w.shape
    out = torch.empty((ci, kh * kw * co), dtype=torch.float32, device=w.device)
    if precision == L.PREC_FP32:
        L.check(L.lib().vidc_pack_conv_weight_dgrad(L.ptr(w), L.ptr(out), co, ci, kh, kw, L.current_stream()), "pack_conv_weight_dgrad")
        return out
    if precision != L.PREC_BF16X3:
        raise RuntimeError("pack_conv_weight_dgrad: precision %d has no data-gradient form" % precision)
    kind = 3
    nb = L.lib().vidc_pack_item_blocks(co, ci, kh, kw, kind)
    if nb <= 0:
        raise RuntimeError("conv weight %dx%dx%dx%d cannot be packed for the bf16x3 data gradient (Cout a multiple of 32, kernels up to 3x3)" % (co, ci, kh, kw))
    item = (L.PackItem * 1)()
    item[0].w, item[0].packed, item[0].Cout, item[0].Cin, item[0].KH, item[0].KW, item[0].kind, item[0].block_begin = L.ptr(w), L.ptr(out), co, ci, kh, kw, kind, 0
    dev = torch.frombuffer(bytearray(bytes(item)), dtype=torch.uint8).to(w.device)
    L.check(L.lib().vidc_pack_conv_weights_batched(L.ptr(dev), 1, nb, L.current_stream()), "pack_conv_weights_batched")
    return out


def conv_backward_data(dc, w_oihw, H, W, stride, pad, precision=0, dilation=1):
    _dev(dc, w_oihw)
    dc = dc.contiguous()
    co, ci, kh, kw = w_oihw.shape
    B, Ho, Wo, _c = dc.shape
    if dilation != 1:
        if dilation < 1 or stride != 1 or kh != kw or dilation * (kh - 1) - pad < 0:
            raise RuntimeError("conv data gradient: unsupported geometry %dx%d stride %d pad %d dilation %d (a dilated conv must have stride 1, a square "
                               "kernel and pad <= dilation * (k-1))" % (kh, kw, stride, pad, dilation))
        if (Ho, Wo) != (H + 2 * pad - dilation * (kh - 1), W + 2 * pad - dilation * (kw - 1)):
            raise RuntimeError("conv data gradient: dc is %dx%d, a %dx%d conv of dilation %d and pad %d over %dx%d gives %dx%d"
                               % (Ho, Wo, kh, kw, dilation, pad, H, W, H + 2 * pad - dilation * (kh - 1), W + 2 * pad - dilation * (kw - 1)))
        one, zero = torch.ones(ci, dtype=torch.float32, device=dc.device), torch.zeros(ci, dtype=torch.float32, device=dc.device)
        return conv2d_bn_act(dc, pack_conv_weight_dgrad(w_oihw, precision), one, zero, kh, kw, stride=1, pad=dilation * (kh - 1) - pad, precision=precision,
                             dilation=dilation)
    if kh != kw or kh - 1 - pad < 0 or (stride > 1 and 2 * pad > kh - 1):
        raise RuntimeError("conv data gradient: unsupported geometry %dx%d stride %d pad %d (square kernels, pad <= k-1, and pad <= (k-1)/2 when strided)"
                           % (kh, kw, stride, pad))
    wd = pack_conv_weight_dgrad(w_oihw, precision)
    g = dc
    if stride > 1:
        g = torch.empty((B, H, W, co), dtype=torch.float32, device=dc.device)
# ... 132 lines not shown
```

Measured before the change: 636.5.

## Fuse stem conv into Winograd input transform and maxpool into output transform

```diff
diff --git a/include/vidc.h b/include/vidc.h
--- a/include/vidc.h
+++ b/include/vidc.h
@@ -136,6 +136,11 @@
 int vidc_winograd_output_transform(const float* mm, float* y, void* y_split, const float* scale1, const float* shift1,
                                    const float* scale2, const float* shift2, int B, int Ho, int Wo, int C, int Cout, int ldy, int m,
                                    int flags, int ldm, vidc_stream_t stream);
+int vidc_winograd_input_transform_stem(const float* const* x, const int* cin, const float* w_packed, float* v, int B, int H, int W, int Cout,
+                                       int G, int g_lo, int g_hi, int relu, int ldv, vidc_stream_t stream);
+int vidc_winograd_output_transform_maxpool(const float* mm, float* y, const float* scale1, const float* shift1, const float* scale2,
+                                           const float* shift2, int B, int Ho, int Wo, int C, int Cout, int ldy, int flags, int ldm,
+                                           vidc_stream_t stream);
 
 int vidc_stem_conv3x3s2(const float* x, const float* w_oihw, float* y, int B, int Cin, int H, int W, int Cout, int ldy,
                         int relu, void* y_split, int split_ch0, vidc_stream_t stream);
@@ -349,7 +354,9 @@
                     VIDC_OP_WINO_IN = 17  ,
                     VIDC_OP_WINO_OUT = 18 ,
                     VIDC_OP_QUANT = 19    ,
-                    VIDC_OP_CAST = 20      };
+                    VIDC_OP_CAST = 20     ,
+                    VIDC_OP_WINO_IN_STEM = 21  ,
+                    VIDC_OP_WINO_OUT_POOL = 22  };
 
 typedef struct vidc_generic_args {
     const void* p[8];
diff --git a/vi_depth_completion_amd/_lib.py b/vi_depth_completion_amd/_lib.py
--- a/vi_depth_completion_amd/_lib.py
+++ b/vi_depth_completion_amd/_lib.py
@@ -15,7 +15,7 @@
 
 RELU1, AFFINE2, RELU2, RESIDUAL, RELU3, ACCUM, SPLIT_OUT, NO_F32_OUT, STATS_OUT, X_PLANAR_GROUPS, MXFP8_OUT, BF16_OUT = 1, 2, 4, 8, 16, 32, 64, 128, 256, 512, 1024, 2048
 UP_RELU, UP_ACCUM, UP_NO_F32_OUT = 1, 2, 4
-OP_CONV, OP_STEM, OP_MAXPOOL, OP_UPSAMPLE, OP_HEAD, OP_WARP_PARAMS, OP_WARP_FWD, OP_WARP_INV, OP_COPY, OP_SPLIT, OP_AVGPOOL, OP_NORMALIZE, OP_DET_IM2COL, OP_NEAREST2X, _OP_RETIRED_15, OP_MASK, OP_WINO_IN, OP_WINO_OUT, OP_QUANT, OP_CAST = range(1, 21)
+OP_CONV, OP_STEM, OP_MAXPOOL, OP_UPSAMPLE, OP_HEAD, OP_WARP_PARAMS, OP_WARP_FWD, OP_WARP_INV, OP_COPY, OP_SPLIT, OP_AVGPOOL, OP_NORMALIZE, OP_DET_IM2COL, OP_NEAREST2X, _OP_RETIRED_15, OP_MASK, OP_WINO_IN, OP_WINO_OUT, OP_QUANT, OP_CAST, OP_WINO_IN_STEM, OP_WINO_OUT_POOL = range(1, 23)
 TILE_AUTO = 0
 PREC_FP32, PREC_BF16X3, PREC_BF16, PREC_MXFP8 = 0, 1, 2, 3
 TILE_KIND_AUTO, TILE_KIND_MFMA, TILE_KIND_STREAM, TILE_KIND_WINOGRAD = range(4)
@@ -182,6 +182,8 @@
     "vidc_winograd_weight_pack_fused": (C.c_int, [_vp, _vp, _i, _i, _vp]),
     "vidc_winograd_input_transform": (C.c_int, [_vp, _vp, _i, _i, _i, _i, _i, _i, _i, _i, _i, _vp]),
     "vidc_winograd_output_transform": (C.c_int, [_vp, _vp, _vp, _vp, _vp, _vp, _vp, _i, _i, _i, _i, _i, _i, _i, _i, _i, _vp]),
+    "vidc_winograd_input_transform_stem": (C.c_int, [C.POINTER(_vp), C.POINTER(C.c_int), _vp, _vp, _i, _i, _i, _i, _i, _i, _i, _i, _i, _vp]),
+    "vidc_winograd_output_transform_maxpool": (C.c_int, [_vp, _vp, _vp, _vp, _vp, _vp, _i, _i, _i, _i, _i, _i, _i, _i, _vp]),
     "vidc_stem_conv3x3s2": (C.c_int, [_vp, _vp, _vp, _i, _i, _i, _i, _i, _i, _i, _vp, _i, _vp]),
     "vidc_stem_conv3x3s2_warped": (C.c_int, [_vp, _vp, _vp, _vp, _i, _i, _i, _i, _i, _i, _vp, _i, _f, _f, _i, _vp]),
     "vidc_maxpool3x3s2": (C.c_int, [_vp, _vp, _i, _i, _i, _i, _i, _i, _vp, _vp]),
diff --git a/vi_depth_completion_amd/csrc/common.h b/vi_depth_completion_amd/csrc/common.h
--- a/vi_depth_completion_amd/csrc/common.h
+++ b/vi_depth_completion_amd/csrc/common.h
@@ -37,6 +37,8 @@
     } while (0)
 
 __host__ __device__ inline int cdiv(int a, int b) { return (a + b - 1) / b; }
+
+__device__ __forceinline__ float stem_mac(float acc, float p, float w) { return fmaf(w, p, acc); }
 
 constexpr int TT = 256;
 inline unsigned blocks(long long n) { return (unsigned)((n + TT - 1) / TT); }
diff --git a/vi_depth_completion_amd/csrc/pointwise.hip b/vi_depth_completion_amd/csrc/pointwise.hip
--- a/vi_depth_completion_amd/csrc/pointwise.hip
+++ b/vi_depth_completion_amd/csrc/pointwise.hip
@@ -72,7 +72,7 @@
 #pragma unroll
                 for (int r = 0; r < 3; ++r)
 #pragma unroll
-                    for (int s = 0; s < 3; ++s) acc += patch[c][r][2 * p + s] * wr[(c * 3 + r) * 3 + s];
+                    for (int s = 0; s < 3; ++s) acc = vidc::stem_mac(acc, patch[c][r][2 * p + s], wr[(c * 3 + r) * 3 + s]);
             if (relu) acc = fmaxf(acc, 0.f);
             const size_t row = (size_t)(b * Ho + oy) * Wo + ox;
             if (y) y[row * ldy + c_out] = acc;
diff --git a/vi_depth_completion_amd/csrc/program.hip b/vi_depth_completion_amd/csrc/program.hip
--- a/vi_depth_completion_amd/csrc/program.hip
+++ b/vi_depth_completion_amd/csrc/program.hip
@@ -67,6 +67,15 @@
             return vidc_winograd_output_transform((const float*)g.p[0], (float*)g.p[1], const_cast<void*>(g.p[2]), (const float*)g.p[3],
                                                   (const float*)g.p[4], (const float*)g.p[5], (const float*)g.p[6], g.i[0], g.i[1], g.i[2], g.i[3],
                                                   g.i[4], g.i[5], g.i[6], g.i[7], g.i[8], s);
+        case VIDC_OP_WINO_IN_STEM: {
+            const float* xs[4] = {(const float*)g.p[0], (const float*)g.p[1], (const float*)g.p[2], (const float*)g.p[3]};
+            return vidc_winograd_input_transform_stem(xs, &g.i[9], (const float*)g.p[4], (float*)const_cast<void*>(g.p[5]), g.i[0], g.i[1], g.i[2], g.i[3],
+                                                      g.i[4], g.i[5], g.i[6], g.i[7], g.i[8], s);
+        }
+        case VIDC_OP_WINO_OUT_POOL:
+            return vidc_winograd_output_transform_maxpool((const float*)g.p[0], (float*)g.p[1], (const float*)g.p[3], (const float*)g.p[4],
+                                                          (const float*)g.p[5], (const float*)g.p[6], g.i[0], g.i[1], g.i[2], g.i[3], g.i[4], g.i[5],
+                                                          g.i[7], g.i[8], s);
         case VIDC_OP_QUANT: {
             long long rows = (long long)(uint32_t)g.i[0] | ((long long)(uint32_t)g.i[1] << 32);
             return vidc_quant_mxfp8((const float*)g.p[0], const_cast<void*>(g.p[1]), rows, g.i[2], g.i[3], g.i[4], s);
diff --git a/vi_depth_completion_amd/csrc/winograd.hip b/vi_depth_completion_amd/csrc/winograd.hip
--- a/vi_depth_completion_amd/csrc/winograd.hip
+++ b/vi_depth_completion_amd/csrc/winograd.hip
@@ -36,6 +36,9 @@
     if constexpr (N == 4) {
         const float4 t = *reinterpret_cast<const float4*>(p);
         r.v[0] = t.x; r.v[1] = t.y; r.v[2] = t.z; r.v[3] = t.w;
+    } else if constexpr (N == 2) {
+        const float2 t = *reinterpret_cast<const float2*>(p);
+        r.v[0] = t.x; r.v[1] = t.y;
     } else {
 #pragma unroll
         for (int i = 0; i < N; ++i) r.v[i] = p[i];
@@ -44,6 +47,7 @@
 }
 template <int N> __device__ __forceinline__ void vstore(float* p, const vecn<N>& a) {
     if constexpr (N == 4) *reinterpret_cast<float4*>(p) = make_float4(a.v[0], a.v[1], a.v[2], a.v[3]);
+    else if constexpr (N == 2) *reinterpret_cast<float2*>(p) = make_float2(a.v[0], a.v[1]);
     else {
 #pragma unroll
         for (int i = 0; i < N; ++i) p[i] = a.v[i];
@@ -211,6 +215,205 @@
             if (st_f32) vstore<N>(&y[row * ldy + c], o);
             if (ysp) vstore_split<N>(ysp, row, ldy, c, o);
         }
+    }
+}
+
+constexpr int kStemTiles = 4;
+constexpr int kStemPW = 8 * kStemTiles + 5;
+constexpr int kStemPitch = 40;
+struct StemGroups {
+    const float* x[4];
+    int cin[4];
+};
+
+template <int CIN>
+__device__ __forceinline__ void wino_in_stem_body(const float* __restrict__ x, const float* __restrict__ wpk, float* __restrict__ v,
+                                                  float (*patch)[13][kStemPitch], int H, int W, int Ho, int Wo, int Cout, int gg, int cb, int th,
+                                                  int tw, int ldv, int relu) {
+    const int b = (int)(blockIdx.y / (unsigned)th), ty = (int)(blockIdx.y - (unsigned)b * (unsigned)th);
+    const int tx0 = blockIdx.x * kStemTiles;
+    const int tid = threadIdx.x, tl = tid >> 6, lane = tid & 63;
+    const int iy_base = 8 * ty - 3, ix_base = 8 * tx0 - 3;
+    const float* xb = x + (size_t)b * CIN * H * W;
+    for (int e = tid; e < CIN * 13 * kStemPW; e += 256) {
+        const int c = e / (13 * kStemPW), rem = e - c * (13 * kStemPW), r = rem / kStemPW, i = rem - r * kStemPW;
+        const int iy = iy_base + r, ix = ix_base + i;
+        float val = 0.f;
+        if ((unsigned)iy < (unsigned)H && (unsigned)ix < (unsigned)W) val = xb[((size_t)c * H + iy) * W + ix];
+        patch[c][r][i] = val;
+    }
+    __syncthreads();
+    const int tx = tx0 + tl;
+    if (tx >= tw) return;
+    const int c = cb * 64 + lane;
+    float wr[CIN * 9];
+#pragma unroll
+    for (int k = 0; k < CIN * 9; ++k) wr[k] = wpk[((size_t)gg * Cout + c) * 27 + k];
+    float d[6][6];
+#pragma unroll
+    for (int pr = 0; pr < 6; ++pr) {
+        float acc[6];
+#pragma unroll
+        for (int ps = 0; ps < 6; ++ps) acc[ps] = 0.f;
+#pragma unroll
+        for (int cc = 0; cc < CIN; ++cc)
+#pragma unroll
+            for (int r = 0; r < 3; ++r) {
+                float seg[13];
+#pragma unroll
+                for (int i = 0; i < 13; ++i) seg[i] = patch[cc][2 * pr + r][8 * tl + i];
+#pragma unroll
+                for (int s = 0; s < 3; ++s)
+#pragma unroll
+                    for (int ps = 0; ps < 6; ++ps) acc[ps] = vidc::stem_mac(acc[ps], seg[2 * ps + s], wr[(cc * 3 + r) * 3 + s]);
+            }
+        const int iy = ty * 4 - 1 + pr;
+#pragma unroll
+        for (int ps = 0; ps < 6; ++ps) {
+            const int ix = tx * 4 - 1 + ps;
+            const float val = relu ? fmaxf(acc[ps], 0.f) : acc[ps];
+            d[pr][ps] = ((unsigned)iy < (unsigned)Ho && (unsigned)ix < (unsigned)Wo) ? val : 0.f;
+        }
+    }
+    float t[6][6];
+#pragma unroll
+    for (int s = 0; s < 6; ++s) {
+        float col[6], out[6];
+#pragma unroll
+        for (int r = 0; r < 6; ++r) col[r] = d[r][s];
+        Wino<4>::bt(col, out);
+#pragma unroll
+        for (int r = 0; r < 6; ++r) t[r][s] = out[r];
+    }
+    float* dst = v + ((size_t)blockIdx.y * tw + tx) * ldv + (size_t)gg * 36 * Cout + c;
+#pragma unroll
+    for (int r = 0; r < 6; ++r) {
+        float out[6];
+        Wino<4>::bt(t[r], out);
+#pragma unroll
+        for (int s = 0; s < 6; ++s) dst[(r * 6 + s) * Cout] = out[s];
+    }
+}
+
+__global__ void __launch_bounds__(256)
+wino_in_stem_kernel(StemGroups gr, const float* __restrict__ wpk, float* __restrict__ v, int H, int W, int Ho, int Wo, int Cout, int g_lo,
+                    int th, int tw, int ldv, int relu) {
+    __shared__ __attribute__((aligned(16))) float patch[3][13][kStemPitch];
+    const int cbs = Cout >> 6;
+    const int gl = (int)blockIdx.z / cbs, gg = g_lo + gl, cb = (int)blockIdx.z - gl * cbs;
+    const float* x = gg == 0 ? gr.x[0] : gg == 1 ? gr.x[1] : gg == 2 ? gr.x[2] : gr.x[3];
+    const int cin = gg == 0 ? gr.cin[0] : gg == 1 ? gr.cin[1] : gg == 2 ? gr.cin[2] : gr.cin[3];
+    if (cin == 3) wino_in_stem_body<3>(x, wpk, v, patch, H, W, Ho, Wo, Cout, gg, cb, th, tw, ldv, relu);
+    else wino_in_stem_body<1>(x, wpk, v, patch, H, W, Ho, Wo, Cout, gg, cb, th, tw, ldv, relu);
+}
+
+constexpr int kPoolCols = 12;
+constexpr int kPoolSlice = 64;
+template <int N>
+__global__ void __launch_bounds__(kPoolCols * kPoolSlice / N)
+wino_out_pool_kernel(const float* __restrict__ mm, float* __restrict__ y, const float* __restrict__ scale1, const float* __restrict__ shift1,
+                     const float* __restrict__ scale2, const float* __restrict__ shift2, int Ho, int Wo, int Hp, int Wp, int C, int Cout, int ldy,
+                     int th, int tw, int flags, int ldm, int slices, int seg_rows) {
+    typedef vecn<N> V;
+    constexpr int kPoolLanes = kPoolSlice / N;
+    __shared__ __attribute__((aligned(16))) float edge[2][kPoolCols][5][kPoolSlice];
+    const int lane = threadIdx.x % kPoolLanes, slot = threadIdx.x / kPoolLanes;
+    const int strip = (int)blockIdx.x / slices, slice = (int)blockIdx.x - strip * slices;
+    const int tx = strip * (kPoolCols - 1) - 1 + slot;
+    const int c = slice * kPoolSlice + lane * N;
+    const int b = blockIdx.z;
+    const int ty0 = (int)blockIdx.y * seg_rows, ty1 = min(th, ty0 + seg_rows);
+    const bool live = tx >= 0 && tx < tw && c < C;
+    const int cl = live ? c : 0;
+    const int gg = cl / Cout, cc = cl - gg * Cout;
+    const V s1 = vload<N>(&scale1[cl]), b1 = vload<N>(&shift1[cl]);
+    const float lo1 = (flags & VIDC_RELU1) ? 0.f : -INFINITY, lo2 = (flags & VIDC_RELU2) ? 0.f : -INFINITY;
+    const bool aff2 = flags & VIDC_AFFINE2;
+    V s2 = vzero<N>(), b2 = vzero<N>();
+    if (aff2) { s2 = vload<N>(&scale2[cl]); b2 = vload<N>(&shift2[cl]); }
+    V ninf;
+#pragma unroll
+    for (int k = 0; k < N; ++k) ninf.v[k] = -INFINITY;
+    V carry[4];
+#pragma unroll
+    for (int s = 0; s < 4; ++s) carry[s] = ninf;
+    for (int ty = ty0 > 0 ? ty0 - 1 : 0; ty < ty1; ++ty) {
+        V o[4][4];
+#pragma unroll
+        for (int r = 0; r < 4; ++r)
+#pragma unroll
+            for (int s = 0; s < 4; ++s) o[r][s] = ninf;
+        if (live) {
+            const unsigned off = (unsigned)((((size_t)b * th + ty) * tw + tx) * ldm + gg * 36 * Cout + cc);
+            V m[6][6];
+#pragma unroll
+            for (int r = 0; r < 6; ++r)
+#pragma unroll
+                for (int s = 0; s < 6; ++s) m[r][s] = vload<N>(mm + (size_t)((r * 6 + s) * Cout) + off);
+            V t[4][6];
+#pragma unroll
+            for (int s = 0; s < 6; ++s) {
+                V col[6], out[4];
+#pragma unroll
+                for (int r = 0; r < 6; ++r) col[r] = m[r][s];
+                Wino<4>::at(col, out);
+#pragma unroll
+                for (int r = 0; r < 4; ++r) t[r][s] = out[r];
+            }
+#pragma unroll
+            for (int r = 0; r < 4; ++r) {
+                V out[4];
+                Wino<4>::at(t[r], out);
+                const bool rok = ty * 4 + r < Ho;
+#pragma unroll
+                for (int s = 0; s < 4; ++s) {
+                    V q = out[s];
+#pragma unroll
+                    for (int k = 0; k < N; ++k) q.v[k] = fmaxf(q.v[k] * s1.v[k] + b1.v[k], lo1);
+                    if (aff2) {
+#pragma unroll
+                        for (int k = 0; k < N; ++k) q.v[k] = fmaxf(q.v[k] * s2.v[k] + b2.v[k], lo2);
+                    }
+                    if (rok && tx * 4 + s < Wo) o[r][s] = q;
+                }
+            }
+        }
+        float(*e)[kPoolSlice] = edge[ty & 1][slot];
+        vstore<N>(&e[0][lane * N], carry[3]);
+#pragma unroll
+        for (int r = 0; r < 4; ++r) vstore<N>(&e[1 + r][lane * N], o[r][3]);
+        __syncthreads();
+        if (live && slot > 0 && ty >= ty0) {
+            V l[5];
+#pragma unroll
+            for (int k = 0; k < 5; ++k) l[k] = tx > 0 ? vload<N>(&edge[ty & 1][slot - 1][k][lane * N]) : ninf;
+#pragma unroll
+            for (int j = 0; j < 2; ++j) {
+                const int py = 2 * ty + j;
+                if (py >= Hp) continue;
+                V cm[5];
+#pragma unroll
+                for (int k = 0; k < N; ++k) {
+                    cm[0].v[k] = fmaxf(fmaxf(l[2 * j].v[k], l[2 * j + 1].v[k]), l[2 * j + 2].v[k]);
+#pragma unroll
+                    for (int s = 0; s < 4; ++s) {
+                        const float top = j == 0 ? carry[s].v[k] : o[1][s].v[k];
+                        cm[1 + s].v[k] = fmaxf(fmaxf(top, o[2 * j][s].v[k]), o[2 * j + 1][s].v[k]);
+                    }
+                }
+#pragma unroll
+                for (int i = 0; i < 2; ++i) {
+                    const int px = 2 * tx + i;
+                    if (px >= Wp) continue;
+                    V p;
+#pragma unroll
+                    for (int k = 0; k < N; ++k) p.v[k] = fmaxf(fmaxf(cm[2 * i].v[k], cm[2 * i + 1].v[k]), cm[2 * i + 2].v[k]);
+                    vstore<N>(&y[((size_t)(b * Hp + py) * Wp + px) * ldy + c], p);
+                }
+            }
+        }
+#pragma unroll
+        for (int s = 0; s < 4; ++s) carry[s] = o[3][s];
     }
 }
 
@@ -315,3 +518,57 @@
     VIDC_CHECK_LAUNCH("wino_out_kernel");
     return VIDC_OK;
 }
+
+extern "C" int vidc_winograd_input_transform_stem(const float* const* x, const int* cin, const float* w_packed, float* v, int B, int H, int W,
+                                                  int Cout, int G, int g_lo, int g_hi, int relu, int ldv, vidc_stream_t stream) {
+    VIDC_REQUIRE(x && cin && w_packed && v, VIDC_ERR_NULL, "vidc_winograd_input_transform_stem: null pointer");
+    VIDC_REQUIRE(G >= 1 && G <= 4 && 0 <= g_lo && g_lo < g_hi && g_hi <= G, VIDC_ERR_SHAPE,
+                 "vidc_winograd_input_transform_stem: groups [%d, %d) of %d (at most 4)", g_lo, g_hi, G);
+    VIDC_REQUIRE(B > 0 && H > 2 && W > 2 && Cout > 0 && Cout % 64 == 0, VIDC_ERR_SHAPE,
+                 "vidc_winograd_input_transform_stem: bad shape (Cout must be a multiple of 64)");
+    StemGroups gr = {};
+    for (int g = g_lo; g < g_hi; ++g) {
+        VIDC_REQUIRE(x[g], VIDC_ERR_NULL, "vidc_winograd_input_transform_stem: null image of group %d", g);
+        VIDC_REQUIRE(cin[g] == 1 || cin[g] == 3, VIDC_ERR_SHAPE, "vidc_winograd_input_transform_stem: unsupported shape (Cin=%d must be 1 or 3)", cin[g]);
+        gr.x[g] = x[g];
+        gr.cin[g] = cin[g];
+    }
+    const int Ho = (H + 2 - 3) / 2 + 1, Wo = (W + 2 - 3) / 2 + 1;
+    const int th = (Ho + 3) / 4, tw = (Wo + 3) / 4;
+    if (ldv == 0) ldv = 36 * G * Cout;
+    VIDC_REQUIRE(ldv >= 36 * G * Cout && ldv % 4 == 0, VIDC_ERR_SHAPE, "vidc_winograd_input_transform_stem: bad row stride ldv = %d", ldv);
+    VIDC_REQUIRE((long long)B * th <= 65535 && (g_hi - g_lo) * (Cout / 64) <= 65535, VIDC_ERR_SHAPE,
+                 "vidc_winograd_input_transform_stem: B * tile rows = %lld exceed the grid", (long long)B * th);
+    const dim3 grid((unsigned)vidc::cdiv(tw, kStemTiles), (unsigned)(B * th), (unsigned)((g_hi - g_lo) * (Cout / 64)));
+    hipLaunchKernelGGL(wino_in_stem_kernel, grid, dim3(256), 0, vidc::as_stream(stream), gr, w_packed, v, H, W, Ho, Wo, Cout, g_lo, th, tw, ldv, relu);
+    VIDC_CHECK_LAUNCH("wino_in_stem_kernel");
+    return VIDC_OK;
+}
+
+extern "C" int vidc_winograd_output_transform_maxpool(const float* mm, float* y, const float* scale1, const float* shift1, const float* scale2,
+                                                      const float* shift2, int B, int Ho, int Wo, int C, int Cout, int ldy, int flags, int ldm,
+                                                      vidc_stream_t stream) {
+    VIDC_REQUIRE(mm && y && scale1 && shift1, VIDC_ERR_NULL, "vidc_winograd_output_transform_maxpool: null pointer");
+    VIDC_REQUIRE(B > 0 && Ho > 0 && Wo > 0 && C > 0 && Cout > 0 && C % Cout == 0 && Cout % 4 == 0 && ldy % 4 == 0 && ldy >= C, VIDC_ERR_SHAPE,
+                 "vidc_winograd_output_transform_maxpool: bad shape (C = G * Cout, Cout and ldy multiples of 4)");
+    VIDC_REQUIRE(!(flags & ~(VIDC_RELU1 | VIDC_AFFINE2 | VIDC_RELU2)), VIDC_ERR_SHAPE, "vidc_winograd_output_transform_maxpool: unsupported flags 0x%x", flags);
+    VIDC_REQUIRE(!(flags & VIDC_AFFINE2) || (scale2 && shift2), VIDC_ERR_NULL, "vidc_winograd_output_transform_maxpool: AFFINE2 without scale2 / shift2");
+    const int th = (Ho + 3) / 4, tw = (Wo + 3) / 4;
+    const int Hp = (Ho + 2 - 3) / 2 + 1, Wp = (Wo + 2 - 3) / 2 + 1;
+    if (ldm == 0) ldm = 36 * C;
+    VIDC_REQUIRE(ldm >= 36 * C && ldm % 4 == 0, VIDC_ERR_SHAPE, "vidc_winograd_output_transform_maxpool: bad row stride ldm = %d", ldm);
+    VIDC_REQUIRE(B <= 65535, VIDC_ERR_SHAPE, "vidc_winograd_output_transform_maxpool: B = %d exceeds the grid", B);
+    VIDC_REQUIRE((long long)B * th * tw * ldm < (1ll << 32), VIDC_ERR_SHAPE, "vidc_winograd_output_transform_maxpool: M exceeds 32-bit element offsets");
+    const int strips = vidc::cdiv(tw, kPoolCols - 1), slices = vidc::cdiv(C, kPoolSlice);
+    const long long base = (long long)strips * slices * B;
+    int segs = (int)((512 + base - 1) / base);
+    segs = segs < 1 ? 1 : segs;
+    int seg_rows = vidc::cdiv(th, segs);
+    seg_rows = seg_rows < 4 ? 4 : seg_rows;
+    segs = vidc::cdiv(th, seg_rows);
+    const dim3 grid((unsigned)(strips * slices), (unsigned)segs, (unsigned)B);
+    hipLaunchKernelGGL(wino_out_pool_kernel<2>, grid, dim3(kPoolCols * kPoolSlice / 2), 0, vidc::as_stream(stream), mm, y, scale1, shift1, scale2, shift2, Ho, Wo, Hp,
+                       Wp, C, Cout, ldy, th, tw, flags, ldm, slices, seg_rows);
+    VIDC_CHECK_LAUNCH("wino_out_pool_kernel");
+    return VIDC_OK;
+}
diff --git a/vi_depth_completion_amd/engine.py b/vi_depth_completion_amd/engine.py
--- a/vi_depth_completion_amd/engine.py
+++ b/vi_depth_completion_amd/engine.py
@@ -109,6 +109,18 @@
             co, ci = u.shape[1], u.shape[2]
             for g in range(len(keys)):
                 L.check(L.lib().vidc_winograd_weight_pack_fused(L.ptr(u[g * 36]), L.ptr(out[g * 36]), co, ci, L.current_stream()), "winograd weights (fused order)")
+            self._cache[ck] = out
+        return self._cache[ck]
+
+    def packed_stems(self, keys):
+        ck = ("stems",) + tuple(keys)
+        if ck not in self._cache:
+            ws = [self.sd()[k + ".weight"] for k in keys]
+            co = ws[0].shape[0]
+            out = torch.zeros((len(ws), co, 27), dtype=torch.float32, device=ws[0].device)
+            for g, w in enumerate(ws):
+                assert w.shape[0] == co and w.shape[1] in (1, 3) and tuple(w.shape[2:]) == (3, 3)
+                out[g, :, :w.shape[1] * 9] = w.reshape(co, -1)
             self._cache[ck] = out
         return self._cache[ck]
 
@@ -250,6 +262,7 @@
                  "warp_params": L.OP_WARP_PARAMS, "warp_fwd": L.OP_WARP_FWD, "warp_inv": L.OP_WARP_INV, "avgpool": L.OP_AVGPOOL,
                  "normalize": L.OP_NORMALIZE, "det_im2col": L.OP_DET_IM2COL, "mask": L.OP_MASK, "wino_in": L.OP_WINO_IN,
                  "wino_out": L.OP_WINO_OUT, "nearest2x": L.OP_NEAREST2X, "copy": L.OP_COPY}, **{f.kind: f.op for f in IMAGE_FORMATS.values()})
+GLUE_KINDS = {"stem": L.OP_WINO_IN_STEM, "pool": L.OP_WINO_OUT_POOL}
 MODE_LAYERS = {"mxfp8": (mxfp8_layer, L.PREC_MXFP8), "bf16": (bf16_layer, L.PREC_BF16)}
 
 
@@ -279,6 +292,7 @@
         self.cuts = []
         self._cut_markers = []
         self.n_fused_splits = self.n_fused_quants = self.n_fused_casts = self.n_fused_warps = 0
+        self.n_glue_stems = self.n_glue_pools = 0
         self.mode = mode if mode is not None else precision_mode()
         if self.mode not in ("fp32", "mixed", "mxfp8", "bf16"):
             raise ValueError("unknown precision mode %r (VIDC_PRECISION: fp32, mixed, mxfp8 or bf16)" % (self.mode,))
@@ -667,6 +681,50 @@
         self.ops = [op for t, op in enumerate(self.ops) if t not in drop]
         self.n_fused_warps = len(drop)
 
+    def _fuse_wino_glue(self):
+        marks = {id(mk) for mk in self._cut_markers}
+        image_keys = [fmt.out_key for fmt in IMAGE_FORMATS.values()]
+        drop = set()
+        for i, (kind, reads, writes, kw) in enumerate(self.ops):
+            if kind == "wino_in" and kw["m"] == 4 and not kw["split"]:
+                x = kw["x"]
+                wr = [t for t in range(len(self.ops)) if x.buf in self.ops[t][2]]
+                stems = sorted((self.ops[t][3] for t in wr if self.ops[t][0] == "stem"), key=lambda k: k["g"])
+                if not wr or len(stems) != len(wr) or max(wr) > i or x.buf in self.pinned or x.G > 4 or x.C % 64 or x.ch_off or x.ld != x.C * x.G or \
+                        [k["g"] for k in stems] != list(range(x.G)) or \
+                        any(t != i and x.buf in self.ops[t][1] for t in range(len(self.ops))) or self._cut_between(marks, min(wr), i):
+                    continue
+                x0 = stems[0]["x"]
+                if any(k.get("warp") is not None or k.get("no_f32") or any(k.get(ik) is not None for ik in image_keys) or k["relu"] != stems[0]["relu"] or
+                       k["y"].buf != x.buf or (k["y"].C, k["y"].G, k["y"].ld) != (x.C, x.G, x.ld) or k["stream_id"] != kw["stream_id"] or
+                       (k["x"].B, k["x"].H, k["x"].W) != (x0.B, x0.H, x0.W) or k["x"].C not in (1, 3) for k in stems) or any(id(self.ops[t]) in marks for t in wr):
+                    continue
+                kw["glue"], kw["stems"] = "stem", stems
+                for k in stems:
+                    kw["wait_mask"] |= k["wait_mask"]
+                reads[:] = [k["x"].buf for k in stems]
+                drop.update(wr)
+                self.buf_elems[x.buf] = 0
+                self.n_glue_stems += len(wr)
+            elif kind == "maxpool" and not kw.get("no_f32") and not any(kw.get(ik) is not None for ik in image_keys):
+                x = kw["x"]
+                wr = [t for t in range(len(self.ops)) if x.buf in self.ops[t][2]]
+                if len(wr) != 1 or wr[0] > i or self.ops[wr[0]][0] != "wino_out" or x.buf in self.pinned or id(self.ops[i]) in marks:
+                    continue
+                j = wr[0]
+                pk = self.ops[j][3]
+                y = pk["y"]
+                if pk["m"] != 4 or pk.get("glue") or pk["flags"] & ~(L.RELU1 | L.AFFINE2 | L.RELU2) or (y.buf, y.ch_off, y.C, y.G, y.ld) != (x.buf, 0, x.C, x.G, x.C * x.G) or \
+                        x.ch_off or x.ld != x.C * x.G or kw["wait_mask"] or kw["stream_id"] != pk["stream_id"] or self._cut_between(marks, j, i) or \
+                        any(t != i and x.buf in self.ops[t][1] for t in range(len(self.ops))):
+                    continue
+                pk["glue"], pk["pool"] = "pool", kw["y"]
+                self.ops[j][2][:] = [kw["y"].buf]
+                drop.add(i)
+                self.buf_elems[x.buf] = 0
+                self.n_glue_pools += 1
+        self.ops = [op for t, op in enumerate(self.ops) if t not in drop]
+
     def _conv_desc(self, kw, dry_run):
         x, y, keys, f = kw["x"], kw["y"], kw["keys"], kw["flags"]
         co, ci, kh, kwid, Ho, Wo = kw["geom"]
@@ -817,6 +875,16 @@
 
     def _lower_wino_in(self, g, kw):
         x, v = kw["x"], kw["v"]
+        if kw.get("glue") == "stem":
+            stems = kw["stems"]
+            wp = self.ws.packed_stems([k["key"] for k in stems])
+            self._keep.append(wp)
+            x0 = stems[0]["x"]
+            _args(g, [self._addr(k["x"]) for k in stems] + [0] * (4 - len(stems)) + [wp.data_ptr(), self._addr(v)],
+                  (x0.B, x0.H, x0.W, x.C, x.G, 0, x.G, int(stems[0]["relu"]), v.ld, 0, 0, 0, 0))
+            for k in stems:
+                g.i[9 + k["g"]] = k["x"].C
+            return "wino_in:F4:%dx%dx%d+stem" % (x.H, x.W, x.C * x.G)
         _args(g, (self._addr(x), self._addr(v)), (x.B, x.H, x.W, x.C * x.G, x.ld, kw["cin"], kw["m"], kw["split"], v.ld))
         return "wino_in:F%d:%dx%dx%d" % (kw["m"], x.H, x.W, x.C * x.G)
 
@@ -825,6 +893,11 @@
         s1, b1 = self.ws.affine(list(keys), list(kw["bn"]) if kw["bn"] is not None else None)
         s2, b2 = self.ws.affine([None] * len(keys), list(kw["bn2"])) if kw["bn2"] is not None else (None, None)
         self._keep += [t for t in (s1, b1, s2, b2) if t is not None]
+        if kw.get("glue") == "pool":
+            pool = kw["pool"]
+            _args(g, (self._addr(mm), self._addr(pool), 0, s1.data_ptr(), b1.data_ptr(), L.ptr(s2) or 0, L.ptr(b2) or 0),
+                  (y.B, y.H, y.W, y.C * y.G, kw["cout"], pool.ld, kw["m"], kw["flags"], mm.ld))
+            return "wino_out:F4:%dx%dx%d+maxpool" % (y.H, y.W, y.C * y.G)
         _args(g, (self._addr(mm), 0 if kw["flags"] & L.NO_F32_OUT else self._addr(y), self._addr(kw.get("split_out")), s1.data_ptr(), b1.data_ptr(),
                   L.ptr(s2) or 0, L.ptr(b2) or 0), (y.B, y.H, y.W, y.C * y.G, kw["cout"], y.ld, kw["m"], kw["flags"], mm.ld))
         return "wino_out:F%d:%dx%dx%d" % (kw["m"], y.H, y.W, y.C * y.G)
@@ -846,6 +919,8 @@
             self._fuse_warp_into_stem()
         if os.environ.get("VIDC_FUSE_SPLIT", "1") == "1":
             self._fuse_images()
+        if os.environ.get("VIDC_WINO_GLUE", "0" if "VIDC_WINO_FUSED" in os.environ else "1") != "0":
+            self._fuse_wino_glue()
         self.cuts = [next(i for i, op in enumerate(self.ops) if op is mk) + 1 for mk in self._cut_markers]
         assert len(self.cuts) < L.MAX_SEGMENTS and self.cuts == sorted(set(self.cuts))
         self.storage = self._plan_buffers()
@@ -868,6 +943,7 @@
                 name = self._lower_image(op.u.g, kw, IMAGE_FORMATS[kind])
             else:
                 name = getattr(self, "_lower_" + kind)(op.u.g, kw)
+                op.kind = GLUE_KINDS.get(kw.get("glue"), op.kind)
             self.op_names.append(name)
         self.workspaces = {sid: torch.zeros(nb // 4 + 4, dtype=torch.float32, device=self.device) for sid, nb in ws_need.items()}
         for op in ws_ops:
@@ -947,6 +1023,9 @@
             elif kind == "wino_in" and kw["x"].G == groups:
                 g = ops[j].u.g
                 cin, a2 = kw["cin"], (kw["m"] + 2) ** 2
+                if kw.get("glue") == "stem":
+                    g.i[5], g.i[6] = g_lo, g_hi
+                    continue
                 g.p[0], g.p[1] = g.p[0] + 4 * g_lo * cin, g.p[1] + 4 * g_lo * a2 * cin
                 g.i[3] = cin * (g_hi - g_lo)
             elif kind == "wino_out" and len(kw["keys"]) == groups:
diff --git a/vi_depth_completion_amd/ops.py b/vi_depth_completion_amd/ops.py
--- a/vi_depth_completion_amd/ops.py
+++ b/vi_depth_completion_amd/ops.py
@@ -245,6 +245,43 @@
     return y
 
 
+def winograd_input_transform_stem(xs_nchw, ws_oihw, relu=True, g_lo=0, g_hi=None, v=None):
+    import ctypes as C
+    _dev(*xs_nchw, *ws_oihw)
+    xs = [x.contiguous().float() for x in xs_nchw]
+    G = len(xs)
+    g_hi = G if g_hi is None else g_hi
+    B, _c, H, W = xs[0].shape
+    co = ws_oihw[0].shape[0]
+    wp = torch.zeros((G, co, 27), dtype=torch.float32, device=xs[0].device)
+    for g, w in enumerate(ws_oihw):
+        wp[g, :, :w.shape[1] * 9] = w.float().reshape(co, -1)
+    Ho, Wo = (H + 2 - 3) // 2 + 1, (W + 2 - 3) // 2 + 1
+    if v is None:
+        v = torch.empty((B * -(-Ho // 4) * -(-Wo // 4), 36 * G * co), dtype=torch.float32, device=xs[0].device)
+    ptrs = (C.c_void_p * G)(*[L.ptr(x) for x in xs])
+    cins = (C.c_int * G)(*[x.shape[1] for x in xs])
+    L.check(L.lib().vidc_winograd_input_transform_stem(ptrs, cins, L.ptr(wp), L.ptr(v), B, H, W, co, G, g_lo, g_hi, int(relu), 0, L.current_stream()),
+            "winograd_input_transform_stem")
+    return v
+
+
+def winograd_output_transform_maxpool(mm, B, Ho, Wo, cout, scale1, shift1, relu1=False, scale2=None, shift2=None, relu2=False):
+    _dev(mm, scale1, shift1)
+    mm = mm.contiguous()
+    Cc = mm.shape[1] // 36
+    y = torch.empty((B, (Ho - 1) // 2 + 1, (Wo - 1) // 2 + 1, Cc), dtype=torch.float32, device=mm.device)
+    s1, b1 = scale1.contiguous().float().view(-1), shift1.contiguous().float().view(-1)
+    flags = (L.RELU1 if relu1 else 0)
+    s2 = b2 = None
+    if scale2 is not None:
+        s2, b2 = scale2.contiguous().float().view(-1), shift2.contiguous().float().view(-1)
+        flags |= L.AFFINE2 | (L.RELU2 if relu2 else 0)
+    L.check(L.lib().vidc_winograd_output_transform_maxpool(L.ptr(mm), L.ptr(y), L.ptr(s1), L.ptr(b1), L.ptr(s2), L.ptr(b2), B, Ho, Wo, Cc, cout, Cc,
+                                                           flags, 0, L.current_stream()), "winograd_output_transform_maxpool")
+    return y
+
+
 def conv3x3_winograd(x, w_oihw_groups, scale1, shift1, m, relu1=False, scale2=None, shift2=None, relu2=False, precision=0, tile=0, splitk=1,
                      split_out=None, no_f32_out=False):
     if precision not in (L.PREC_FP32, L.PREC_BF16X3):
```

New measurement: 642.5, median of 6. About the same (+0.9%).
